# ZihanLiao/pytorch-kaldi-resnet

Hardware: AMD Instinct MI355X
Metric: utterances/sec (300-frame x 80 fbank, bs256/GPU), ResNet-34 + AAM-softmax training step (higher is better)
Workload: dtype f32 (operands as 2 fp16 terms of value x 2^k, 3 cross products, f32 accumulate); 1 GPU; BASELINE configs[1]: ResNet-34 + AAM-softmax (m 0.2, s 30), 1211 speakers, 300-frame x 80 fbank, per-GPU batch 256, fwd+CE+bwd+SGD(0.9, wd 5e-4); global_batch=256, frames=300, feat_dim=80, parallelism=dp1, launch=hipGraph replay (1 graph), mfma=f16x3

## Files before the change

include/spkhip.h:

```cpp
#ifndef SPKHIP_H
#define SPKHIP_H
#include <stddef.h>
#ifdef __cplusplus
extern "C" {
#endif

int spk_version(void);
const char* spk_last_error(void);
int spk_build_flags(void);

#define SPK_IN_AFFINE_RELU 1
#define SPK_EPI_AFFINE 2
#define SPK_EPI_ADD 4
#define SPK_EPI_RELU 8
#define SPK_EPI_STATS 16
#define SPK_IN_BNBWD 64
#define SPK_EPI_BNBWD 32

#define SPK_CONV_WS 128
#define SPK_CONV_PIPE 1024

#define SPK_CONV_M16 (1 << 17)

#define SPK_WGRAD_GROUPS 2048

#define SPK_WGRAD_NOSHIFT (1 << 18)
#define SPK_WGRAD_M16 (1 << 19)
#define SPK_IN_PRESPLIT (1 << 14)
#define SPK_SIDE_PRESPLIT (1 << 15)
#define SPK_DY_PRESPLIT (1 << 16)
#define SPK_EPI_WMASK (1 << 24)


int spk_pack_conv_weight(const float* w, float* wpk, int Cout, int Cin, int KH, int KW, int transpose, void* stream);
int spk_pack_conv_weight_split(const float* w, void* wpk, int Cout, int Cin, int KH, int KW, int transpose, int split,
                               void* stream);
int spk_pack_job_bytes(void);
int spk_pack_conv_weights_batched(const void* jobs, int njobs, int total_blocks, int has_f16 , void* stream);

int spk_conv_mfma(const float* in, const float* wpk, float* out, const float* in_scale, const float* in_shift,
                  const float* epi_scale, const float* epi_shift, const float* epi_add, const float* in_raw,
                  const float* in_act, const float* in_bn4, const float* in_coef, const unsigned* in_mask , const unsigned* bn_mask , const unsigned* add_mask ,
                  float* side_draw, float* side_dz,
                  const float* bn_raw, const float* bn_act, const float* bn4, float* stats, int B, int IH,
                  int IW, int Cin, int OH, int OW, int OHf, int OWf, int Cout, int IS, int OS, int ooy, int oox,
                  int ntaps, const int* tap_dy , const int* tap_dx , const int* tap_w , int TH,
                  int TW, int MT, int NT, int kc, int ips, int flags, int split, const unsigned* in_amax, unsigned* out_amax,
                  unsigned* side_amax, void* stream);
int spk_conv_mfma_len(const float* in, const float* wpk, float* out, const float* in_scale, const float* in_shift,
                      const float* epi_scale, const float* epi_shift, const float* epi_add, const float* in_raw,
                      const float* in_act, const float* in_bn4, const float* in_coef, const unsigned* in_mask,
                      const unsigned* bn_mask, const unsigned* add_mask, float* side_draw, float* side_dz,
                      const float* bn_raw, const float* bn_act, const float* bn4, float* stats, int B, int IH,
                      int IW, int Cin, int OH, int OW, int OHf, int OWf, int Cout, int IS, int OS, int ooy, int oox,
                      int ntaps, const int* tap_dy , const int* tap_dx , const int* tap_w , int TH,
                      int TW, int MT, int NT, int kc, int ips, int flags, int split, const unsigned* in_amax, unsigned* out_amax,
                      unsigned* side_amax, const int* wlen , void* stream);

int spk_conv_wgrad_limits(int WN, int* max_halo_pix , int* max_tile_pix );
size_t spk_conv_wgrad_workspace(int nsplit, int ksize, int Cin, int Cout);
int spk_conv3x3_c32_stream(const float* in, const float* wpk, float* out, const float* in_scale, const float* in_shift, float* stats,
                           int B, int H, int W, int flags, const unsigned* in_amax, unsigned* out_amax, int nblocks, void* stream);
int spk_conv1x1_stream(const float* in, const float* wpk, float* out, const float* in_scale, const float* in_shift,
                       const float* epi_add, const unsigned* add_mask, const float* bn_raw, const unsigned* bn_mask,
                       const float* bn4, float* stats, long long P, int C, int flags, const unsigned* in_amax, unsigned* out_amax,
                       int nblocks, void* stream);
int spk_conv1x1_stream_rows(int nblocks, int C);
int spk_wgrad_reduce(const float* partial, float* dw, int nslab, int ksize, int Cin, int Cout, int accumulate, void* stream);
int spk_conv_wgrad(const float* x, const float* dy, float* dw, float* partial, const float* in_scale,
                   const float* in_shift, int B, int IH, int IW, int Cin, int OH, int OW, int Cout, int ksize, int stride,
                   int TH, int TW, int WN, int nsplit, int flags, int accumulate, int split , const unsigned* dy_amax , const unsigned* x_amax , void* stream);

int spk_stem_fwd_blocks(int B, int F, int T);
int spk_stem_conv_fwd(const float* x, const float* w, float* out, float* stats, const float* epi_scale,
                      const float* epi_shift, int B, int F, int T, int flags,
                      unsigned* amax_out , void* stream);
int spk_stem_conv_fwd_len(const float* x, const float* w, float* out, float* stats, const float* epi_scale,
                          const float* epi_shift, int B, int F, int T, int flags, unsigned* amax_out, const int* len ,
                          void* stream);
int spk_stem_wgrad_blocks(int B, int F, int T);
int spk_stem_conv_wgrad(const float* x, const float* draw, float* dw, float* partial, int B, int F, int T,
                        int accumulate, void* stream);

int spk_bn_stats_blocks(long long N, int C);
int spk_bn_stats_partial(const float* x, float* partial , long long N, int C, void* stream);
size_t spk_bn_finalize_workspace(int nblk, int C);
int spk_bn_finalize(const float* partial, int nblk, int C, double count, const float* gamma, const float* beta,
                    float* running_mean, float* running_var, long long* num_batches_tracked, float* mean, float* invstd,
                    float* scale, float* shift, float momentum, float eps, double* ws,
                    const unsigned* amax_in, unsigned* est_out ,
                    void* stream);
int spk_bn_eval_coeffs(const float* gamma, const float* beta, const float* running_mean, const float* running_var,
                       float* scale, float* shift, int C, float eps, void* stream);
int spk_bn_apply(const float* raw, const float* scale, const float* shift, const float* res, const float* res_scale,
                 const float* res_shift, float* out, unsigned* mask_out, long long N, int C, int relu,
                 unsigned* amax_out , void* stream);
int spk_bn_bwd_reduce(const float* dy, const float* raw, const float* act, const float* mean, const float* invstd,
                      const float* scale, const float* shift, float* partial, long long N, int C, int mask_mode,
                      unsigned* chan_amax , void* stream);
int spk_bn_bwd_finalize(const float* partial, int nblk, int C, double count, const float* gamma, const float* invstd,
                        float* dgamma, float* dbeta, float* coef , int accumulate, double* ws,
                        const unsigned* amax_in, const unsigned* raw_amax, const float* mean, unsigned* est_out ,
                        const unsigned* chan_amax ,
                        void* stream);
int spk_bn_bwd_apply(const float* dy, const float* raw, const float* act, const float* mean, const float* invstd,
                     const float* scale, const float* shift, const float* coef, float* draw, float* dz_out, long long N,
                     int C, int mask_mode, unsigned* amax_out ,
                     const unsigned* pair_scale , void* stream);
int spk_absmax(const float* x, unsigned* slot, long long n, void* stream);
int spk_bnbwd_estimate(const float* coef, const float* mean, const float* invstd, int C, const unsigned* amax_in,
                       const unsigned* raw_amax, unsigned* est, void* stream);
int spk_f16_window_count(const float* x, const float* scale, const float* shift, long long n, int C, const unsigned* slot,
                         int pairs, unsigned long long* counts , void* stream);
int spk_affine_estimate(const float* scale, const float* shift, int C, const unsigned* amax_in, unsigned* est, void* stream);

int spk_stats_pool_fwd(const float* x , float* out , int B, int H, int W, int C,
                       int mode, void* stream);
int spk_stats_pool_fwd_len(const float* x, float* out, const int* wlen, int B, int H, int W, int C, int mode, void* stream);
int spk_stats_pool_bwd(const float* x, const float* gout, float* dx, int B, int H, int W, int C, int mode,
                       unsigned* amax_out , void* stream);

int spk_gemm_splitk(int M, int N, int K);
size_t spk_gemm_workspace(int M, int N, int K);
int spk_gemm_f32(const float* A, const float* B, float* C, const float* bias, int M, int N, int K, long long sam,
                 long long sak, long long sbk, long long sbn, long long ldc, float alpha, int accumulate, float* workspace,
                 void* stream);
int spk_colsum(const float* dy, float* db, int M, int N, int accumulate, void* stream);

int spk_l2norm_fwd(const float* x, float* y, float* inv_norm, int R, int D, float eps, void* stream);
int spk_l2norm_bwd(const float* y, const float* inv_norm, const float* dy, float* dx, int R, int D, float eps,
                   int accumulate, void* stream);
int spk_aam_margin_fwd(const float* cosv, const long long* label, float* logits, int B, int S, float m, float s,
                       void* stream);
int spk_aam_margin_bwd(const float* cosv, const long long* label, const float* dlogits, float* dcos, int B, int S,
                       float m, float s, void* stream);
int spk_softmax_ce(const float* logits, const long long* label, float* loss_row, float* dlogits, int* rank, int B, int S,
                   float grad_scale, void* stream);
int spk_mean(const float* v, float* out, int n, void* stream);
int spk_relu_bwd(const float* y, const float* dy, float* dx, long long n, void* stream);

int spk_sgd_step(float* p, const float* g, float* buf, long long n, float lr, float momentum, float weight_decay,
                 float grad_scale, int first_step, void* stream);

int spk_center_normalize(const float* emb , const float* mean , float* out, int N, int D, float eps,
                         void* stream);
int spk_trial_cosine(const float* en , const float* te , const int* ia, const int* ib, float* out,
                     int T, int D, int n_en, int n_te, void* stream);
int spk_topk_mean_std(const float* scores, float* mean_out, float* std_out, int N, int M, int k, long long ld, void* stream);

int spk_fbank_tile_frames(int L, int S, int P, int F);
int spk_fbank_fwd(const float* wave, const int* nsamp, const long long* utt_ids, int B, long long Nmax, const float* window,
                  const float* twiddle, const float* mel_w, const int* mel_lo, const int* mel_off, int L, int S, int P, int F,
                  int snip_edges, float dither, float preemph, int remove_dc, float energy_floor, unsigned long long seed,
                  float* feats, float* log_energy, int* T_out, int Tcap, void* stream);
int spk_fbank_dither_noise(float* out , long long utt_id, unsigned long long seed, int frame0, int nframes, int L,
                           void* stream);
int spk_vad_count(const float* log_energy, const int* T, int B, int Tcap, double energy_threshold, double mean_scale,
                  int frames_context, double proportion, int* vad , int* idx , int* count ,
                  void* stream);
int spk_cmn_select(const float* x, const int* T, const int* idx, const int* count, double* prefix, float* out, int B, int F,
                   int Tcap, int Tout, int cmn_window, void* stream);

int spk_resample_tile(int iu, int ou, int K);
int spk_resample_fwd(const float* wave_in, const int* nsamp_in, int B, long long Nmax_in, const int* first, const float* wq,
                     int fi, int fo, int K, float* wave_out, int* nsamp_out, long long Nmax_out, void* stream);

int spk_augment_max_rir(void);
int spk_augment_max_early(void);
int spk_augment_workspace(int B, long long Nmax, int Rmax, int Emax, long long Fmax, int nd, long long* sizes );
int spk_augment_fwd(const float* wave, const int* nsamp, int B, long long Nmax, const float* rir_pool, long long rir_pool_len,
                    const long long* rir_off, const int* rir_row, int Rmax, int Emax, const float* noise_pool,
                    long long noise_pool_len, const int* desc_ptr, const long long* desc_off, const int* desc_len,
                    const double* desc_snr, int nd, long long Fmax, const float* twiddle, float* spectra, float* y, double* work,
                    int quantize, float* out, unsigned long long* clipped, void* stream);

int spk_cm_decode(const unsigned char* codes, const float* colhdr, const int* lengths, int B, int F, int T, float* out, void* stream);
int spk_cm_compress(const float* x, const int* T, int B, int F, int Tcap, float* ws, float* minrange, int* hdr, unsigned char* codes,
                    void* stream);

#ifdef __cplusplus
}
#endif
#endif
```

pytorch-kaldi-resnet_amd/csrc/bn.hip:

```cpp
#include "spk_common.h"

enum { MASK_NONE = 0, MASK_ACT = 1, MASK_RAW = 2, MASK_BITS = 3 };

__global__ __launch_bounds__(256) void bn_stats_partial_kernel(const float* __restrict__ x, float* __restrict__ partial,
                                                               long long N, int C, int rows_per_block) {
    __shared__ float red[256][8];
    const int tid = threadIdx.x;
    const int qpr = C >> 2;
    const int quad = tid % qpr, prow = tid / qpr, rstep = 256 / qpr;
    const long long r0 = (long long)blockIdx.x * rows_per_block;
    long long r1 = r0 + rows_per_block;
    if (r1 > N) r1 = N;
    f32x4 s = {0.f, 0.f, 0.f, 0.f}, ss = {0.f, 0.f, 0.f, 0.f};
    for (long long r = r0 + prow; r < r1; r += rstep) {
        const f32x4 v = *(const f32x4*)(x + r * C + quad * 4);
        s += v;
        ss += v * v;
    }
#pragma unroll
    for (int k = 0; k < 4; ++k) {
        red[tid][k] = s[k];
        red[tid][4 + k] = ss[k];
    }
    __syncthreads();
    if (tid < qpr) {
        float a[8];
#pragma unroll
        for (int k = 0; k < 8; ++k) a[k] = 0.f;
        for (int p = 0; p < rstep; ++p)
#pragma unroll
            for (int k = 0; k < 8; ++k) a[k] += red[p * qpr + tid][k];
        float* dst = partial + ((size_t)blockIdx.x * C + tid * 4) * 2;
#pragma unroll
        for (int k = 0; k < 4; ++k) {
            dst[k * 2 + 0] = a[k];
            dst[k * 2 + 1] = a[4 + k];
        }
    }
}

static bool bn_c_ok(int C) { return C >= 4 && C <= 1024 && (C & (C - 1)) == 0; }

#ifndef BN_STATS_BLOCKS
#define BN_STATS_BLOCKS 4096
#endif
extern "C" int spk_bn_stats_blocks(long long N, int C) {
    (void)C;
    long long nb = (N + 255) / 256;
    if (nb > BN_STATS_BLOCKS) nb = BN_STATS_BLOCKS;
    return (int)(nb < 1 ? 1 : nb);
}

extern "C" int spk_bn_stats_partial(const float* x, float* partial, long long N, int C, void* stream) {
    SPK_REQUIRE(x && partial, "spk_bn_stats_partial: null pointer");
    SPK_REQUIRE(N > 0 && bn_c_ok(C), "spk_bn_stats_partial: N=%lld C=%d (C must be a power of two in [4,1024])", N, C);
    const int nb = spk_bn_stats_blocks(N, C);
    const int rpb = (int)((N + nb - 1) / nb);
    hipLaunchKernelGGL(bn_stats_partial_kernel, dim3(nb), dim3(256), 0, (hipStream_t)stream, x, partial, N, C, rpb);
    SPK_LAUNCH_CHECK("spk_bn_stats_partial");
    return 0;
}

#define BN_STAGE_ROWS 256
__global__ __launch_bounds__(256) void bn_fold_partials_kernel(const float* __restrict__ partial, double* __restrict__ ws,
                                                               int nblk, int C) {
    __shared__ double red[8][32][2];
    const int tid = threadIdx.x, c = tid & 31, row = tid >> 5;
    const int ch = blockIdx.x * 32 + c;
    const int per = (nblk + BN_STAGE_ROWS - 1) / BN_STAGE_ROWS;
    const int k0 = blockIdx.y * per;
    int k1 = k0 + per;
    if (k1 > nblk) k1 = nblk;
    double s = 0.0, ss = 0.0;
    if (ch < C) {
        const size_t pitch = (size_t)8 * C * 2;
        const float* q = partial + ((size_t)(k0 + row) * C + ch) * 2;
        int k = k0 + row;
        for (; k + 24 < k1; k += 32, q += 4 * pitch) {
            const float2 a = *(const float2*)q, b = *(const float2*)(q + pitch);
            const float2 c2 = *(const float2*)(q + 2 * pitch), d = *(const float2*)(q + 3 * pitch);
            s += (double)a.x; ss += (double)a.y;
            s += (double)b.x; ss += (double)b.y;
            s += (double)c2.x; ss += (double)c2.y;
            s += (double)d.x; ss += (double)d.y;
        }
        for (; k < k1; k += 8, q += pitch) {
            const float2 p = *(const float2*)q;
            s += (double)p.x;
            ss += (double)p.y;
        }
    }
    red[row][c][0] = s;
    red[row][c][1] = ss;
    __syncthreads();
    if (row == 0 && ch < C) {
        for (int k = 1; k < 8; ++k) {
            s += red[k][c][0];
            ss += red[k][c][1];
        }
        ws[((size_t)blockIdx.y * C + ch) * 2 + 0] = s;
        ws[((size_t)blockIdx.y * C + ch) * 2 + 1] = ss;
    }
}

template <typename T>
__device__ inline void bn_sum_rows(const T* __restrict__ partial, int nrows, int C, int ch, int row, double& s, double& ss) {
    const size_t pitch = (size_t)8 * C * 2;
    const T* p = partial + ((size_t)row * C + ch) * 2;
    int k = row;
    for (; k + 24 < nrows; k += 32, p += 4 * pitch) {
        const T a0 = p[0], a1 = p[1], b0 = p[pitch], b1 = p[pitch + 1];
        const T c0 = p[2 * pitch], c1 = p[2 * pitch + 1], d0 = p[3 * pitch], d1 = p[3 * pitch + 1];
        s += (double)a0; ss += (double)a1;
        s += (double)b0; ss += (double)b1;
        s += (double)c0; ss += (double)c1;
        s += (double)d0; ss += (double)d1;
    }
    for (; k < nrows; k += 8, p += pitch) {
        s += (double)p[0];
        ss += (double)p[1];
    }
}

template <typename T>
__global__ __launch_bounds__(256) void bn_finalize_kernel(const T* __restrict__ partial, int nblk, int C, double count,
                                                          const float* __restrict__ gamma, const float* __restrict__ beta,
                                                          float* __restrict__ running_mean, float* __restrict__ running_var,
                                                          long long* __restrict__ nbt, float* __restrict__ mean_out,
                                                          float* __restrict__ invstd_out, float* __restrict__ scale,
                                                          float* __restrict__ shift, float momentum, float eps,
                                                          const unsigned* __restrict__ amax_in, unsigned* __restrict__ est_out) {
    __shared__ double red[8][32][2];
    const int tid = threadIdx.x, c = tid & 31, row = tid >> 5;
    const int ch = blockIdx.x * 32 + c;
    double s = 0.0, ss = 0.0;
    if (ch < C) bn_sum_rows<T>(partial, nblk, C, ch, row, s, ss);
    red[row][c][0] = s;
    red[row][c][1] = ss;
    __syncthreads();
    if (row == 0 && ch < C) {
        for (int k = 1; k < 8; ++k) {
            s += red[k][c][0];
            ss += red[k][c][1];
        }
        const double mean = s / count;
        double var = ss / count - mean * mean;
        if (var < 0.0) var = 0.0;
        const float invstd = (float)(1.0 / sqrt(var + (double)eps));
        const float g = gamma[ch], b = beta[ch];
        const float sc = g * invstd;
        mean_out[ch] = (float)mean;
        invstd_out[ch] = invstd;
        const float shv = b - (float)mean * sc;
        scale[ch] = sc;
        shift[ch] = shv;
        if (est_out) {
            const float e = fabsf(sc) * __uint_as_float(*amax_in) + fabsf(shv);
            const unsigned bits = __float_as_uint(e);
            if (bits > __hip_atomic_load(est_out, __ATOMIC_RELAXED, __HIP_MEMORY_SCOPE_AGENT)) atomicMax(est_out, bits);
        }
        if (running_mean) {
            const double unbiased = count > 1.0 ? var * (count / (count - 1.0)) : var;
            running_mean[ch] = (1.f - momentum) * running_mean[ch] + momentum * (float)mean;
            running_var[ch] = (1.f - momentum) * running_var[ch] + momentum * (float)unbiased;
        }
    }
    if (nbt && blockIdx.x == 0 && tid == 0) *nbt += 1;
}

extern "C" size_t spk_bn_finalize_workspace(int nblk, int C) {
    return nblk > BN_STAGE_ROWS ? (size_t)BN_STAGE_ROWS * C * 2 * sizeof(double) : 0;
}

extern "C" int spk_bn_finalize(const float* partial, int nblk, int C, double count, const float* gamma, const float* beta,
                               float* running_mean, float* running_var, long long* num_batches_tracked, float* mean,
                               float* invstd, float* scale, float* shift, float momentum, float eps, double* ws,
                               const unsigned* amax_in, unsigned* est_out, void* stream) {
    SPK_REQUIRE(partial && gamma && beta && mean && invstd && scale && shift, "spk_bn_finalize: null pointer");
    SPK_REQUIRE(nblk > 0 && C > 0 && count > 0, "spk_bn_finalize: bad sizes");
    SPK_REQUIRE((running_mean == nullptr) == (running_var == nullptr), "spk_bn_finalize: running stats must come in pairs");
    SPK_REQUIRE(!est_out || amax_in, "spk_bn_finalize: est_out needs amax_in");
    hipStream_t st = (hipStream_t)stream;
    if (spk_bn_finalize_workspace(nblk, C)) {
        SPK_REQUIRE(ws, "spk_bn_finalize: %d partial rows need the fp64 workspace", nblk);
        hipLaunchKernelGGL(bn_fold_partials_kernel, dim3(spk_ceil_div(C, 32), BN_STAGE_ROWS), dim3(256), 0, st, partial, ws, nblk, C);
        SPK_LAUNCH_CHECK("spk_bn_finalize(fold)");
        hipLaunchKernelGGL(bn_finalize_kernel<double>, dim3(spk_ceil_div(C, 32)), dim3(256), 0, st, ws, BN_STAGE_ROWS, C, count,
                           gamma, beta, running_mean, running_var, num_batches_tracked, mean, invstd, scale, shift, momentum, eps,
                           amax_in, est_out);
    } else {
        hipLaunchKernelGGL(bn_finalize_kernel<float>, dim3(spk_ceil_div(C, 32)), dim3(256), 0, st, partial, nblk, C, count, gamma,
                           beta, running_mean, running_var, num_batches_tracked, mean, invstd, scale, shift, momentum, eps, amax_in,
                           est_out);
    }
    SPK_LAUNCH_CHECK("spk_bn_finalize");
    return 0;
}

__global__ void bn_eval_coeffs_kernel(const float* gamma, const float* beta, const float* rm, const float* rv,
                                      float* scale, float* shift, int C, float eps) {
    const int c = blockIdx.x * blockDim.x + threadIdx.x;
    if (c >= C) return;
    const float invstd = 1.f / sqrtf(rv[c] + eps);
    const float sc = gamma[c] * invstd;
    scale[c] = sc;
    shift[c] = beta[c] - rm[c] * sc;
}

extern "C" int spk_bn_eval_coeffs(const float* gamma, const float* beta, const float* running_mean,
                                  const float* running_var, float* scale, float* shift, int C, float eps, void* stream) {
    SPK_REQUIRE(gamma && beta && running_mean && running_var && scale && shift, "spk_bn_eval_coeffs: null pointer");
    hipLaunchKernelGGL(bn_eval_coeffs_kernel, dim3(spk_ceil_div(C, 256)), dim3(256), 0, (hipStream_t)stream, gamma, beta,
                       running_mean, running_var, scale, shift, C, eps);
    SPK_LAUNCH_CHECK("spk_bn_eval_coeffs");
    return 0;
}

#ifndef BN_APPLY_U
#define BN_APPLY_U 4
#endif
#ifndef BN_APPLY_CAP
#define BN_APPLY_CAP 0
#endif
#ifndef BN_BWD_APPLY_U
#define BN_BWD_APPLY_U 1
#endif
#ifndef BN_BWD_APPLY_CAP
#define BN_BWD_APPLY_CAP 2048
#endif
static int stream_grid(long long nquads, int per_thread = 1, int cap = 8192) {
    long long nb = (nquads + 256LL * per_thread - 1) / (256LL * per_thread);
    if (cap > 0 && nb > cap) nb = cap;
    if (nb > 2147483647LL) nb = 2147483647LL;
    return (int)(nb < 1 ? 1 : nb);
}
#ifndef BN_NT
#define BN_NT 1
#endif
static __device__ __forceinline__ f32x4 ld_stream(const float* p) {
#if BN_NT
    return __builtin_nontemporal_load((const f32x4*)p);
#else
    return *(const f32x4*)p;
#endif
}
static __device__ __forceinline__ void st_stream(float* p, f32x4 v) {
#if BN_NT
    __builtin_nontemporal_store(v, (f32x4*)p);
#else
    *(f32x4*)p = v;
#endif
}
__global__ __launch_bounds__(256) void bn_apply_kernel(const float* __restrict__ raw, const float* __restrict__ scale,
                                                       const float* __restrict__ shift, const float* __restrict__ res,
                                                       const float* __restrict__ rscale, const float* __restrict__ rshift,
                                                       float* __restrict__ out, unsigned* __restrict__ mask_out, long long nquads,
                                                       int C, int relu, unsigned* __restrict__ amax_out) {
    const int cmask = C - 1;
    float mx = 0.f;
    constexpr int U = BN_APPLY_U;
    const long long stride = (long long)gridDim.x * 256;
    const bool fixed_c = C <= 1024;
    const int c0 = (threadIdx.x * 4) & cmask;
    f32x4 psc = *(const f32x4*)(scale + c0), psh = *(const f32x4*)(shift + c0), prs = psc, prh = psh;
    if (rscale) {
        prs = *(const f32x4*)(rscale + c0);
        prh = *(const f32x4*)(rshift + c0);
    }
    for (long long i0 = (long long)blockIdx.x * 256 + threadIdx.x; i0 < nquads; i0 += stride * U) {
        f32x4 rv[U], sv[U];
        long long idx[U];
#pragma unroll
        for (int u = 0; u < U; ++u) {
            const long long i = i0 + stride * u;
            idx[u] = i < nquads ? i : i0;
            rv[u] = ld_stream(raw + idx[u] * 4);
            if (res) sv[u] = ld_stream(res + idx[u] * 4);
        }
#pragma unroll
        for (int u = 0; u < U; ++u) {
            const long long i = i0 + stride * u;
            if (i >= nquads) continue;
            if (!fixed_c) {
                const int c = (int)((i * 4) & cmask);
                psc = *(const f32x4*)(scale + c);
                psh = *(const f32x4*)(shift + c);
                if (rscale) {
                    prs = *(const f32x4*)(rscale + c);
                    prh = *(const f32x4*)(rshift + c);
                }
            }
            f32x4 v = rv[u] * psc + psh;
            if (res) {
                f32x4 r = sv[u];
                if (rscale) r = r * prs + prh;
                v += r;
            }
            if (relu) {
                v[0] = fmaxf(v[0], 0.f);
                v[1] = fmaxf(v[1], 0.f);
                v[2] = fmaxf(v[2], 0.f);
                v[3] = fmaxf(v[3], 0.f);
            }
            st_stream(out + i * 4, v);
            mx = fmaxf(fmaxf(mx, fmaxf(fabsf(v[0]), fabsf(v[1]))), fmaxf(fabsf(v[2]), fabsf(v[3])));
            if (mask_out) {
                unsigned bits = (v[0] > 0.f ? 1u : 0u) | (v[1] > 0.f ? 2u : 0u) | (v[2] > 0.f ? 4u : 0u) | (v[3] > 0.f ? 8u : 0u);
                bits <<= 4 * (threadIdx.x & 7);
                bits |= __shfl_xor(bits, 1, 64);
                bits |= __shfl_xor(bits, 2, 64);
                bits |= __shfl_xor(bits, 4, 64);
                if ((threadIdx.x & 7) == 0) mask_out[i >> 3] = bits;
            }
        }
    }
    if (amax_out) spk_wave_amax_commit(mx, amax_out);
}

extern "C" int spk_bn_apply(const float* raw, const float* scale, const float* shift, const float* res,
                            const float* res_scale, const float* res_shift, float* out, unsigned* mask_out, long long N, int C,
                            int relu, unsigned* amax_out, void* stream) {
    SPK_REQUIRE(raw && scale && shift && out, "spk_bn_apply: null pointer");
    SPK_REQUIRE(N > 0 && bn_c_ok(C), "spk_bn_apply: N=%lld C=%d", N, C);
    SPK_REQUIRE((res_scale == nullptr) == (res_shift == nullptr), "spk_bn_apply: residual affine must come in pairs");
    SPK_REQUIRE(!res_scale || res, "spk_bn_apply: residual affine without residual");
    SPK_REQUIRE(!mask_out || C % 32 == 0, "spk_bn_apply: the sign mask needs C %% 32 == 0 (C=%d)", C);
    const long long nquads = N * C / 4;
    hipLaunchKernelGGL(bn_apply_kernel, dim3(stream_grid(nquads, BN_APPLY_U, BN_APPLY_CAP)), dim3(256), 0, (hipStream_t)stream, raw, scale, shift, res,
                       res_scale, res_shift, out, mask_out, nquads, C, relu, amax_out);
    SPK_LAUNCH_CHECK("spk_bn_apply");
    return 0;
}

__device__ inline f32x4 bn_mask(f32x4 dy, int mode, const float* act, const float* raw_p, f32x4 rawv, f32x4 sc, f32x4 sh,
                                long long off, int C = 0) {
    if (mode == MASK_BITS) {
        const int lg = 31 - __builtin_clz((unsigned)C);
        const long long pix = off >> lg;
        const int c = (int)(off & (C - 1));
        const unsigned bits = ((const unsigned*)act)[pix * (C >> 5) + (c >> 5)] >> (c & 31);
#pragma unroll
        for (int k = 0; k < 4; ++k) dy[k] = ((bits >> k) & 1u) ? dy[k] : 0.f;
    } else if (mode == MASK_ACT) {
        const f32x4 a = *(const f32x4*)(act + off);
#pragma unroll
        for (int k = 0; k < 4; ++k) dy[k] = a[k] > 0.f ? dy[k] : 0.f;
    } else if (mode == MASK_RAW) {
        const f32x4 z = rawv * sc + sh;
#pragma unroll
        for (int k = 0; k < 4; ++k) dy[k] = z[k] > 0.f ? dy[k] : 0.f;
    }
    (void)raw_p;
    return dy;
}

__global__ __launch_bounds__(256) void bn_bwd_reduce_kernel(const float* __restrict__ dy, const float* __restrict__ raw,
                                                            const float* __restrict__ act, const float* __restrict__ mean,
                                                            const float* __restrict__ invstd, const float* __restrict__ scale,
                                                            const float* __restrict__ shift, float* __restrict__ partial,
                                                            long long N, int C, int rows_per_block, int mode,
                                                            unsigned* __restrict__ chan_amax) {
    __shared__ float red[256][8];
    const int tid = threadIdx.x;
    const int qpr = C >> 2;
    const int quad = tid % qpr, prow = tid / qpr, rstep = 256 / qpr;
    const long long r0 = (long long)blockIdx.x * rows_per_block;
    long long r1 = r0 + rows_per_block;
    if (r1 > N) r1 = N;
    const f32x4 mu = *(const f32x4*)(mean + quad * 4), is = *(const f32x4*)(invstd + quad * 4);
    const f32x4 sc = *(const f32x4*)(scale + quad * 4), sh = *(const f32x4*)(shift + quad * 4);
    f32x4 s = {0.f, 0.f, 0.f, 0.f}, ss = {0.f, 0.f, 0.f, 0.f}, mx = {0.f, 0.f, 0.f, 0.f};
    for (long long r = r0 + prow; r < r1; r += rstep) {
        const long long off = r * C + quad * 4;
        const f32x4 rv = ld_stream(raw + off);
        f32x4 d = ld_stream(dy + off);
        d = bn_mask(d, mode, act, raw, rv, sc, sh, off, C);
        const f32x4 xh = (rv - mu) * is;
        s += d;
        ss += d * xh;
#pragma unroll
        for (int k = 0; k < 4; ++k) mx[k] = fmaxf(mx[k], spk_finite_abs(d[k]));
    }
#pragma unroll
    for (int k = 0; k < 4; ++k) {
        red[tid][k] = s[k];
        red[tid][4 + k] = ss[k];
    }
    __syncthreads();
    if (tid < qpr) {
        float a[8];
#pragma unroll
        for (int k = 0; k < 8; ++k) a[k] = 0.f;
        for (int p = 0; p < rstep; ++p)
#pragma unroll
            for (int k = 0; k < 8; ++k) a[k] += red[p * qpr + tid][k];
        float* dst = partial + ((size_t)blockIdx.x * C + tid * 4) * 2;
#pragma unroll
        for (int k = 0; k < 4; ++k) {
            dst[k * 2 + 0] = a[k];
            dst[k * 2 + 1] = a[4 + k];
        }
    }
    if (chan_amax) {
        __syncthreads();
#pragma unroll
        for (int k = 0; k < 4; ++k) red[tid][k] = mx[k];
        __syncthreads();
        if (tid < qpr) {
#pragma unroll
            for (int k = 0; k < 4; ++k) {
                float m = 0.f;
                for (int p = 0; p < rstep; ++p) m = fmaxf(m, red[p * qpr + tid][k]);
                const unsigned bits = __float_as_uint(m);
                unsigned* slot = chan_amax + tid * 4 + k;
                if (bits > __hip_atomic_load(slot, __ATOMIC_RELAXED, __HIP_MEMORY_SCOPE_AGENT)) atomicMax(slot, bits);
            }
        }
    }
}

extern "C" int spk_bn_bwd_reduce(const float* dy, const float* raw, const float* act, const float* mean, const float* invstd,
                                 const float* scale, const float* shift, float* partial, long long N, int C, int mask_mode,
                                 unsigned* chan_amax, void* stream) {
    SPK_REQUIRE(dy && raw && mean && invstd && scale && shift && partial, "spk_bn_bwd_reduce: null pointer");
    SPK_REQUIRE(N > 0 && bn_c_ok(C), "spk_bn_bwd_reduce: N=%lld C=%d", N, C);
    SPK_REQUIRE(mask_mode >= 0 && mask_mode <= 3, "spk_bn_bwd_reduce: mask_mode=%d", mask_mode);
    SPK_REQUIRE((mask_mode != MASK_ACT && mask_mode != MASK_BITS) || act, "spk_bn_bwd_reduce: MASK_ACT / MASK_BITS need the activated tensor / its sign bits");
    const int nb = spk_bn_stats_blocks(N, C);
    const int rpb = (int)((N + nb - 1) / nb);
    hipLaunchKernelGGL(bn_bwd_reduce_kernel, dim3(nb), dim3(256), 0, (hipStream_t)stream, dy, raw, act, mean, invstd, scale,
                       shift, partial, N, C, rpb, mask_mode, chan_amax);
    SPK_LAUNCH_CHECK("spk_bn_bwd_reduce");
    return 0;
}

__device__ inline float bnbwd_bound(float k1, float m1, float m2, float mean, float invstd, float A, float R) {
    const float xh = (R + fabsf(mean)) * fabsf(invstd);
    return fabsf(k1) * (A + fabsf(m1) + xh * fabsf(m2)) * (1.f + 1.52587890625e-05f);
}

template <typename T>
__global__ __launch_bounds__(256) void bn_bwd_finalize_kernel(const T* __restrict__ partial, int nblk, int C, double count,
                                                              const float* __restrict__ gamma, const float* __restrict__ invstd,
                                                              float* __restrict__ dgamma, float* __restrict__ dbeta,
                                                              float* __restrict__ coef, int accumulate,
                                                              const unsigned* __restrict__ amax_in, const unsigned* __restrict__ raw_amax,
                                                              const float* __restrict__ mean, unsigned* __restrict__ est_out,
                                                              const unsigned* __restrict__ chan_amax) {
    __shared__ double red[8][32][2];
    const int tid = threadIdx.x, c = tid & 31, row = tid >> 5;
    const int ch = blockIdx.x * 32 + c;
    double s = 0.0, ss = 0.0;
    if (ch < C) bn_sum_rows<T>(partial, nblk, C, ch, row, s, ss);
    red[row][c][0] = s;
    red[row][c][1] = ss;
    __syncthreads();
    if (row == 0 && ch < C) {
        for (int k = 1; k < 8; ++k) {
            s += red[k][c][0];
            ss += red[k][c][1];
        }
        dbeta[ch] = accumulate ? dbeta[ch] + (float)s : (float)s;
        dgamma[ch] = accumulate ? dgamma[ch] + (float)ss : (float)ss;
        const float k1 = gamma[ch] * invstd[ch], m1 = (float)(s / count), m2 = (float)(ss / count);
        coef[ch] = k1;
        coef[C + ch] = m1;
        coef[2 * C + ch] = m2;
        if (est_out) {
            const float A = chan_amax ? __uint_as_float(chan_amax[ch]) : __uint_as_float(*amax_in);
            const float e = bnbwd_bound(k1, m1, m2, mean[ch], invstd[ch], A, __uint_as_float(*raw_amax));
            const unsigned bits = __float_as_uint(e);
            if (bits > __hip_atomic_load(est_out, __ATOMIC_RELAXED, __HIP_MEMORY_SCOPE_AGENT)) atomicMax(est_out, bits);
        }
    }
}

extern "C" int spk_bn_bwd_finalize(const float* partial, int nblk, int C, double count, const float* gamma,
                                   const float* invstd, float* dgamma, float* dbeta, float* coef, int accumulate,
                                   double* ws, const unsigned* amax_in, const unsigned* raw_amax, const float* mean,
                                   unsigned* est_out, const unsigned* chan_amax, void* stream) {
    SPK_REQUIRE(partial && gamma && invstd && dgamma && dbeta && coef, "spk_bn_bwd_finalize: null pointer");
    SPK_REQUIRE(nblk > 0 && C > 0 && count > 0, "spk_bn_bwd_finalize: bad sizes");
    SPK_REQUIRE(!est_out || ((amax_in || chan_amax) && raw_amax && mean),
                "spk_bn_bwd_finalize: est_out needs amax_in (or chan_amax), raw_amax and mean");
    hipStream_t st = (hipStream_t)stream;
    if (spk_bn_finalize_workspace(nblk, C)) {
        SPK_REQUIRE(ws, "spk_bn_bwd_finalize: %d partial rows need the fp64 workspace", nblk);
        hipLaunchKernelGGL(bn_fold_partials_kernel, dim3(spk_ceil_div(C, 32), BN_STAGE_ROWS), dim3(256), 0, st, partial, ws, nblk, C);
        SPK_LAUNCH_CHECK("spk_bn_bwd_finalize(fold)");
        hipLaunchKernelGGL(bn_bwd_finalize_kernel<double>, dim3(spk_ceil_div(C, 32)), dim3(256), 0, st, ws, BN_STAGE_ROWS, C, count,
                           gamma, invstd, dgamma, dbeta, coef, accumulate, amax_in, raw_amax, mean, est_out, chan_amax);
    } else {
        hipLaunchKernelGGL(bn_bwd_finalize_kernel<float>, dim3(spk_ceil_div(C, 32)), dim3(256), 0, st, partial, nblk, C, count, gamma,
                           invstd, dgamma, dbeta, coef, accumulate, amax_in, raw_amax, mean, est_out, chan_amax);
    }
    SPK_LAUNCH_CHECK("spk_bn_bwd_finalize");
    return 0;
}

__global__ __launch_bounds__(256) void bn_bwd_apply_kernel(const float* __restrict__ dy, const float* __restrict__ raw,
                                                           const float* __restrict__ act, const float* __restrict__ mean,
                                                           const float* __restrict__ invstd, const float* __restrict__ scale,
                                                           const float* __restrict__ shift, const float* __restrict__ coef,
                                                           float* __restrict__ draw, float* __restrict__ dz_out,
                                                           unsigned nquads, int C, int mode, unsigned* __restrict__ amax_out,
                                                           const unsigned* __restrict__ pair_scale) {
    const int cmask = C - 1;
    float mx = 0.f;
    const float sig = pair_scale ? spk_sigma_from_amax_bits(*pair_scale) : 1.f;
    constexpr int U = BN_BWD_APPLY_U;
    const unsigned stride = gridDim.x * 256u;
    const int lgq = 29 - __builtin_clz((unsigned)C);
    const unsigned cw = (unsigned)C >> 5;
    const bool fixed_c = C <= 1024;
    const int c0 = (threadIdx.x * 4) & cmask;
    f32x4 pmu = *(const f32x4*)(mean + c0), pis = *(const f32x4*)(invstd + c0), pk1 = *(const f32x4*)(coef + c0);
    f32x4 pm1 = *(const f32x4*)(coef + C + c0), pm2 = *(const f32x4*)(coef + 2 * C + c0), psc = pmu, psh = pmu;
    if (mode == MASK_RAW) {
        psc = *(const f32x4*)(scale + c0);
        psh = *(const f32x4*)(shift + c0);
    }
    for (unsigned i0 = blockIdx.x * 256u + threadIdx.x; i0 < nquads; i0 += stride * U) {
        f32x4 rvv[U], dv[U], av[U];
        unsigned mw[U];
#pragma unroll
        for (int u = 0; u < U; ++u) {
            const unsigned i = i0 + stride * u;
            const unsigned ii = i < nquads && i >= i0 ? i : i0;
            const size_t off = (size_t)ii * 4;
            rvv[u] = ld_stream(raw + off);
            dv[u] = ld_stream(dy + off);
            if (mode == MASK_BITS) mw[u] = ((const unsigned*)act)[(size_t)(ii >> lgq) * cw + (((ii * 4u) & (unsigned)cmask) >> 5)];
            else if (mode == MASK_ACT) av[u] = *(const f32x4*)(act + off);
        }
#pragma unroll
        for (int u = 0; u < U; ++u) {
            const unsigned i = i0 + stride * u;
            if (i >= nquads || i < i0) continue;
            const int c = fixed_c ? c0 : (int)((i * 4u) & (unsigned)cmask);
            if (!fixed_c) {
                pmu = *(const f32x4*)(mean + c);
                pis = *(const f32x4*)(invstd + c);
                pk1 = *(const f32x4*)(coef + c);
                pm1 = *(const f32x4*)(coef + C + c);
                pm2 = *(const f32x4*)(coef + 2 * C + c);
                if (mode == MASK_RAW) {
                    psc = *(const f32x4*)(scale + c);
                    psh = *(const f32x4*)(shift + c);
                }
            }
            const size_t off = (size_t)i * 4;
            const f32x4 rv = rvv[u];
            f32x4 d = dv[u];
            if (mode == MASK_BITS) {
                const unsigned bits = mw[u] >> (c & 31);
#pragma unroll
                for (int k = 0; k < 4; ++k) d[k] = ((bits >> k) & 1u) ? d[k] : 0.f;
            } else if (mode == MASK_ACT) {
#pragma unroll
                for (int k = 0; k < 4; ++k) d[k] = av[u][k] > 0.f ? d[k] : 0.f;
            } else if (mode == MASK_RAW) {
                const f32x4 z = rv * psc + psh;
#pragma unroll
                for (int k = 0; k < 4; ++k) d[k] = z[k] > 0.f ? d[k] : 0.f;
            }
            const f32x4 xh = (rv - pmu) * pis;
            const f32x4 o = pk1 * (d - pm1 - xh * pm2);
            if (dz_out) st_stream(dz_out + off, d);
            if (pair_scale) {
                uint2 t0, t1;
                split2h(o, sig, t0, t1);
                st_stream(draw + off, spk_pair_pack(t0, t1));
            } else
                st_stream(draw + off, o);
            mx = fmaxf(fmaxf(mx, fmaxf(fabsf(o[0]), fabsf(o[1]))), fmaxf(fabsf(o[2]), fabsf(o[3])));
        }
    }
    if (amax_out) spk_wave_amax_commit(mx, amax_out);
}

extern "C" int spk_bn_bwd_apply(const float* dy, const float* raw, const float* act, const float* mean, const float* invstd,
                                const float* scale, const float* shift, const float* coef, float* draw, float* dz_out,
                                long long N, int C, int mask_mode, unsigned* amax_out, const unsigned* pair_scale, void* stream) {
    SPK_REQUIRE(dy && raw && mean && invstd && scale && shift && coef && draw, "spk_bn_bwd_apply: null pointer");
    SPK_REQUIRE(N > 0 && bn_c_ok(C), "spk_bn_bwd_apply: N=%lld C=%d", N, C);
    SPK_REQUIRE(mask_mode >= 0 && mask_mode <= 3, "spk_bn_bwd_apply: mask_mode=%d", mask_mode);
    SPK_REQUIRE((mask_mode != MASK_ACT && mask_mode != MASK_BITS) || act, "spk_bn_bwd_apply: MASK_ACT / MASK_BITS need the activated tensor / its sign bits");
    const long long nquads = N * C / 4;
    SPK_REQUIRE(nquads < 2147483647LL / 8, "spk_bn_bwd_apply: %lld values exceed the 32-bit group index of the kernel", N * C);
    hipLaunchKernelGGL(bn_bwd_apply_kernel, dim3(stream_grid(nquads, BN_BWD_APPLY_U, BN_BWD_APPLY_CAP)), dim3(256), 0, (hipStream_t)stream, dy, raw, act, mean,
                       invstd, scale, shift, coef, draw, dz_out, (unsigned)nquads, C, mask_mode, amax_out, pair_scale);
    SPK_LAUNCH_CHECK("spk_bn_bwd_apply");
    return 0;
}

__global__ __launch_bounds__(256) void absmax_kernel(const float* __restrict__ x, long long n, unsigned* __restrict__ slot) {
    float mx = 0.f;
    const long long nq = n >> 2;
    for (long long i = (long long)blockIdx.x * 256 + threadIdx.x; i < nq; i += (long long)gridDim.x * 256) {
        const f32x4 v = *(const f32x4*)(x + i * 4);
        mx = fmaxf(fmaxf(mx, fmaxf(spk_finite_abs(v[0]), spk_finite_abs(v[1]))), fmaxf(spk_finite_abs(v[2]), spk_finite_abs(v[3])));
    }
    if (blockIdx.x == 0 && threadIdx.x < (n & 3)) mx = fmaxf(mx, spk_finite_abs(x[nq * 4 + threadIdx.x]));
    spk_wave_amax_commit(mx, slot);
}

extern "C" int spk_absmax(const float* x, unsigned* slot, long long n, void* stream) {
    SPK_REQUIRE(x && slot && n > 0, "spk_absmax: bad arguments");
    SPK_REQUIRE((((size_t)x) & 15) == 0, "spk_absmax: x must be 16-byte aligned");
    hipLaunchKernelGGL(absmax_kernel, dim3(stream_grid(n / 4 + 1)), dim3(256), 0, (hipStream_t)stream, x, n, slot);
    SPK_LAUNCH_CHECK("spk_absmax");
    return 0;
}

__global__ __launch_bounds__(256) void bnbwd_estimate_kernel(const float* __restrict__ coef, const float* __restrict__ mean,
                                                             const float* __restrict__ invstd, int C,
                                                             const unsigned* __restrict__ amax_in, const unsigned* __restrict__ raw_amax,
                                                             unsigned* __restrict__ est) {
    __shared__ float red[4];
    const float A = __uint_as_float(*amax_in), R = __uint_as_float(*raw_amax);
    float mx = 0.f;
    for (int c = threadIdx.x; c < C; c += 256)
        mx = fmaxf(mx, bnbwd_bound(coef[c], coef[C + c], coef[2 * C + c], mean[c], invstd[c], A, R));
#pragma unroll
    for (int off = 32; off >= 1; off >>= 1) mx = fmaxf(mx, __shfl_xor(mx, off, 64));
    if ((threadIdx.x & 63) == 0) red[threadIdx.x >> 6] = mx;
    __syncthreads();
    if (threadIdx.x == 0) *est = __float_as_uint(fmaxf(fmaxf(red[0], red[1]), fmaxf(red[2], red[3])));
}

__global__ __launch_bounds__(256) void affine_estimate_kernel(const float* __restrict__ scale, const float* __restrict__ shift, int C,
                                                              const unsigned* __restrict__ amax_in, unsigned* __restrict__ est) {
    __shared__ float red[2][4];
    float ms = 0.f, mh = 0.f;
    for (int c = threadIdx.x; c < C; c += 256) {
        ms = fmaxf(ms, fabsf(scale[c]));
        mh = fmaxf(mh, fabsf(shift[c]));
    }
#pragma unroll
    for (int off = 32; off >= 1; off >>= 1) {
        ms = fmaxf(ms, __shfl_xor(ms, off, 64));
        mh = fmaxf(mh, __shfl_xor(mh, off, 64));
    }
    if ((threadIdx.x & 63) == 0) {
        red[0][threadIdx.x >> 6] = ms;
        red[1][threadIdx.x >> 6] = mh;
    }
    __syncthreads();
    if (threadIdx.x == 0) {
        ms = fmaxf(fmaxf(red[0][0], red[0][1]), fmaxf(red[0][2], red[0][3]));
        mh = fmaxf(fmaxf(red[1][0], red[1][1]), fmaxf(red[1][2], red[1][3]));
        *est = __float_as_uint(ms * __uint_as_float(*amax_in) + mh);
    }
}

extern "C" int spk_affine_estimate(const float* scale, const float* shift, int C, const unsigned* amax_in, unsigned* est,
                                   void* stream) {
    SPK_REQUIRE(scale && shift && amax_in && est && C > 0, "spk_affine_estimate: bad arguments");
    hipLaunchKernelGGL(affine_estimate_kernel, dim3(1), dim3(256), 0, (hipStream_t)stream, scale, shift, C, amax_in, est);
    SPK_LAUNCH_CHECK("spk_affine_estimate");
    return 0;
}

extern "C" int spk_bnbwd_estimate(const float* coef, const float* mean, const float* invstd, int C, const unsigned* amax_in,
                                  const unsigned* raw_amax, unsigned* est, void* stream) {
    SPK_REQUIRE(coef && mean && invstd && amax_in && raw_amax && est && C > 0, "spk_bnbwd_estimate: bad arguments");
    hipLaunchKernelGGL(bnbwd_estimate_kernel, dim3(1), dim3(256), 0, (hipStream_t)stream, coef, mean, invstd, C, amax_in, raw_amax, est);
    SPK_LAUNCH_CHECK("spk_bnbwd_estimate");
    return 0;
}

__global__ __launch_bounds__(256) void f16_window_count_kernel(const float* __restrict__ x, const float* __restrict__ scale,
                                                               const float* __restrict__ shift, long long nquads, int C,
                                                               const unsigned* __restrict__ slot, int pairs,
                                                               unsigned long long* __restrict__ counts) {
    const float sig = spk_sigma_from_amax_bits(*slot);
    const int cmask = C - 1;
    unsigned n = 0, sat = 0, lo_lost = 0, hi_sub = 0;
    for (long long i = (long long)blockIdx.x * 256 + threadIdx.x; i < nquads; i += (long long)gridDim.x * 256) {
        f32x4 v = *(const f32x4*)(x + i * 4);
        float hi[4], lo[4];
        if (pairs) {
            const uint4 u = __builtin_bit_cast(uint4, v);
            const f16x4 a = __builtin_bit_cast(f16x4, (uint2){u.x, u.y}), b = __builtin_bit_cast(f16x4, (uint2){u.z, u.w});
#pragma unroll
            for (int k = 0; k < 4; ++k) {
                hi[k] = (float)a[k];
                lo[k] = (float)b[k];
                sat += fabsf(hi[k]) >= 65504.f;
            }
        } else {
            if (scale) {
                const int c = (int)((i * 4) & cmask);
                v = v * *(const f32x4*)(scale + c) + *(const f32x4*)(shift + c);
#pragma unroll
                for (int k = 0; k < 4; ++k) v[k] = fmaxf(v[k], 0.f);
            }
#pragma unroll
            for (int k = 0; k < 4; ++k) {
                const float u = v[k] * sig;
                sat += fabsf(u) > 65504.f;
                const float uc = __builtin_amdgcn_fmed3f(u, -65504.f, 65504.f);
                const _Float16 a = (_Float16)uc;
                hi[k] = (float)a;
                lo[k] = (float)(_Float16)(uc - (float)a);
            }
        }
#pragma unroll
        for (int k = 0; k < 4; ++k) {
            n += 1;
            lo_lost += lo[k] != 0.f && fabsf(lo[k]) < 6.103515625e-05f;
            hi_sub += hi[k] != 0.f && fabsf(hi[k]) < 6.103515625e-05f;
        }
    }
    unsigned vals[4] = {n, sat, lo_lost, hi_sub};
#pragma unroll
    for (int j = 0; j < 4; ++j) {
        unsigned v = vals[j];
#pragma unroll
        for (int off = 32; off >= 1; off >>= 1) v += __shfl_xor(v, off, 64);
        if ((threadIdx.x & 63) == 0 && v) atomicAdd(counts + j, (unsigned long long)v);
    }
}

extern "C" int spk_f16_window_count(const float* x, const float* scale, const float* shift, long long n, int C,
                                    const unsigned* slot, int pairs, unsigned long long* counts, void* stream) {
    SPK_REQUIRE(x && slot && counts && n > 0 && n % 4 == 0, "spk_f16_window_count: bad arguments (n must be a multiple of 4)");
    SPK_REQUIRE((scale == nullptr) == (shift == nullptr), "spk_f16_window_count: scale / shift come in pairs");
    SPK_REQUIRE(!scale || (bn_c_ok(C) && !pairs), "spk_f16_window_count: the affine form needs a power-of-two C and an fp32 tensor");
    hipLaunchKernelGGL(f16_window_count_kernel, dim3(stream_grid(n / 4)), dim3(256), 0, (hipStream_t)stream, x, scale, shift, n / 4,
                       scale ? C : 4, slot, pairs, counts);
    SPK_LAUNCH_CHECK("spk_f16_window_count");
    return 0;
}
```

pytorch-kaldi-resnet_amd/csrc/conv_split.hip:

```cpp
#include "conv_kernel.h"

template <int MT, int NT, int SPLIT>
static int launch_split(const ConvArgs& a, size_t lds_bytes, hipStream_t st) {
    if (a.flags & SPK_IN_BNBWD) {
#ifndef SPK_NO_FL_VARIANTS
        if constexpr (SPLIT == 3 && MT == 2 && NT == 1) {
            const int var = a.flags | (a.add_mask ? SPK_FL_ADDMASK : 0) | (a.bn_mask ? SPK_FL_BNMASK : 0) | (a.in_mask ? SPK_FL_INMASK : 0);
            constexpr int V2 = SPK_IN_BNBWD | SPK_SIDE_PRESPLIT | SPK_EPI_STATS | SPK_EPI_BNBWD | SPK_FL_INMASK;
            constexpr int V1 = SPK_IN_BNBWD | SPK_SIDE_PRESPLIT | SPK_EPI_ADD | SPK_EPI_STATS | SPK_EPI_BNBWD | SPK_FL_ADDMASK | SPK_FL_BNMASK;
            if (!a.in_act && !a.bn_act && !a.side_dz && (var == V1 || var == V2)) {
                if (var == V2) hipLaunchKernelGGL((conv_mfma_kernel<MT, NT, true, SPLIT, V2>), dim3(a.nblocks), dim3(256), lds_bytes, st, a);
                else hipLaunchKernelGGL((conv_mfma_kernel<MT, NT, true, SPLIT, V1>), dim3(a.nblocks), dim3(256), lds_bytes, st, a);
                SPK_LAUNCH_CHECK("spk_conv_mfma(split)");
                return 0;
            }
        }
#endif
        hipLaunchKernelGGL((conv_mfma_kernel<MT, NT, true, SPLIT>), dim3(a.nblocks), dim3(256), lds_bytes, st, a);
    } else if (a.flags & SPK_EPI_WMASK) {
        hipLaunchKernelGGL((conv_mfma_kernel<MT, NT, false, SPLIT, SPK_EPI_WMASK>), dim3(a.nblocks), dim3(256), lds_bytes, st, a);
    } else {
#ifndef SPK_NO_FL_VARIANTS
        if constexpr (SPLIT == 3 && ((MT == 2 && NT == 1) || (MT == 1 && NT == 2) || (MT == 2 && NT == 2))) {
            if (!a.add_mask && !a.bn_mask && !a.bn_act) {
                if (a.flags == (SPK_IN_AFFINE_RELU | SPK_EPI_STATS)) {
                    hipLaunchKernelGGL((conv_mfma_kernel<MT, NT, false, SPLIT, SPK_IN_AFFINE_RELU | SPK_EPI_STATS>), dim3(a.nblocks), dim3(256), lds_bytes, st, a);
                    SPK_LAUNCH_CHECK("spk_conv_mfma(split)");
                    return 0;
                }
                if (a.flags == SPK_EPI_STATS) {
                    hipLaunchKernelGGL((conv_mfma_kernel<MT, NT, false, SPLIT, SPK_EPI_STATS>), dim3(a.nblocks), dim3(256), lds_bytes, st, a);
                    SPK_LAUNCH_CHECK("spk_conv_mfma(split)");
                    return 0;
                }
            }
        }
#endif
        hipLaunchKernelGGL((conv_mfma_kernel<MT, NT, false, SPLIT>), dim3(a.nblocks), dim3(256), lds_bytes, st, a);
    }
    SPK_LAUNCH_CHECK("spk_conv_mfma(split)");
    return 0;
}

int spk_launch_conv_split(const ConvArgs& a, size_t lds_bytes, int MT, int NT, int split, hipStream_t st) {
#define CASE(M, N)                                                      \
    if (MT == M && NT == N) {                                           \
        if (split == 3) return launch_split<M, N, 3>(a, lds_bytes, st); \
        if (split == 6) return launch_split<M, N, 6>(a, lds_bytes, st); \
        return launch_split<M, N, 9>(a, lds_bytes, st);                 \
    }
    CASE(1, 1) CASE(2, 1) CASE(3, 1) CASE(4, 1) CASE(1, 2) CASE(2, 2) CASE(3, 2) CASE(1, 4)
#undef CASE
    spk_set_error("spk_conv_mfma: unsupported split tile config MT=%d NT=%d", MT, NT);
    return -1;
}

#ifdef CONV_STAMPS
extern "C" int spk_debug_stamps(unsigned long long* out, int nblocks) {
    if (nblocks < 0) {
        void* p = nullptr;
        if (hipGetSymbolAddress(&p, HIP_SYMBOL(g_conv_stamps)) != hipSuccess) return -1;
        return (int)hipMemset(p, 0, sizeof(unsigned long long) * 16 * CONV_STAMP_BLOCKS);
    }
    if (nblocks > CONV_STAMP_BLOCKS) nblocks = CONV_STAMP_BLOCKS;
    return (int)hipMemcpyFromSymbol(out, HIP_SYMBOL(g_conv_stamps), (size_t)nblocks * 16 * sizeof(unsigned long long), 0, hipMemcpyDeviceToHost);
}
#endif
```

pytorch-kaldi-resnet_amd/csrc/spk_common.h:

```cpp
#pragma once
#include <hip/hip_runtime.h>
#include <stdint.h>

typedef float f32x4 __attribute__((ext_vector_type(4)));
typedef float f32x16 __attribute__((ext_vector_type(16)));

void spk_set_error(const char* fmt, ...);
#define SPK_REQUIRE(cond, ...)                 \
    do {                                       \
        if (!(cond)) {                         \
            spk_set_error(__VA_ARGS__);        \
            return -1;                         \
        }                                      \
    } while (0)
#define SPK_LAUNCH_CHECK(name)                                                          \
    do {                                                                                \
        hipError_t e__ = hipGetLastError();                                             \
        if (e__ != hipSuccess) {                                                        \
            spk_set_error("%s: launch failed: %s", name, hipGetErrorString(e__));       \
            return (int)e__;                                                            \
        }                                                                               \
    } while (0)

enum {
    SPK_IN_AFFINE_RELU = 1,
    SPK_EPI_AFFINE = 2,
    SPK_EPI_ADD = 4,
    SPK_EPI_RELU = 8,
    SPK_EPI_STATS = 16,
    SPK_EPI_BNBWD = 32,
    SPK_IN_BNBWD = 64,
    SPK_CONV_WS = 128,
    SPK_CONV_PIPE = 1024,
    SPK_WGRAD_GROUPS = 2048,
    SPK_IN_PRESPLIT = 1 << 14,
    SPK_SIDE_PRESPLIT = 1 << 15,
    SPK_DY_PRESPLIT = 1 << 16,
    SPK_CONV_M16 = 1 << 17,
    SPK_WGRAD_NOSHIFT = 1 << 18,
    SPK_WGRAD_M16 = 1 << 19,
    SPK_EPI_WMASK = 1 << 24
};

static inline int spk_ceil_div(int a, int b) { return (a + b - 1) / b; }

typedef __bf16 bf16x8 __attribute__((ext_vector_type(8)));
#ifdef __HIPCC__
static __device__ __forceinline__ unsigned pack_bf16x2(float lo, float hi, float& rlo, float& rhi) {
    const __bf16 a = (__bf16)lo, b = (__bf16)hi;
    rlo = lo - (float)a;
    rhi = hi - (float)b;
    return (unsigned)__builtin_bit_cast(unsigned short, a) | ((unsigned)__builtin_bit_cast(unsigned short, b) << 16);
}
static __device__ __forceinline__ void split3(f32x4 w, uint2& t0, uint2& t1, uint2& t2) {
    float r0, r1, r2, r3, q0, q1, q2, q3;
    t0.x = pack_bf16x2(w[0], w[1], r0, r1);
    t0.y = pack_bf16x2(w[2], w[3], r2, r3);
    t1.x = pack_bf16x2(r0, r1, q0, q1);
    t1.y = pack_bf16x2(r2, r3, q2, q3);
    t2.x = pack_bf16x2(q0, q1, r0, r1);
    t2.y = pack_bf16x2(q2, q3, r2, r3);
}
typedef _Float16 f16x8 __attribute__((ext_vector_type(8)));
#define SPK_F16_ACT_SIGMA 64.0f
typedef _Float16 f16x4 __attribute__((ext_vector_type(4)));
static __device__ __forceinline__ void split2h(f32x4 w, float sigma, uint2& t0, uint2& t1) {
    f32x4 u = w * sigma;
#pragma unroll
    for (int k = 0; k < 4; ++k) u[k] = __builtin_amdgcn_fmed3f(u[k], -65504.f, 65504.f);
    const f16x4 a = __builtin_convertvector(u, f16x4);
    const f32x4 r = u - __builtin_convertvector(a, f32x4);
    const f16x4 b = __builtin_convertvector(r, f16x4);
    t0 = __builtin_bit_cast(uint2, a);
    t1 = __builtin_bit_cast(uint2, b);
}
static __device__ __forceinline__ f32x4 spk_pair_pack(uint2 t0, uint2 t1) {
    return __builtin_bit_cast(f32x4, (uint4){t0.x, t0.y, t1.x, t1.y});
}
static __device__ __forceinline__ void spk_pair_unpack(f32x4 v, uint2& t0, uint2& t1) {
    const uint4 u = __builtin_bit_cast(uint4, v);
    t0 = (uint2){u.x, u.y};
    t1 = (uint2){u.z, u.w};
}
static __device__ __forceinline__ void spk_terms(f32x4 w, float sigma, bool pairs, uint2& t0, uint2& t1) {
    if (pairs) spk_pair_unpack(w, t0, t1);
    else split2h(w, sigma, t0, t1);
}
static __device__ __forceinline__ float spk_sigma_from_amax_bits(unsigned bits) {
    const int e = (int)((bits >> 23) & 0xffu);
    if (e == 0 || e == 255) return 1.f;
    int se = 127 + 14 - (e - 127);
    se = se < 1 ? 1 : (se > 254 ? 254 : se);
    return __uint_as_float((unsigned)se << 23);
}
static __device__ __forceinline__ float spk_finite_abs(float v) {
    const float a = fabsf(v);
    return a < __builtin_inff() ? a : 0.f;
}
static __device__ __forceinline__ void spk_wave_amax_commit(float v, unsigned* dst) {
#pragma unroll
    for (int off = 32; off >= 1; off >>= 1) v = fmaxf(v, __shfl_xor(v, off, 64));
    if ((threadIdx.x & 63) == 0) {
        const unsigned bits = __float_as_uint(v);
        if (bits > __hip_atomic_load(dst, __ATOMIC_RELAXED, __HIP_MEMORY_SCOPE_AGENT)) atomicMax(dst, bits);
    }
}
#endif

static __device__ __forceinline__ unsigned spk_m20(unsigned magic32) { return (magic32 + 0xFFFu) >> 12; }
static __device__ __forceinline__ int spk_div20(int p, unsigned m20) { return (int)(__umul24((unsigned)p, m20) >> 20); }
```

pytorch-kaldi-resnet_amd/csrc/stem.hip:

```cpp
#include "spk_common.h"

#define STEM_C 32

template <bool LEN>
__global__ __launch_bounds__(256) void stem_fwd_kernel(const float* __restrict__ x, const float* __restrict__ w,
                                                       float* __restrict__ out, float* __restrict__ stats,
                                                       const float* __restrict__ epi_scale,
                                                       const float* __restrict__ epi_shift, int B, int F, int T,
                                                       int flags, unsigned* __restrict__ amax_out, const int* __restrict__ len) {
    __shared__ float red[4][STEM_C][2];
    float mx = 0.f;
    const int tid = threadIdx.x, cg = tid & 3, pl = tid >> 2;
    float wr[9][8];
#pragma unroll
    for (int t = 0; t < 9; ++t)
#pragma unroll
        for (int c = 0; c < 8; ++c) wr[t][c] = w[(cg * 8 + c) * 9 + t];
    float es[8], eh[8], ssum[8], ssq[8];
#pragma unroll
    for (int c = 0; c < 8; ++c) {
        es[c] = (flags & SPK_EPI_AFFINE) ? epi_scale[cg * 8 + c] : 1.f;
        eh[c] = (flags & SPK_EPI_AFFINE) ? epi_shift[cg * 8 + c] : 0.f;
        ssum[c] = 0.f;
        ssq[c] = 0.f;
    }
    const int FT = F * T;
    const long long NP = (long long)B * FT;
    for (long long p = (long long)blockIdx.x * 64 + pl; p < NP; p += (long long)gridDim.x * 64) {
        const int b = (int)(p / FT);
        const int rem = (int)(p - (long long)b * FT);
        const int f = rem / T, t0 = rem - f * T;
        const float* xb = x + (size_t)b * FT;
        const int Tb = LEN ? min(len[b], T) : T;
        float xv[9];
#pragma unroll
        for (int kh = 0; kh < 3; ++kh)
#pragma unroll
            for (int kw = 0; kw < 3; ++kw) {
                const int ff = f + kh - 1, tt = t0 + kw - 1;
                xv[kh * 3 + kw] = (ff >= 0 && ff < F && tt >= 0 && tt < Tb) ? xb[ff * T + tt] : 0.f;
            }
        const bool tail = LEN && t0 >= Tb;
        float o[8];
#pragma unroll
        for (int c = 0; c < 8; ++c) {
            float v = 0.f;
#pragma unroll
            for (int t = 0; t < 9; ++t) v = fmaf(xv[t], wr[t][c], v);
            if (flags & SPK_EPI_AFFINE) v = v * es[c] + eh[c];
            if (flags & SPK_EPI_RELU) v = fmaxf(v, 0.f);
            if (tail) v = 0.f;
            o[c] = v;
            mx = fmaxf(mx, fabsf(v));
            ssum[c] += v;
            ssq[c] += v * v;
        }
        f32x4* dst = (f32x4*)(out + (size_t)p * STEM_C + cg * 8);
        dst[0] = (f32x4){o[0], o[1], o[2], o[3]};
        dst[1] = (f32x4){o[4], o[5], o[6], o[7]};
    }
    if (amax_out) spk_wave_amax_commit(mx, amax_out);
    if (flags & SPK_EPI_STATS) {
#pragma unroll
        for (int c = 0; c < 8; ++c) {
#pragma unroll
            for (int off = 4; off < 64; off <<= 1) {
                ssum[c] += __shfl_xor(ssum[c], off, 64);
                ssq[c] += __shfl_xor(ssq[c], off, 64);
            }
        }
        const int lane = tid & 63, wave = tid >> 6;
        if (lane < 4) {
#pragma unroll
            for (int c = 0; c < 8; ++c) {
                red[wave][lane * 8 + c][0] = ssum[c];
                red[wave][lane * 8 + c][1] = ssq[c];
            }
        }
        __syncthreads();
        if (tid < STEM_C) {
            float s0 = 0.f, s1 = 0.f;
#pragma unroll
            for (int wv = 0; wv < 4; ++wv) {
                s0 += red[wv][tid][0];
                s1 += red[wv][tid][1];
            }
            stats[((size_t)blockIdx.x * STEM_C + tid) * 2 + 0] = s0;
            stats[((size_t)blockIdx.x * STEM_C + tid) * 2 + 1] = s1;
        }
    }
}

extern "C" int spk_stem_fwd_blocks(int B, int F, int T) {
    long long np = (long long)B * F * T;
    long long nb = (np + 63) / 64;
    return (int)(nb < 2048 ? nb : 2048);
}

extern "C" int spk_stem_conv_fwd(const float* x, const float* w, float* out, float* stats, const float* epi_scale,
                                 const float* epi_shift, int B, int F, int T, int flags, unsigned* amax_out, void* stream) {
    SPK_REQUIRE(x && w && out, "spk_stem_conv_fwd: null pointer");
    SPK_REQUIRE(B > 0 && F > 0 && T > 0, "spk_stem_conv_fwd: empty input");
    SPK_REQUIRE(!(flags & SPK_EPI_STATS) || stats, "spk_stem_conv_fwd: EPI_STATS needs a stats buffer");
    SPK_REQUIRE(!(flags & SPK_EPI_AFFINE) || (epi_scale && epi_shift), "spk_stem_conv_fwd: EPI_AFFINE needs scale/shift");
    SPK_REQUIRE(!(flags & SPK_EPI_WMASK), "spk_stem_conv_fwd: SPK_EPI_WMASK needs the lengths (spk_stem_conv_fwd_len)");
    hipLaunchKernelGGL(stem_fwd_kernel<false>, dim3(spk_stem_fwd_blocks(B, F, T)), dim3(256), 0, (hipStream_t)stream, x, w, out,
                       stats, epi_scale, epi_shift, B, F, T, flags, amax_out, nullptr);
    SPK_LAUNCH_CHECK("spk_stem_conv_fwd");
    return 0;
}

extern "C" int spk_stem_conv_fwd_len(const float* x, const float* w, float* out, float* stats, const float* epi_scale,
                                     const float* epi_shift, int B, int F, int T, int flags, unsigned* amax_out, const int* len,
                                     void* stream) {
    SPK_REQUIRE(x && w && out && len, "spk_stem_conv_fwd_len: null pointer");
    SPK_REQUIRE(B > 0 && F > 0 && T > 0, "spk_stem_conv_fwd_len: empty input");
    SPK_REQUIRE(flags & SPK_EPI_WMASK, "spk_stem_conv_fwd_len: flags must carry SPK_EPI_WMASK");
    SPK_REQUIRE(!(flags & SPK_EPI_STATS) || stats, "spk_stem_conv_fwd_len: EPI_STATS needs a stats buffer");
    SPK_REQUIRE(!(flags & SPK_EPI_AFFINE) || (epi_scale && epi_shift), "spk_stem_conv_fwd_len: EPI_AFFINE needs scale/shift");
    hipLaunchKernelGGL(stem_fwd_kernel<true>, dim3(spk_stem_fwd_blocks(B, F, T)), dim3(256), 0, (hipStream_t)stream, x, w, out,
                       stats, epi_scale, epi_shift, B, F, T, flags, amax_out, len);
    SPK_LAUNCH_CHECK("spk_stem_conv_fwd_len");
    return 0;
}

__global__ __launch_bounds__(256) void stem_wgrad_kernel(const float* __restrict__ x, const float* __restrict__ draw,
                                                         float* __restrict__ partial, int B, int F, int T) {
    __shared__ float red[4][STEM_C * 9];
    const int tid = threadIdx.x, cg = tid & 3, pl = tid >> 2;
    float acc[9][8];
#pragma unroll
    for (int t = 0; t < 9; ++t)
#pragma unroll
        for (int c = 0; c < 8; ++c) acc[t][c] = 0.f;
    const int FT = F * T;
    const long long NP = (long long)B * FT;
    for (long long p = (long long)blockIdx.x * 64 + pl; p < NP; p += (long long)gridDim.x * 64) {
        const int b = (int)(p / FT);
        const int rem = (int)(p - (long long)b * FT);
        const int f = rem / T, t0 = rem - f * T;
        const float* xb = x + (size_t)b * FT;
        float xv[9];
#pragma unroll
        for (int kh = 0; kh < 3; ++kh)
#pragma unroll
            for (int kw = 0; kw < 3; ++kw) {
                const int ff = f + kh - 1, tt = t0 + kw - 1;
                xv[kh * 3 + kw] = (ff >= 0 && ff < F && tt >= 0 && tt < T) ? xb[ff * T + tt] : 0.f;
            }
        const f32x4* src = (const f32x4*)(draw + (size_t)p * STEM_C + cg * 8);
        const f32x4 d0 = src[0], d1 = src[1];
        const float d[8] = {d0[0], d0[1], d0[2], d0[3], d1[0], d1[1], d1[2], d1[3]};
#pragma unroll
        for (int t = 0; t < 9; ++t)
#pragma unroll
            for (int c = 0; c < 8; ++c) acc[t][c] = fmaf(xv[t], d[c], acc[t][c]);
    }
    const int lane = tid & 63, wave = tid >> 6;
#pragma unroll
    for (int t = 0; t < 9; ++t)
#pragma unroll
        for (int c = 0; c < 8; ++c) {
            float v = acc[t][c];
#pragma unroll
            for (int off = 4; off < 64; off <<= 1) v += __shfl_xor(v, off, 64);
            if (lane < 4) red[wave][(lane * 8 + c) * 9 + t] = v;
        }
    __syncthreads();
    for (int i = tid; i < STEM_C * 9; i += 256)
        partial[(size_t)blockIdx.x * (STEM_C * 9) + i] = (red[0][i] + red[1][i]) + (red[2][i] + red[3][i]);
}

__global__ __launch_bounds__(256) void stem_wgrad_reduce_kernel(const float* __restrict__ partial, float* __restrict__ dw,
                                                                int nblk, int accumulate) {
    __shared__ double red[256];
    const int i = blockIdx.x;
    double s = 0.0;
    for (int k = threadIdx.x; k < nblk; k += 256) s += (double)partial[(size_t)k * (STEM_C * 9) + i];
    red[threadIdx.x] = s;
    __syncthreads();
    for (int off = 128; off > 0; off >>= 1) {
        if ((int)threadIdx.x < off) red[threadIdx.x] += red[threadIdx.x + off];
        __syncthreads();
    }
    if (threadIdx.x == 0) dw[i] = accumulate ? dw[i] + (float)red[0] : (float)red[0];
}

extern "C" int spk_stem_wgrad_blocks(int B, int F, int T) {
    long long np = (long long)B * F * T;
    long long nb = (np + 63) / 64;
    return (int)(nb < 1024 ? nb : 1024);
}

extern "C" int spk_stem_conv_wgrad(const float* x, const float* draw, float* dw, float* partial, int B, int F, int T,
                                   int accumulate, void* stream) {
    SPK_REQUIRE(x && draw && dw && partial, "spk_stem_conv_wgrad: null pointer");
    SPK_REQUIRE(B > 0 && F > 0 && T > 0, "spk_stem_conv_wgrad: empty input");
    const int nblk = spk_stem_wgrad_blocks(B, F, T);
    hipLaunchKernelGGL(stem_wgrad_kernel, dim3(nblk), dim3(256), 0, (hipStream_t)stream, x, draw, partial, B, F, T);
    SPK_LAUNCH_CHECK("spk_stem_conv_wgrad");
    hipLaunchKernelGGL(stem_wgrad_reduce_kernel, dim3(STEM_C * 9), dim3(256), 0, (hipStream_t)stream, partial, dw, nblk, accumulate);
    SPK_LAUNCH_CHECK("spk_stem_wgrad_reduce");
    return 0;
}
```

pytorch-kaldi-resnet_amd/engine.py:

```python
import torch

from . import ops
from .hip import MASK_ACT, MASK_BITS, MASK_NONE, MASK_RAW


class _Conv:
    def __init__(self, holder):
        self.h = holder
        self.cin, self.cout, self.k, self.stride = holder.cin, holder.cout, holder.k, holder.stride
        self.wpk = None
        self.wpk_t = None

    def repack(self, need_t):
        w = self.h.weight.data
        if self.cin == 1:
            return
        self.wpk = ops.pack_conv_weight(w, False, self.wpk)
        if need_t:
            self.wpk_t = ops.pack_conv_weight(w, True, self.wpk_t)

    def pack_jobs(self, need_t):
        w = self.h.weight.data
        if self.cin == 1:
            return []
        n = ops.packed_numel(w)
        if self.wpk is None or self.wpk.numel() != n:
            self.wpk = torch.empty(n, device=w.device, dtype=torch.float32)
        jobs = [(w, self.wpk, False)]
        if need_t:
            nt = ops.packed_numel(w, bwd=True)
            if self.wpk_t is None or self.wpk_t.numel() != nt:
                self.wpk_t = torch.empty(nt, device=w.device, dtype=torch.float32)
            jobs.append((w, self.wpk_t, True))
        return jobs


class _BN:
    def __init__(self, holder):
        self.h = holder
        self.c = holder.c
        self.t4 = None
        self.s4 = None
        self.e2 = None

    def finalize(self, partial, count, amax_in=None, est_out=None, keep=True):
        name = "t4" if keep else "s4"
        if getattr(self, name) is None:
            setattr(self, name, torch.empty(4, self.c, device=partial.device, dtype=torch.float32))
        t4 = getattr(self, name)
        h = self.h
        ops.bn_finalize(partial, count, h.weight.data, h.bias.data, h.running_mean, h.running_var, h.num_batches_tracked,
                        t4, amax_in=amax_in, est_out=est_out)
        return t4

    def eval_coeffs(self):
        h = self.h
        if self.e2 is None:
            self.e2 = torch.empty(2, self.c, device=h.weight.device, dtype=torch.float32)
        ops.bn_eval_coeffs(h.weight.data, h.bias.data, h.running_mean, h.running_var, self.e2)
        return self.e2


class _Block:
    def __init__(self, bp):
        self.kind = bp.kind
        self.convs = [_Conv(bp.conv1), _Conv(bp.conv2)] + ([_Conv(bp.conv3)] if bp.kind == "bottleneck" else [])
        self.bns = [_BN(bp.bn1), _BN(bp.bn2)] + ([_BN(bp.bn3)] if bp.kind == "bottleneck" else [])
        self.ds = None
        if bp.downsample is not None:
            self.ds = (_Conv(bp.downsample[0]), _BN(bp.downsample[1]))


class _LogitsFn(torch.autograd.Function):

    @staticmethod
    def forward(ctx, eng, x, y, anchor):
        logits, saved = eng.forward_train(x, y)
        ctx.eng = eng
        ctx.saved = saved
        return logits

    @staticmethod
    def backward(ctx, dlogits):
        ctx.eng.backward(ctx.saved, dlogits.contiguous())
        ctx.saved = None
        return None, None, None, None


class Engine:
    def __init__(self, model):
        self.m = model
        r = model.res
        self.stem_conv = _Conv(r.conv1)
        self.stem_bn = _BN(r.bn1)
        self.blocks = []
        for li in range(1, 5):
            for bp in getattr(r, "layer%d" % li):
                self.blocks.append(_Block(bp))
        self.head_bn = _BN(model.bn1) if hasattr(model, "bn1") else None
        self.pool_mode = 1 if model.pooling == "mean+std" else 0
        self.dirty = True
        self._packed_for_bwd = False
        self._pack_tables = {}
        self._amax_pool = None
        self._amax_fwd = None
        self._amax_eval = None
        self._fwd_gen = 0
        self.wgrad_stream = None
        self.use_side_stream = True
        self.fuse_bn_reduce = True
        self.fuse_bn_apply = True
        import os
        self.use_sign_masks = os.environ.get("SPK_SIGN_MASKS", "1") == "1"
        self.fuse_apply_min_c = int(os.environ.get("SPK_FUSE_APPLY_MINC", "0"))
        self._fuse_apply_max_c = int(os.environ["SPK_FUSE_APPLY_MAXC"]) if "SPK_FUSE_APPLY_MAXC" in os.environ else None
        self.fuse_apply_1x1 = os.environ.get("SPK_FUSE_APPLY_1X1", "0") == "1"
        self.pair_draw = os.environ.get("SPK_PAIR_DRAW", "1") == "1"
        self.chan_amax = os.environ.get("SPK_CHAN_AMAX", "1") == "1"
        self.window_counts = None
        self.bound_log = None

    @property
    def fuse_apply_max_c(self):
        if self._fuse_apply_max_c is not None:
            return self._fuse_apply_max_c
        return 32 if (self.pair_draw and ops.split_for(3, True) == 3) else 1000000

    @fuse_apply_max_c.setter
    def fuse_apply_max_c(self, v):
        self._fuse_apply_max_c = v

    def _all_convs(self):
        for b in self.blocks:
            for c in b.convs:
                yield c
            if b.ds is not None:
                yield b.ds[0]

    def _repack(self, need_t):
        if not self.dirty and (self._packed_for_bwd or not need_t):
            return
        jobs = [j for c in self._all_convs() for j in c.pack_jobs(need_t)]
        key = [(w.data_ptr(), p.data_ptr(), t, ops.split_for(w.shape[2], t)) for w, p, t in jobs]
        tab = self._pack_tables.get(need_t)
        if tab is None or tab.key != key:
            assert not torch.cuda.is_current_stream_capturing() or tab is None, "pack table changed during graph capture"
            tab = self._pack_tables[need_t] = ops.PackTable(jobs, jobs[0][0].device)
        tab.run()
        self.dirty = False
        self._packed_for_bwd = need_t

    def _check_input(self, x):
        if not x.is_cuda:
            raise RuntimeError("pytorch_kaldi_resnet_amd runs on MI355X only: input must be a device tensor "
                               "(there is no CPU fallback)")
        if x.dim() != 3 or x.size(1) != self.m.feat_dim:
            raise RuntimeError("expected input [B, %d, T], got %s" % (self.m.feat_dim, tuple(x.shape)))
        if x.dtype != torch.float32:
            raise RuntimeError("expected float32 input")
        return x.contiguous()

    def _fwd_pool(self, device, train=False):
        if ops.split_for(3) != 3 and ops.split_for(3, True) != 3:
            return None
        name = "_amax_fwd" if train else "_amax_eval"
        if getattr(self, name) is None:
            setattr(self, name, ops.AmaxPool(device))
        pool = getattr(self, name)
        pool.reset()
        return pool

    def _count(self, x, slot, affine=None, pairs=False):
        if self.window_counts is not None and slot is not None:
            ops.f16_window_count(x, slot, self.window_counts, affine=affine, pairs=pairs)

    def trunk_eval(self, x, wl=None):
        self._repack(False)
        pool = self._fwd_pool(x.device)
        take = (lambda: pool.take()) if pool is not None else (lambda: None)
        f16 = ops.split_for(3) == 3
        e = self.stem_bn.eval_coeffs()
        a_amax = take()
        a, _ = ops.stem_fwd(x, self.stem_conv.h.weight.data, epi_affine=(e[0], e[1]), relu=True, amax_out=a_amax,
                            wlen=None if wl is None else wl[0])
        stage = 0
        for b in self.blocks:
            evs = [bn.eval_coeffs() for bn in b.bns]
            if b.ds is not None:
                ed = b.ds[1].eval_coeffs()
                res, _ = ops.conv_fwd(a, b.ds[0].wpk, b.ds[0].cout, 1, b.ds[0].stride, epi_affine=(ed[0], ed[1]),
                                      in_amax=a_amax if ops.split_for(1) == 3 else None)
            else:
                res = a
            h, h_amax = a, a_amax
            n = len(b.convs)
            for i, (c, ev) in enumerate(zip(b.convs, evs)):
                last = i == n - 1
                o_amax = take()
                if c.stride == 2:
                    stage += 1
                h, _ = ops.conv_fwd(h, c.wpk, c.cout, c.k, c.stride, epi_affine=(ev[0], ev[1]),
                                    epi_add=res if last else None, relu=True,
                                    in_amax=h_amax if ops.split_for(c.k) == 3 else None, out_amax=o_amax,
                                    wlen=None if wl is None else wl[stage])
                h_amax = o_amax
            a, a_amax = h, h_amax
        return a

    def embed_eval(self, x, wl=None):
        feat = self.trunk_eval(x, wl)
        pooled = ops.stats_pool_fwd(feat, self.pool_mode, wlen=None if wl is None else wl[3])
        return ops.linear_fwd(pooled, self.m.fc1.weight.data, self.m.fc1.bias.data)

    @staticmethod
    def stage_widths(lengths, B, T, device):
        if isinstance(lengths, torch.Tensor):
            if lengths.dtype.is_floating_point or lengths.dtype.is_complex or lengths.dtype == torch.bool:
                raise TypeError("lengths must be integers, got a %s tensor" % lengths.dtype)
            L = lengths.detach().to("cpu", torch.int64).reshape(-1)
            if lengths.dim() != 1:
                raise ValueError("lengths must be one-dimensional [B], got shape %s" % (tuple(lengths.shape),))
        else:
            vals = list(lengths)
            if not all(isinstance(v, int) or (hasattr(v, "__index__") and not isinstance(v, (bool, float))) for v in vals) \
                    or any(isinstance(v, bool) for v in vals):
                raise TypeError("lengths must be integers")
            L = torch.tensor([int(v) for v in vals], dtype=torch.int64)
        if L.numel() != B:
            raise ValueError("lengths has %d entries for a batch of %d utterances" % (L.numel(), B))
        if B and (int(L.min()) < 1 or int(L.max()) > T):
            raise ValueError("lengths must lie in [1, T=%d], got min %d max %d" % (T, int(L.min()), int(L.max())))
        w = [L]
        for _ in range(3):
            w.append((w[-1] + 1) // 2)
        return torch.stack(w).to(torch.int32).to(device)

    def predict(self, x, lengths=None):
        x = self._check_input(x)
        with torch.no_grad():
            if lengths is not None:
                if self.m.training:
                    raise RuntimeError("predict(lengths=...) needs eval mode: with BatchNorm batch statistics a padded batch has "
                                       "no per-utterance meaning (call model.eval() first)")
                return self.embed_eval(x, self.stage_widths(lengths, x.shape[0], x.shape[2], x.device))
            if self.m.training:
                emb, _ = self._embed_train(x, save=False)
                return emb
            return self.embed_eval(x)

    def _head_fwd(self, emb, y, train, save):
        m = self.m
        sv = {}
        h = emb
        if m.loss in ("softmax", "AAM-v1"):
            bn = self.head_bn
            if train:
                part = ops.bn_stats_partial(emb)
                t4 = bn.finalize(part, emb.shape[0], keep=save)
                h = ops.bn_apply(emb, t4[2], t4[3], relu=True)
            else:
                e2 = bn.eval_coeffs()
                h = ops.bn_apply(emb, e2[0], e2[1], relu=True)
            sv["h"] = h
        if m.loss == "softmax":
            logits = ops.linear_fwd(h, m.last.weight.data, m.last.bias.data)
        else:
            if y is None:
                raise RuntimeError("AAM heads need labels (scripts/model.py:483: label=None fails in the reference too)")
            y = y.contiguous()
            hn, hinv = ops.l2norm_fwd(h)
            wn, winv = ops.l2norm_fwd(m.last.weight.data)
            B, S, D = h.shape[0], wn.shape[0], wn.shape[1]
            cosv = ops.gemm(hn, wn, B, S, D, D, 1, 1, D)
            logits = ops.aam_margin_fwd(cosv, y, m.m, m.s)
            if save:
                sv.update(hn=hn, hinv=hinv, wn=wn, winv=winv, cosv=cosv, y=y)
        return logits, sv

    def _head_bwd(self, emb, sv, dlogits, acc):
        m = self.m
        if m.loss == "softmax":
            dh = ops.linear_bwd(sv["h"], m.last.weight.data, dlogits, m.last.weight.grad, m.last.bias.grad, accumulate=acc)
        else:
            dcos = ops.aam_margin_bwd(sv["cosv"], sv["y"], dlogits, m.m, m.s)
            B, S = dcos.shape
            D = sv["wn"].shape[1]
            dhn = ops.gemm(dcos, sv["wn"], B, D, S, S, 1, D, 1)
            dwn = ops.gemm(dcos, sv["hn"], S, D, B, 1, S, D, 1)
            dh = ops.l2norm_bwd(sv["hn"], sv["hinv"], dhn)
            ops.l2norm_bwd(sv["wn"], sv["winv"], dwn, out=m.last.weight.grad, accumulate=acc)
        if m.loss in ("softmax", "AAM-v1"):
            bn = self.head_bn
            dh = ops.bn_backward(dh, emb, sv["h"], bn.t4, bn.h.weight.data, bn.h.weight.grad, bn.h.bias.grad, MASK_ACT,
                                 accumulate=acc)
        return dh

    def _trunk_train(self, x, save):
        saved = {"x": x, "blocks": []}
        pool = self._fwd_pool(x.device, train=save)
        if save:
            self._fwd_gen += 1
        saved["gen"] = self._fwd_gen
        take = (lambda: pool.take()) if pool is not None else (lambda: None)
        f16 = ops.split_for(3) == 3
        raw0, st = ops.stem_fwd(x, self.stem_conv.h.weight.data, stats=True)
        B, F, T, _ = raw0.shape
        t4 = self.stem_bn.finalize(st, B * F * T, keep=save)
        use_masks = save and self.use_sign_masks
        a_amax = take()
        a = ops.bn_apply(raw0, t4[2], t4[3], relu=True, mask=use_masks, amax_out=a_amax)
        a, amask = a if use_masks else (a, None)
        saved["raw0"] = raw0
        for b in self.blocks:
            rec = {"x": a, "xmask": amask, "in_amax": [], "raw_amax": []}
            raws = []
            h, aff, h_amax = a, None, a_amax
            for c, bn in zip(b.convs, b.bns):
                rec["in_amax"].append(h_amax)
                raw_amax = take()
                rec["raw_amax"].append(raw_amax)
                if ops.split_for(c.k) == 3:
                    self._count(h, h_amax, affine=aff)
                raw, st = ops.conv_fwd(h, c.wpk, c.cout, c.k, c.stride, in_affine=aff, stats=True,
                                       in_amax=h_amax if ops.split_for(c.k) == 3 else None, out_amax=raw_amax)
                est = take()
                t4 = bn.finalize(st, raw.shape[0] * raw.shape[1] * raw.shape[2], amax_in=raw_amax, est_out=est, keep=save)
                raws.append(raw)
                h, aff, h_amax = raw, (t4[2], t4[3]), est
            out_amax = take()
            if b.ds is not None:
                rawd, st = ops.conv_fwd(a, b.ds[0].wpk, b.ds[0].cout, 1, b.ds[0].stride, stats=True,
                                        in_amax=a_amax if ops.split_for(1) == 3 else None)
                td = b.ds[1].finalize(st, rawd.shape[0] * rawd.shape[1] * rawd.shape[2], keep=save)
                out = ops.bn_apply(h, aff[0], aff[1], res=rawd, res_affine=(td[2], td[3]), relu=True, mask=use_masks,
                                   amax_out=out_amax)
                rec["rawd"] = rawd
            else:
                out = ops.bn_apply(h, aff[0], aff[1], res=a, relu=True, mask=use_masks, amax_out=out_amax)
            out, amask = out if use_masks else (out, None)
            rec["raws"] = raws
            rec["out"] = out
            rec["mask"] = amask
            if save:
                saved["blocks"].append(rec)
            a, a_amax = out, out_amax
        return a, saved

    def _embed_train(self, x, save):
        self._repack(save)
        feat, saved = self._trunk_train(x, save)
        pooled = ops.stats_pool_fwd(feat, self.pool_mode)
        emb = ops.linear_fwd(pooled, self.m.fc1.weight.data, self.m.fc1.bias.data)
        saved["feat"], saved["pooled"], saved["emb"] = feat, pooled, emb
        return emb, saved

    def forward_train(self, x, y):
        emb, saved = self._embed_train(x, True)
        logits, sv = self._head_fwd(emb, y, True, True)
        saved["head"] = sv
        return logits, saved

    def forward_logits(self, x, y=None):
        x = self._check_input(x)
        m = self.m
        if m.training and torch.is_grad_enabled():
            anchor = m.fc1.bias
            return _LogitsFn.apply(self, x, y, anchor)
        with torch.no_grad():
            if m.training:
                emb, _ = self._embed_train(x, save=False)
                logits, _ = self._head_fwd(emb, y, True, False)
            else:
                emb = self.embed_eval(x)
                logits, _ = self._head_fwd(emb, y, False, False)
            return logits

    def _wgrad(self, x, dy, dw, k, stride, in_affine=None, accumulate=False, dy_amax=None, x_amax=None, dy_presplit=False):
        if not self.use_side_stream:
            return ops.conv_wgrad(x, dy, dw, k, stride, in_affine=in_affine, accumulate=accumulate, dy_amax=dy_amax,
                                  x_amax=x_amax, dy_presplit=dy_presplit)
        if self.wgrad_stream is None:
            self.wgrad_stream = torch.cuda.Stream()
        main = torch.cuda.current_stream()
        side = self.wgrad_stream
        side.wait_stream(main)
        for t in (x, dy):
            t.record_stream(side)
        with torch.cuda.stream(side):
            ops.conv_wgrad(x, dy, dw, k, stride, in_affine=in_affine, accumulate=accumulate, dy_amax=dy_amax, x_amax=x_amax,
                           dy_presplit=dy_presplit)

    def _join_wgrad(self):
        if self.use_side_stream and self.wgrad_stream is not None:
            torch.cuda.current_stream().wait_stream(self.wgrad_stream)

    def backward(self, saved, dlogits, on_stage_done=None):
        m = self.m
        acc = not m.attach_grads()
        if saved.get("gen") != self._fwd_gen:
            raise RuntimeError("backward of a training forward whose BatchNorm statistics rows and operand-scale slots were reused "
                               "by a later training forward (the engine keeps one set per model: run backward before the next "
                               "forward that requires grad)")
        with torch.no_grad():
            demb = self._head_bwd(saved["emb"], saved["head"], dlogits, acc)
            dpooled = ops.linear_bwd(saved["pooled"], m.fc1.weight.data, demb, m.fc1.weight.grad, m.fc1.bias.grad,
                                     accumulate=acc)
            amx = None
            if ops.split_for(3, True) == 3:
                if self._amax_pool is None:
                    self._amax_pool = ops.AmaxPool(dpooled.device)
                amx = self._amax_pool
                amx.reset()
            d_amax = amx.take() if amx else None
            d = ops.stats_pool_bwd(saved["feat"], dpooled, self.pool_mode, amax_out=d_amax)
            if on_stage_done:
                on_stage_done("head")
            nblk = len(self.blocks)
            stage_of = []
            for li in range(1, 5):
                stage_of += [li] * len(getattr(m.res, "layer%d" % li))
            part = None
            last_stage = stage_of[-1]
            for bi in range(nblk - 1, -1, -1):
                if bi > 0:
                    prev = (saved["blocks"][bi - 1]["raws"][-1], self.blocks[bi - 1].bns[-1].t4)
                else:
                    prev = (saved["raw0"], self.stem_bn.t4)
                chan = self.chan_amax and amx is not None and stage_of[bi] == last_stage
                if chan and bi > 0 and stage_of[bi - 1] == last_stage:
                    prev = None
                d, part, d_amax = self._block_bwd(self.blocks[bi], saved["blocks"][bi], d, acc, part, prev, d_amax, amx, chan)
                saved["blocks"][bi] = None
                if on_stage_done and (bi == 0 or stage_of[bi - 1] != stage_of[bi]):
                    self._join_wgrad()
                    on_stage_done("layer%d" % stage_of[bi])
            bn = self.stem_bn
            draw0 = ops.bn_backward(d, saved["raw0"], None, bn.t4, bn.h.weight.data, bn.h.weight.grad, bn.h.bias.grad,
                                    MASK_RAW, draw_out=d, accumulate=acc, partial=part)
            ops.stem_wgrad(saved["x"], draw0, self.stem_conv.h.weight.grad, accumulate=acc)
            self._join_wgrad()
            if on_stage_done:
                on_stage_done("stem")

    def _block_bwd(self, b, rec, dout, acc, dout_partial=None, prev=None, dout_amax=None, amx=None, chan=False):
        x, raws, out = rec["x"], rec["raws"], rec["out"]
        n = len(b.convs)
        g, g_part, g_amax, dz = dout, dout_partial, dout_amax, None
        take = (lambda: amx.take()) if amx is not None else (lambda: None)
        for i in range(n - 1, -1, -1):
            c, bn, raw = b.convs[i], b.bns[i], raws[i]
            last = i == n - 1
            inp = x if i == 0 else raws[i - 1]
            in_aff = None if i == 0 else (b.bns[i - 1].t4[2], b.bns[i - 1].t4[3])
            hw = (inp.shape[1], inp.shape[2])
            act = out if last else None
            f16 = amx is not None and ops.split_for(c.k, True) == 3
            add_dz, bnb = False, None
            if i > 0:
                if c.stride == 1 and self.fuse_bn_reduce:
                    bnb = (raws[i - 1], None, b.bns[i - 1].t4)
            elif b.ds is None:
                add_dz = True
                if c.stride == 1 and self.fuse_bn_reduce and prev is not None:
                    bnb = (prev[0], x, prev[1])
                    if rec.get("xmask") is not None:
                        bnb = bnb + (rec["xmask"],)
            res_amax, draw_amax = take(), take()
            pairs = f16 and self.pair_draw
            raw_amax = rec["raw_amax"][i] if f16 else None
            if self.fuse_bn_apply and c.stride == 1 and (self.fuse_apply_min_c <= c.cout <= self.fuse_apply_max_c
                                                         or (c.k == 1 and self.fuse_apply_1x1)):
                ca = None
                if g_part is None:
                    ca = amx.take_n(c.cout) if (chan and last and f16) else None
                    g_part = ops.bn_bwd_partial(g, raw, act, bn.t4, MASK_ACT if last else MASK_RAW, chan_amax=ca)
                est = take() if f16 else None
                coef = ops.bn_bwd_coef(g_part, raw.numel() // raw.shape[-1], bn.h.weight.data, bn.t4, bn.h.weight.grad,
                                       bn.h.bias.grad, acc, amax_in=g_amax, raw_amax=raw_amax, est_out=est, chan_amax=ca)
                draw = torch.empty_like(raw)
                lazy_dz = b.ds is None and rec.get("mask") is not None and n > 1
                dzb = torch.empty_like(raw) if (last and not lazy_dz) else None
                inb = (raw, act, bn.t4, coef)
                if last and rec.get("mask") is not None:
                    inb = inb + (rec["mask"],)
                if add_dz and lazy_dz:
                    res = ops.conv_dgrad(g, c.wpk_t, c.cin, c.k, 1, hw, add=dout, add_mask=rec["mask"], bn_bwd=bnb,
                                         in_bnbwd=inb, side=(draw, dzb), in_amax=est, out_amax=res_amax, side_amax=draw_amax,
                                         side_presplit=pairs)
                else:
                    res = ops.conv_dgrad(g, c.wpk_t, c.cin, c.k, 1, hw, add=dz if add_dz else None, bn_bwd=bnb,
                                         in_bnbwd=inb, side=(draw, dzb), in_amax=est, out_amax=res_amax, side_amax=draw_amax,
                                         side_presplit=pairs)
                if last:
                    dz = dzb
                draw_slot = est if pairs else draw_amax
                self._count(draw, draw_slot, pairs=pairs)
                if self.bound_log is not None and est is not None:
                    self.bound_log.append((c.cout, c.k, est, draw_amax))
            else:
                lazy_dz = False
                est = take() if pairs else None
                pair = (g_amax, raw_amax, est) if pairs else None
                if last:
                    bits = rec.get("mask")
                    lazy_dz = b.ds is None and bits is not None and n > 1
                    ca = amx.take_n(c.cout) if (chan and pairs and g_part is None) else None
                    draw = ops.bn_backward(g, raw, bits if bits is not None else out, bn.t4, bn.h.weight.data, bn.h.weight.grad,
                                           bn.h.bias.grad, MASK_BITS if bits is not None else MASK_ACT,
                                           dz_out=None if lazy_dz else g, accumulate=acc, partial=g_part, amax_out=draw_amax,
                                           pair=pair, chan_amax=ca)
                    dz = None if lazy_dz else g
                else:
                    draw = ops.bn_backward(g, raw, None, bn.t4, bn.h.weight.data, bn.h.weight.grad, bn.h.bias.grad, MASK_RAW,
                                           draw_out=g, accumulate=acc, partial=g_part, amax_out=draw_amax, pair=pair)
                draw_slot = est if pairs else draw_amax
                self._count(draw, draw_slot, pairs=pairs)
                if self.bound_log is not None and est is not None:
                    self.bound_log.append((c.cout, c.k, est, draw_amax))
                if add_dz and dz is None and rec.get("mask") is not None:
                    res = ops.conv_dgrad(draw, c.wpk_t, c.cin, c.k, c.stride, hw, add=dout, add_mask=rec["mask"], bn_bwd=bnb,
                                         in_amax=draw_slot if f16 else None, out_amax=res_amax, in_presplit=pairs)
                else:
                    res = ops.conv_dgrad(draw, c.wpk_t, c.cin, c.k, c.stride, hw, add=dz if add_dz else None, bn_bwd=bnb,
                                         in_amax=draw_slot if f16 else None, out_amax=res_amax, in_presplit=pairs)
            g, g_part = res if bnb is not None else (res, None)
            g_amax = res_amax
            self._wgrad(inp, draw, c.h.weight.grad, c.k, c.stride, in_affine=in_aff, accumulate=acc,
                        dy_amax=draw_slot if f16 else None, x_amax=rec["in_amax"][i] if f16 else None, dy_presplit=pairs)
        dx, part, dx_amax = g, g_part, g_amax
        if b.ds is not None:
            cd, bnd = b.ds
            f16d = amx is not None and ops.split_for(1, True) == 3
            drawd_amax = take() if f16d else None
            drawd = ops.bn_backward(dz, rec["rawd"], None, bnd.t4, bnd.h.weight.data, bnd.h.weight.grad, bnd.h.bias.grad,
                                    MASK_NONE, draw_out=dz, accumulate=acc, amax_out=drawd_amax)
            self._count(drawd, drawd_amax)
            self._wgrad(x, drawd, cd.h.weight.grad, 1, cd.stride, accumulate=acc, dy_amax=drawd_amax,
                        x_amax=rec["in_amax"][0] if f16d else None)
            ops.conv_dgrad(drawd, cd.wpk_t, cd.cin, 1, cd.stride, (x.shape[1], x.shape[2]), out=dx, accumulate=True,
                           in_amax=drawd_amax, out_amax=dx_amax)
            part = None
        return dx, part, dx_amax

    def loss_and_grad(self, x, y, on_stage_done=None):
        x = self._check_input(x)
        y = y.contiguous()
        with torch.no_grad():
            logits, saved = self.forward_train(x, y)
            loss_row, dl, rank = ops.softmax_ce(logits, y, grad_scale=1.0 / logits.shape[0])
            loss = ops.mean(loss_row)
        self.backward(saved, dl, on_stage_done)
        return loss, logits, rank


STAGE_ORDER = ["head", "layer4", "layer3", "layer2", "layer1", "stem"]


class GraphedTrainStep:

    def __init__(self, engine, batch, frames, warmup=2, side_stream=None, segmented=False, pool=None):
        import os
        if side_stream is None:
            side_stream = os.environ.get("SPK_GRAPH_SIDE", "0") == "1"
        m = engine.m
        dev = m.flat_parameters().device
        self.eng = engine
        side, engine.use_side_stream = engine.use_side_stream, bool(side_stream)
        self.x = torch.zeros(batch, m.feat_dim, frames, device=dev)
        self.y = torch.zeros(batch, dtype=torch.long, device=dev)
        self.shape = (batch, m.feat_dim, frames)
        saved_buffers = [b.clone() for b in m.buffers()]
        s = torch.cuda.Stream()
        s.wait_stream(torch.cuda.current_stream())
        with torch.cuda.stream(s):
            for _ in range(warmup):
                for p in m.parameters():
                    p.grad = None
                engine.loss_and_grad(self.x, self.y)
        torch.cuda.current_stream().wait_stream(s)
        torch.cuda.synchronize()
        for b, sb in zip(m.buffers(), saved_buffers):
            b.copy_(sb)
        for p in m.parameters():
            p.grad = None
        engine.dirty = True
        self.segments = []
        cap = {"g": None, "ctx": None}

        def begin():
            g = torch.cuda.CUDAGraph()
            kw = {"pool": self.segments[0][0].pool()} if self.segments else ({"pool": pool} if pool is not None else {})
            ctx = torch.cuda.graph(g, capture_error_mode="thread_local", **kw)
            ctx.__enter__()
            cap["g"], cap["ctx"] = g, ctx

        def end(name):
            cap["ctx"].__exit__(None, None, None)
            self.segments.append((cap["g"], name))
            cap["g"] = cap["ctx"] = None

        def cut(name):
            end(name)
            if name != STAGE_ORDER[-1]:
                begin()

        begin()
        try:
            self.loss, self.logits, self.rank = engine.loss_and_grad(self.x, self.y, cut if segmented else None)
            if cap["ctx"] is not None:
                end(None)
        except BaseException:
            if cap["ctx"] is not None:
                cap["ctx"].__exit__(None, None, None)
            raise
        self.graph = self.segments[0][0]
        assert [n for _, n in self.segments] == (STAGE_ORDER if segmented else [None])
        self.pack_table = engine._pack_tables.get(True)
        assert self.pack_table is not None and self.pack_table.launches_captured >= 1, \
            "the captured training step does not contain the conv-weight re-pack"
        engine.dirty = True
        engine.use_side_stream = side

    def matches(self, x):
        return tuple(x.shape) == self.shape

    def pool(self):
        return self.segments[0][0].pool()

    def __call__(self, x, y, on_stage_done=None):
        self.x.copy_(x, non_blocking=True)
        self.y.copy_(y, non_blocking=True)
        for g, name in self.segments:
            g.replay()
            if name is not None and on_stage_done is not None:
                on_stage_done(name)
        self.eng.dirty, self.eng._packed_for_bwd = False, True
        self.eng.m.attach_grads()
        return self.loss, self.logits, self.rank


class GraphedStepCache:

    def __init__(self, engine, segmented=False, max_graphs=64, warmup=2):
        self.eng, self.segmented, self.max_graphs, self.warmup = engine, segmented, max_graphs, warmup
        self.steps = {}
        self._pool_owner = None
        self.captures = 0

    def get(self, batch, frames):
        key = (int(batch), int(frames))
        st = self.steps.pop(key, None)
        if st is None:
            pool = self._pool_owner.pool() if self._pool_owner is not None else None
            st = GraphedTrainStep(self.eng, key[0], key[1], warmup=self.warmup, segmented=self.segmented, pool=pool)
            if self._pool_owner is None:
                self._pool_owner = st
            self.captures += 1
            while len(self.steps) >= self.max_graphs:
                old = next(iter(self.steps))
                if self.steps[old] is self._pool_owner:
                    self.steps[old] = self.steps.pop(old)
                    if len(self.steps) == 1:
                        break
                    continue
                del self.steps[old]
        self.steps[key] = st
        return st

    def __call__(self, x, y, on_stage_done=None):
        return self.get(x.shape[0], x.shape[2])(x, y, on_stage_done)

    def __len__(self):
        return len(self.steps)
```

pytorch-kaldi-resnet_amd/hip.py:

```python
import ctypes
import os

import torch

_HERE = os.path.dirname(os.path.abspath(__file__))
LIB_PATH = os.environ.get("SPK_LIB", os.path.join(_HERE, "libspkhip.so"))

IN_AFFINE_RELU, EPI_AFFINE, EPI_ADD, EPI_RELU, EPI_STATS, EPI_BNBWD, IN_BNBWD, CONV_WS = 1, 2, 4, 8, 16, 32, 64, 128
CONV_PIPE = 1024
WGRAD_GROUPS = 2048
IN_PRESPLIT, SIDE_PRESPLIT, DY_PRESPLIT = 1 << 14, 1 << 15, 1 << 16
CONV_M16 = 1 << 17
WGRAD_NOSHIFT = 1 << 18
WGRAD_M16 = 1 << 19
EPI_WMASK = 1 << 24
MASK_NONE, MASK_ACT, MASK_RAW, MASK_BITS = 0, 1, 2, 3

_P = ctypes.c_void_p
_I = ctypes.c_int
_L = ctypes.c_longlong
_F = ctypes.c_float
_D = ctypes.c_double
_IP = ctypes.POINTER(ctypes.c_int)

_SIGS = {
    "spk_pack_conv_weight": [_P, _P, _I, _I, _I, _I, _I, _P],
    "spk_pack_conv_weight_split": [_P, _P, _I, _I, _I, _I, _I, _I, _P],
    "spk_pack_job_bytes": [],
    "spk_build_flags": [],
    "spk_pack_conv_weights_batched": [_P, _I, _I, _I, _P],
    "spk_conv_mfma": [_P] * 21 + [_I] * 14 + [_IP, _IP, _IP] + [_I] * 8 + [_P, _P, _P, _P],
    "spk_conv_mfma_len": [_P] * 21 + [_I] * 14 + [_IP, _IP, _IP] + [_I] * 8 + [_P, _P, _P, _P, _P],
    "spk_conv3x3_c32_stream": [_P] * 6 + [_I] * 4 + [_P, _P, _I, _P],
    "spk_conv1x1_stream": [_P] * 11 + [_L, _I, _I, _P, _P, _I, _P],
    "spk_conv1x1_stream_rows": [_I, _I],
    "spk_conv_wgrad": [_P] * 6 + [_I] * 16 + [_P, _P, _P],
    "spk_conv_wgrad_limits": [_I, _IP, _IP],
    "spk_wgrad_reduce": [_P, _P, _I, _I, _I, _I, _I, _P],
    "spk_stem_fwd_blocks": [_I, _I, _I],
    "spk_stem_conv_fwd": [_P] * 6 + [_I] * 4 + [_P, _P],
    "spk_stem_conv_fwd_len": [_P] * 6 + [_I] * 4 + [_P, _P, _P],
    "spk_stem_wgrad_blocks": [_I, _I, _I],
    "spk_stem_conv_wgrad": [_P] * 4 + [_I] * 4 + [_P],
    "spk_bn_stats_blocks": [_L, _I],
    "spk_bn_stats_partial": [_P, _P, _L, _I, _P],
    "spk_bn_finalize": [_P, _I, _I, _D] + [_P] * 9 + [_F, _F, _P, _P, _P, _P],
    "spk_bn_eval_coeffs": [_P] * 6 + [_I, _F, _P],
    "spk_bn_apply": [_P] * 8 + [_L, _I, _I, _P, _P],
    "spk_bn_bwd_reduce": [_P] * 8 + [_L, _I, _I, _P, _P],
    "spk_bn_bwd_finalize": [_P, _I, _I, _D] + [_P] * 5 + [_I, _P, _P, _P, _P, _P, _P, _P],
    "spk_bn_bwd_apply": [_P] * 10 + [_L, _I, _I, _P, _P, _P],
    "spk_absmax": [_P, _P, _L, _P],
    "spk_bnbwd_estimate": [_P, _P, _P, _I, _P, _P, _P, _P],
    "spk_f16_window_count": [_P, _P, _P, _L, _I, _P, _I, _P, _P],
    "spk_affine_estimate": [_P, _P, _I, _P, _P, _P],
    "spk_stats_pool_fwd": [_P, _P, _I, _I, _I, _I, _I, _P],
    "spk_stats_pool_fwd_len": [_P, _P, _P, _I, _I, _I, _I, _I, _P],
    "spk_stats_pool_bwd": [_P, _P, _P, _I, _I, _I, _I, _I, _P, _P],
    "spk_gemm_f32": [_P] * 4 + [_I] * 3 + [_L] * 5 + [_F, _I, _P, _P],
    "spk_gemm_splitk": [_I, _I, _I],
    "spk_colsum": [_P, _P, _I, _I, _I, _P],
    "spk_l2norm_fwd": [_P, _P, _P, _I, _I, _F, _P],
    "spk_l2norm_bwd": [_P, _P, _P, _P, _I, _I, _F, _I, _P],
    "spk_aam_margin_fwd": [_P, _P, _P, _I, _I, _F, _F, _P],
    "spk_aam_margin_bwd": [_P, _P, _P, _P, _I, _I, _F, _F, _P],
    "spk_softmax_ce": [_P] * 5 + [_I, _I, _F, _P],
    "spk_mean": [_P, _P, _I, _P],
    "spk_relu_bwd": [_P, _P, _P, _L, _P],
    "spk_sgd_step": [_P, _P, _P, _L, _F, _F, _F, _F, _I, _P],
    "spk_center_normalize": [_P, _P, _P, _I, _I, _F, _P],
    "spk_trial_cosine": [_P, _P, _P, _P, _P, _I, _I, _I, _I, _P],
    "spk_topk_mean_std": [_P, _P, _P, _I, _I, _I, _L, _P],
    "spk_fbank_tile_frames": [_I, _I, _I, _I],
    "spk_fbank_fwd": [_P, _P, _P, _I, _L] + [_P] * 5 + [_I] * 5 + [_F, _F, _I, _F, ctypes.c_ulonglong, _P, _P, _P, _I, _P],
    "spk_fbank_dither_noise": [_P, _L, ctypes.c_ulonglong, _I, _I, _I, _P],
    "spk_vad_count": [_P, _P, _I, _I, _D, _D, _I, _D, _P, _P, _P, _P],
    "spk_cmn_select": [_P] * 6 + [_I] * 5 + [_P],
    "spk_resample_tile": [_I, _I, _I],
    "spk_resample_fwd": [_P, _P, _I, _L, _P, _P, _I, _I, _I, _P, _P, _L, _P],
    "spk_augment_max_rir": [],
    "spk_augment_max_early": [],
    "spk_augment_workspace": [_I, _L, _I, _I, _L, _I, ctypes.POINTER(_L)],
    "spk_cm_decode": [_P, _P, _P, _I, _I, _I, _P, _P],
    "spk_cm_compress": [_P, _P, _I, _I, _I, _P, _P, _P, _P, _P],
    "spk_augment_fwd": [_P, _P, _I, _L, _P, _L, _P, _P, _I, _I, _P, _L, _P, _P, _P, _P, _I, _L, _P, _P, _P, _P, _I, _P, _P, _P],
}

_lib = None


def lib():
    global _lib
    if _lib is None:
        if not os.path.exists(LIB_PATH) and "SPK_LIB" not in os.environ:
            try:
                import importlib.util
                spec = importlib.util.spec_from_file_location("spk_build", os.path.join(_HERE, "build.py"))
                mod = importlib.util.module_from_spec(spec)
                spec.loader.exec_module(mod)
                mod.build(force=True, verbose=False)
            except Exception as e:
                raise RuntimeError("libspkhip.so is missing at %s and building it failed (%s). Run `python "
                                   "__graft_entry__.py build` (hipcc --offload-arch=gfx950). There is no fallback path."
                                   % (LIB_PATH, e))
        if not os.path.exists(LIB_PATH):
            raise RuntimeError(
                "libspkhip.so is missing at %s: run `python __graft_entry__.py build` "
                "(hipcc --offload-arch=gfx950). There is no fallback path." % LIB_PATH)
        l = ctypes.CDLL(LIB_PATH)
        l.spk_last_error.restype = ctypes.c_char_p
        l.spk_version.restype = ctypes.c_int
        l.spk_conv_wgrad_workspace.restype = ctypes.c_size_t
        l.spk_conv_wgrad_workspace.argtypes = [_I, _I, _I, _I]
        l.spk_bn_finalize_workspace.restype = ctypes.c_size_t
        l.spk_bn_finalize_workspace.argtypes = [_I, _I]
        l.spk_gemm_workspace.restype = ctypes.c_size_t
        l.spk_gemm_workspace.argtypes = [_I, _I, _I]
        for name, sig in _SIGS.items():
            fn = getattr(l, name)
            fn.argtypes = sig
            fn.restype = ctypes.c_int
        _lib = l
    return _lib


def has_experimental():
    return bool(lib().spk_build_flags() & 1)


def exported_symbols():
    return ["spk_version", "spk_last_error", "spk_conv_wgrad_workspace", "spk_bn_finalize_workspace", "spk_gemm_workspace"] + list(_SIGS)


def ptr(t):
    if t is None:
        return None
    assert t.is_cuda, "libspkhip takes device tensors only"
    assert t.is_contiguous(), "libspkhip takes contiguous tensors only"
    return t.data_ptr()


def stream():
    return torch.cuda.current_stream().cuda_stream


def check(rc, name):
    if rc != 0:
        msg = lib().spk_last_error().decode()
        raise RuntimeError("%s failed (rc=%d): %s" % (name, rc, msg))


def call(name, *args):
    rc = getattr(lib(), name)(*args)
    check(rc, name)
```

pytorch-kaldi-resnet_amd/ops.py:

```python
import ctypes
import os

import torch

from . import hip, tiling
from .hip import (CONV_M16, CONV_PIPE, CONV_WS, DY_PRESPLIT, IN_PRESPLIT, SIDE_PRESPLIT, WGRAD_GROUPS, EPI_ADD, EPI_AFFINE, EPI_BNBWD, EPI_RELU,
                  EPI_STATS, EPI_WMASK, IN_AFFINE_RELU, IN_BNBWD, MASK_ACT, MASK_NONE, MASK_RAW,
                  call, ptr, stream)

BN_EPS = 1e-5
BN_MOMENTUM = 0.1

PROFILE = None
_raw_call = call


def call(name, *args, label=None, flops=0.0, nbytes=0.0):
    if PROFILE is None:
        return _raw_call(name, *args)
    e0 = torch.cuda.Event(enable_timing=True)
    e1 = torch.cuda.Event(enable_timing=True)
    e0.record()
    _raw_call(name, *args)
    e1.record()
    PROFILE.append((label or name, flops, e0, e1, nbytes))


def _iarr(v):
    return (ctypes.c_int * len(v))(*v)


class AmaxPool:

    def __init__(self, device, n=4096):
        self.table = torch.zeros(n, device=device, dtype=torch.int32)
        self.next = 0

    def take_n(self, n):
        i = self.next
        assert i + n <= self.table.numel(), "AmaxPool exhausted"
        self.next = i + n
        return self.table[i:i + n]

    def reset(self):
        self.table.zero_()
        self.next = 0

    def take(self):
        i = self.next
        assert i < self.table.numel(), "AmaxPool exhausted"
        self.next = i + 1
        return self.table[i:i + 1]


def absmax_into(t, slot):
    call("spk_absmax", ptr(t), ptr(slot), t.numel(), stream())
    return slot


def affine_estimate(scale, shift, amax_in, est):
    call("spk_affine_estimate", ptr(scale), ptr(shift), scale.numel(), ptr(amax_in), ptr(est), stream())
    return est


def _amax_fwd_fallback(x, in_affine):
    slot = absmax_into(x, torch.zeros(1, device=x.device, dtype=torch.int32))
    if in_affine is None:
        return slot
    return affine_estimate(in_affine[0], in_affine[1], slot, torch.zeros(1, device=x.device, dtype=torch.int32))


def bnbwd_estimate(coef, bn4, amax_in, raw_amax, est=None):
    if est is None:
        est = torch.zeros(1, device=coef.device, dtype=torch.int32)
    call("spk_bnbwd_estimate", ptr(coef), ptr(bn4[0]), ptr(bn4[1]), coef.shape[1], ptr(amax_in), ptr(raw_amax), ptr(est), stream())
    return est


def _amax_fallback(dy, in_bnbwd):
    slot = torch.zeros(1, device=dy.device, dtype=torch.int32)
    absmax_into(dy, slot)
    if in_bnbwd is None:
        return slot
    raw_slot = absmax_into(in_bnbwd[0], torch.zeros(1, device=dy.device, dtype=torch.int32))
    return bnbwd_estimate(in_bnbwd[3], in_bnbwd[2], slot, raw_slot)


def f16_window_count(x, slot, counts, affine=None, pairs=False):
    C = x.shape[-1]
    call("spk_f16_window_count", ptr(x), ptr(affine[0]) if affine else None, ptr(affine[1]) if affine else None, x.numel(), C,
         ptr(slot), 1 if pairs else 0, ptr(counts), stream())
    return counts


def conv_out_hw(h, w, ksize, stride):
    pad = 1 if ksize == 3 else 0
    return (h + 2 * pad - ksize) // stride + 1, (w + 2 * pad - ksize) // stride + 1


MFMA_MODES = {"f32": 0, "bf16x6": 6, "bf16x9": 9, "f16x3": 3}
SPLIT = MFMA_MODES[os.environ.get("SPK_MFMA", "f16x3")]
SPLIT_BWD = MFMA_MODES[os.environ["SPK_MFMA_BWD"]] if os.environ.get("SPK_MFMA_BWD") else None


WS_CONV = os.environ.get("SPK_CONV_WS", "auto")
assert WS_CONV in ("0", "1", "auto"), "SPK_CONV_WS must be 0, 1 or auto"
WS_AUTO_MIN_COUT = 128
PIPE_CONV = os.environ.get("SPK_CONV_PIPE", "1") == "1"
PIPE_M16 = os.environ.get("SPK_PIPE_M16", "1") == "1"
PIPE_WGRAD = os.environ.get("SPK_WGRAD_PIPE", "0") == "1"
PIPE_BNBWD = os.environ.get("SPK_PIPE_BNBWD", "0") == "1"
GROUPED_1X1 = os.environ.get("SPK_WGRAD_1X1_GROUPS", "1") == "1"
WM16 = os.environ.get("SPK_WM16", "1") == "1"
C32M16 = os.environ.get("SPK_C32M16", "1") == "1"
WM_SHIFT = os.environ.get("SPK_WM_SHIFT", "1") == "1"
GROUPED_3X3 = os.environ.get("SPK_WGRAD_3X3_GROUPS", "1") == "1"
GROUPED_1X1_BLOCKS = int(os.environ.get("SPK_WGRAD_1X1_BLOCKS", "512"))
PIPE_MIN_CIN = int(os.environ.get("SPK_PIPE_MIN_CIN", "64"))
PIPE_MAX_LDS = int(os.environ.get("SPK_PIPE_MAX_LDS", str(80 * 1024)))
WS_WGRAD = os.environ.get("SPK_WGRAD_WS", "0") == "1"
WS_WGRAD_BLOCKS = int(os.environ.get("SPK_WGRAD_WS_BLOCKS", "256"))
WS_MIN_TAPS = int(os.environ.get("SPK_WS_MIN_TAPS", "9"))
LABEL_SHAPES = os.environ.get("SPK_LABEL_SHAPES", "0") == "1"
WS_FORCE = None


def _experimental():
    return hip.has_experimental()


SPLIT_1X1 = os.environ.get("SPK_SPLIT_1X1", "1") == "1"
KC_CANDIDATES = tuple(int(v) for v in os.environ.get("SPK_KC", "4,2").split(","))


def split_for(ksize, bwd=False):
    mode = SPLIT_BWD if (bwd and SPLIT_BWD is not None) else SPLIT
    if ksize == 3:
        return mode
    return 3 if (mode == 3 and SPLIT_1X1 and ksize == 1) else 0


def pack_conv_weight(w, transpose=False, out=None):
    Cout, Cin, KH, KW = w.shape
    split = split_for(KH, bwd=transpose)
    n = packed_numel(w, bwd=transpose)
    if out is None or out.numel() != n:
        out = torch.empty(n, device=w.device, dtype=torch.float32)
    if split:
        call("spk_pack_conv_weight_split", ptr(w), ptr(out), Cout, Cin, KH, KW, 1 if transpose else 0, split, stream(),
             label="spk_pack_conv_weight")
    else:
        call("spk_pack_conv_weight", ptr(w), ptr(out), Cout, Cin, KH, KW, 1 if transpose else 0, stream(),
             label="spk_pack_conv_weight")
    return out


def packed_numel(w, bwd=False):
    sp = split_for(w.shape[2], bwd)
    return w.numel() * 3 // 2 if sp in (6, 9) else (w.numel() + 4 if sp == 3 else w.numel())


class PackTable:

    def __init__(self, jobs, device):
        import struct
        assert hip.lib().spk_pack_job_bytes() == 48
        blob, block0 = b"", 0
        self.key = []
        for w, wpk, transpose in jobs:
            Cout, Cin, KH, KW = w.shape
            split = split_for(KH, bwd=transpose)
            assert wpk.numel() == packed_numel(w, bwd=transpose) and w.is_contiguous()
            blob += struct.pack("<QQ8i", w.data_ptr(), wpk.data_ptr(), Cout, Cin, KH * KW, 1 if transpose else 0, split,
                                w.numel(), block0, 0)
            block0 += (w.numel() + 255) // 256
            self.key.append((w.data_ptr(), wpk.data_ptr(), transpose, split))
        self.njobs, self.blocks = len(jobs), block0
        self.has_f16 = any(k[3] == 3 for k in self.key)
        self.table = torch.frombuffer(bytearray(blob), dtype=torch.uint8).to(device)
        self.launches = 0
        self.launches_captured = 0

    def run(self):
        self.launches += 1
        if torch.cuda.is_current_stream_capturing():
            self.launches_captured += 1
        call("spk_pack_conv_weights_batched", ptr(self.table), self.njobs, self.blocks, 1 if self.has_f16 else 0, stream(),
             label="spk_pack_conv_weight")


STREAM_1X1 = os.environ.get("SPK_STREAM_1X1", "1") == "1"
STREAM_1X1_BLOCKS = int(os.environ.get("SPK_STREAM_1X1_BLOCKS", "512"))


def _conv1x1_stream(x, wpk, out, in_affine, epi_add, add_mask, bn_bwd, want_stats, in_amax, out_amax, in_presplit):
    B, H, W, C = x.shape
    P = B * H * W
    tp = 64 * (1 if C >= 128 else (2 if C == 64 else 4))
    nblocks = max(1, min(STREAM_1X1_BLOCKS, -(-P // tp)))
    flags = 0
    if in_affine is not None:
        flags |= IN_AFFINE_RELU
    if in_presplit:
        assert in_affine is None
        flags |= IN_PRESPLIT
    if epi_add is not None:
        assert epi_add.shape == out.shape
        flags |= EPI_ADD
    bn_mask = bn_bwd[3] if (bn_bwd is not None and len(bn_bwd) > 3) else None
    for mk in (bn_mask, add_mask):
        if mk is not None:
            assert mk.dtype == torch.int32 and mk.numel() == out.numel() // 32, "sign mask shape"
    stats = None
    if bn_bwd is not None:
        want_stats = True
        flags |= EPI_BNBWD
        assert bn_bwd[0].shape == out.shape
    if want_stats:
        flags |= EPI_STATS
        stats = torch.empty(hip.lib().spk_conv1x1_stream_rows(nblocks, C), C, 2, device=x.device, dtype=torch.float32)
    call("spk_conv1x1_stream", ptr(x), ptr(wpk), ptr(out), ptr(in_affine[0]) if in_affine else None,
         ptr(in_affine[1]) if in_affine else None, ptr(epi_add), ptr(add_mask), ptr(bn_bwd[0]) if bn_bwd else None, ptr(bn_mask),
         ptr(bn_bwd[2]) if bn_bwd else None, ptr(stats), P, C, flags, ptr(in_amax), ptr(out_amax), nblocks, stream(),
         label="conv1x1_stream_kernel<%d>" % C + (" C%d %dx%d" % (C, H, W) if LABEL_SHAPES else ""),
         flops=2.0 * P * C * C,
         nbytes=4.0 * (P * C * (2 + (1 if epi_add is not None else 0) + (1 if bn_bwd is not None else 0))
                       + (P * C / 32) * ((bn_mask is not None) + (add_mask is not None)) + wpk.numel()))
    return stats


STREAM_C32 = os.environ.get("SPK_STREAM_C32", "1") == "1"
STREAM_C32_BLOCKS = int(os.environ.get("SPK_STREAM_C32_BLOCKS", "512"))


def _conv3x3_c32_stream(x, wpk, out, in_affine, in_amax, out_amax):
    B, H, W, _ = x.shape
    ntiles = B * (-(-H // 8)) * (-(-W // 16))
    nblocks = max(1, min(STREAM_C32_BLOCKS, ntiles))
    stats = torch.empty(4 * nblocks, 32, 2, device=x.device, dtype=torch.float32)
    flags = EPI_STATS | (IN_AFFINE_RELU if in_affine is not None else 0)
    call("spk_conv3x3_c32_stream", ptr(x), ptr(wpk), ptr(out), ptr(in_affine[0]) if in_affine else None,
         ptr(in_affine[1]) if in_affine else None, ptr(stats), B, H, W, flags, ptr(in_amax), ptr(out_amax), nblocks, stream(),
         label="conv3x3_c32_stream_kernel" + (" C32 %dx%d" % (H, W) if LABEL_SHAPES else ""),
         flops=2.0 * B * H * W * 32 * 32 * 9, nbytes=4.0 * (2 * B * H * W * 32 + wpk.numel()))
    return stats


def _conv_launch(x, wpk, out, Cout, taps, IS, OS, ooy, oox, OH, OW, in_affine, epi_affine, epi_add, relu, want_stats,
                 bn_bwd=None, in_bnbwd=None, side=None, split=0, add_mask=None, in_amax=None, out_amax=None, side_amax=None,
                 in_presplit=False, side_presplit=False, wlen=None):
    B, IH, IW, Cin = x.shape
    OHf, OWf = out.shape[1], out.shape[2]
    if wlen is not None:
        _check_wlen(wlen, B)
    if (STREAM_C32 and wlen is None and split == 3 and Cin == 32 and Cout == 32 and IS == 1 and OS == 1 and ooy == 0 and oox == 0
            and (IH, IW) == (OH, OW) == (OHf, OWf) and want_stats and in_bnbwd is None and side is None and epi_affine is None
            and epi_add is None and not relu and bn_bwd is None and not in_presplit and not side_presplit and add_mask is None
            and list(taps) == [(kh - 1, kw - 1, kh * 3 + kw) for kh in range(3) for kw in range(3)] and B * OH * OW * 32 < 2 ** 31 - 65536):
        return _conv3x3_c32_stream(x, wpk, out, in_affine, in_amax, out_amax)
    if (STREAM_1X1 and wlen is None and split == 3 and len(taps) == 1 and taps[0][0] == 0 and taps[0][1] == 0 and IS == 1 and OS == 1 and ooy == 0
            and oox == 0 and Cin == Cout and Cin in (32, 64, 128) and (IH, IW) == (OH, OW) == (OHf, OWf) and in_bnbwd is None
            and side is None and epi_affine is None and not relu and not side_presplit and out is not x
            and (bn_bwd is None or bn_bwd[1] is None or len(bn_bwd) > 3) and B * OH * OW * Cin < 2 ** 31):
        return _conv1x1_stream(x, wpk, out, in_affine, epi_add, add_mask, bn_bwd, want_stats, in_amax, out_amax, in_presplit)
    dys = [t[0] for t in taps]
    dxs = [t[1] for t in taps]
    tws = [t[2] for t in taps]
    ips = 1
    if len(taps) == 1 and IS > 1 and dys[0] == 0 and dxs[0] == 0:
        ips, IS = IS, 1
    key = (OH, OW, IS, max(dys) - min(dys) + 1, max(dxs) - min(dxs) + 1, len(taps), Cout)
    if tiling.AUTOTUNE and key not in (tiling.FORCE_CONV_SPLIT if split else tiling.FORCE_CONV) and PROFILE is None and not torch.cuda.is_current_stream_capturing():
        _autotune_conv(key, x, wpk, out, Cout, taps, IS, OS, ooy, oox, OH, OW, in_affine, epi_affine, epi_add, relu, split,
                       in_amax=in_amax, in_presplit=in_presplit)
    TH, TW, MT, NT = tiling.conv_tile(*key, mode=1 if in_bnbwd is not None else 0, split=split)
    ws, WC = None, 1
    pipe_fused = (PIPE_CONV and PIPE_BNBWD and split == 3 and in_bnbwd is not None and len(in_bnbwd) > 4 and MT * NT <= 4
                  and Cout <= 128 and WS_FORCE is None and WS_CONV != "1" and not side_presplit)
    ws_on = (WS_CONV == "1" or WS_FORCE is not None or (
        WS_CONV == "auto" and _experimental() and split == 3 and in_bnbwd is not None and Cout >= WS_AUTO_MIN_COUT
        and not pipe_fused))
    if side_presplit or in_presplit:
        ws_on = False
    if split and ws_on and len(taps) >= WS_MIN_TAPS and ips == 1:
        ws = WS_FORCE or tiling.ws_tile(*key)
    if ws is not None:
        TH, TW, MT, NT, WC = ws
    kc = 1
    if len(taps) == 1:
        halo = ((TH - 1) * IS + 1) * ((TW - 1) * IS + 1)
        for cand in KC_CANDIDATES:
            if Cin % (32 * cand) == 0 and cand * halo * tiling.LDS_PIX_BYTES <= tiling.LDS_HARD:
                kc = cand
                break
    flags = 0
    halo9 = ((TH - 1) * IS + key[3]) * ((TW - 1) * IS + key[4])
    bnbwd_ok = in_bnbwd is None or pipe_fused
    pipe = (PIPE_CONV and ws is None and split == 3 and len(taps) == 9 and kc == 1 and bnbwd_ok and halo9 <= 576
            and (2 * halo9 + 1) * 80 <= PIPE_MAX_LDS and Cin >= PIPE_MIN_CIN)
    if pipe:
        flags |= CONV_PIPE
    m16 = pipe and PIPE_M16 and in_bnbwd is None and (MT, NT) == (3, 2) and halo9 <= 512 and IS == 1
    if m16:
        flags |= CONV_M16
    if ws is not None:
        flags |= CONV_WS | ({1: 0, 2: 1, 4: 2}[WC] << 8)
    if in_affine is not None:
        flags |= IN_AFFINE_RELU
    if in_presplit:
        assert split == 3 and in_affine is None and in_bnbwd is None, "f16 pair input: f16x3 mode, plain input"
        flags |= IN_PRESPLIT
    if side_presplit:
        assert split == 3 and in_bnbwd is not None, "f16 pair side output: fused BatchNorm-backward data gradient in the f16x3 mode"
        flags |= SIDE_PRESPLIT
    if epi_affine is not None:
        flags |= EPI_AFFINE
    if epi_add is not None:
        flags |= EPI_ADD
        assert epi_add.shape == out.shape
    if relu:
        flags |= EPI_RELU
    in_mask = in_bnbwd[4] if (in_bnbwd is not None and len(in_bnbwd) > 4) else None
    bn_mask = bn_bwd[3] if (bn_bwd is not None and len(bn_bwd) > 3) else None
    for mk, ref in ((in_mask, x), (bn_mask, out), (add_mask, out)):
        if mk is not None:
            assert mk.dtype == torch.int32 and mk.numel() == ref.numel() // 32, "sign mask shape"
    if in_bnbwd is not None:
        flags |= IN_BNBWD
        assert in_affine is None and side is not None and side[0].shape == x.shape
        assert in_bnbwd[0].shape == x.shape and (in_bnbwd[1] is None or in_bnbwd[1].shape == x.shape)
    stats = None
    if bn_bwd is not None:
        want_stats = True
        flags |= EPI_BNBWD
        assert bn_bwd[0].shape == out.shape and (bn_bwd[1] is None or bn_bwd[1].shape == out.shape)
    if wlen is not None:
        flags |= EPI_WMASK
    if want_stats:
        flags |= EPI_STATS
        ntile = (4 // WC) * B * (-(-OH // TH)) * (-(-OW // TW))
        stats = torch.empty(ntile, Cout, 2, device=x.device, dtype=torch.float32)
    call("spk_conv_mfma" if wlen is None else "spk_conv_mfma_len", ptr(x), ptr(wpk), ptr(out),
         ptr(in_affine[0]) if in_affine else None, ptr(in_affine[1]) if in_affine else None,
         ptr(epi_affine[0]) if epi_affine else None, ptr(epi_affine[1]) if epi_affine else None,
         ptr(epi_add),
         ptr(in_bnbwd[0]) if in_bnbwd else None, ptr(in_bnbwd[1]) if (in_bnbwd and in_mask is None) else None,
         ptr(in_bnbwd[2]) if in_bnbwd else None, ptr(in_bnbwd[3]) if in_bnbwd else None,
         ptr(in_mask), ptr(bn_mask), ptr(add_mask),
         ptr(side[0]) if side else None, ptr(side[1]) if side else None,
         ptr(bn_bwd[0]) if bn_bwd else None, ptr(bn_bwd[1]) if (bn_bwd and bn_mask is None) else None,
         ptr(bn_bwd[2]) if bn_bwd else None, ptr(stats), B, IH, IW, Cin, OH, OW, OHf, OWf, Cout, IS, OS, ooy, oox, len(taps),
         _iarr(dys), _iarr(dxs), _iarr(tws), TH, TW, MT, NT, kc, ips, flags, split, ptr(in_amax), ptr(out_amax), ptr(side_amax),
         *(() if wlen is None else (ptr(wlen),)), stream(),
         label=(("conv_ws_kernel<%d,%d,%d,%s,%d>" % (MT, NT, WC, "true" if in_bnbwd is not None else "false", split)) if ws is not None
                else ("conv_pipe_kernel<%d,%d,false,false%s>" % (MT, NT, (",true,true" if in_presplit else ",false,true") if m16 else (",true" if in_presplit else "")) if in_bnbwd is None
                      else "conv_pipe_kernel<%d,%d,true,true>" % (MT, NT)) if pipe
                else "conv_mfma_kernel<%d,%d,%s,%d>" % (MT, NT, "true" if in_bnbwd is not None else "false", split)) + (
             " C%d %dx%d" % (Cout, OH, OW) if LABEL_SHAPES else ""),
         flops=2.0 * B * OH * OW * Cout * Cin * len(taps),
         nbytes=4.0 * (B * (IH // ips) * (IW // ips) * Cin * (min(1.0, len(taps) * OH * OW / max(1, (IH // ips) * (IW // ips))) if IS == 1 and OS > 1 else 1.0)
                       + B * OH * OW * Cout * (1 + (1 if epi_add is not None else 0) + (1 if bn_bwd is not None else 0))
                       + (2 * x.numel() if in_bnbwd is not None else 0)
                       + (x.numel() / 32 if in_mask is not None else 0) + (B * OH * OW * Cout / 32) * ((bn_mask is not None) + (add_mask is not None))
                       + wpk.numel()))
    return stats


def _check_wlen(wlen, B):
    if not (wlen.is_cuda and wlen.dtype == torch.int32 and wlen.dim() == 1 and wlen.numel() == B and wlen.is_contiguous()):
        raise RuntimeError("wlen must be a contiguous int32 device tensor [%d], got %s %s %s" % (B, wlen.dtype, tuple(wlen.shape), wlen.device))


def _time_launch(fn, reps=2):
    fn()
    e0, e1 = torch.cuda.Event(enable_timing=True), torch.cuda.Event(enable_timing=True)
    e0.record()
    for _ in range(reps):
        fn()
    e1.record()
    e1.synchronize()
    return e0.elapsed_time(e1) / reps


def _autotune_conv(key, x, wpk, out, Cout, taps, IS, OS, ooy, oox, OH, OW, in_affine, epi_affine, epi_add, relu, split=0,
                   in_amax=None, in_presplit=False):
    scratch = torch.empty_like(out)
    if split == 3 and in_amax is None:
        in_amax = _amax_fwd_fallback(x, in_affine)
    add = epi_add if (epi_add is None or epi_add.data_ptr() != out.data_ptr()) else scratch
    best = None
    table = tiling.FORCE_CONV_SPLIT if split else tiling.FORCE_CONV
    for cand in tiling.conv_candidates(*key, split=split):
        table[key] = cand
        try:
            ms = _time_launch(lambda: _conv_launch(x, wpk, scratch, Cout, taps, IS, OS, ooy, oox, OH, OW, in_affine,
                                                   epi_affine, add, relu, True, split=split, in_amax=in_amax,
                                                   in_presplit=in_presplit))
        except RuntimeError:
            continue
        if best is None or ms < best[0]:
            best = (ms, cand)
    if best is None:
        del table[key]
    else:
        table[key] = best[1]


def _autotune_wgrad(key, x, dy, ksize, stride, in_affine, dy_amax=None, x_amax=None, dy_presplit=False):
    scratch = torch.empty(dy.shape[3], x.shape[3], ksize, ksize, device=x.device, dtype=torch.float32)
    best = None
    for cand in tiling.wgrad_candidates(*key):
        tiling.FORCE_WGRAD[key] = cand
        try:
            ms = _time_launch(lambda: conv_wgrad(x, dy, scratch, ksize, stride, in_affine=in_affine, dy_amax=dy_amax,
                                                 x_amax=x_amax, dy_presplit=dy_presplit))
        except RuntimeError:
            continue
        if best is None or ms < best[0]:
            best = (ms, cand)
    if best is None:
        del tiling.FORCE_WGRAD[key]
    else:
        tiling.FORCE_WGRAD[key] = best[1]


def conv_fwd(x, wpk, Cout, ksize, stride, in_affine=None, epi_affine=None, epi_add=None, relu=False, stats=False,
             out=None, in_amax=None, out_amax=None, wlen=None):
    B, IH, IW, Cin = x.shape
    if split_for(ksize) == 3 and in_amax is None:
        in_amax = _amax_fwd_fallback(x, in_affine)
    OH, OW = conv_out_hw(IH, IW, ksize, stride)
    if out is None:
        out = torch.empty(B, OH, OW, Cout, device=x.device, dtype=torch.float32)
    if ksize == 3:
        taps = [(kh - 1, kw - 1, kh * 3 + kw) for kh in range(3) for kw in range(3)]
    else:
        taps = [(0, 0, 0)]
    st = _conv_launch(x, wpk, out, Cout, taps, stride, 1, 0, 0, OH, OW, in_affine, epi_affine, epi_add, relu, stats,
                      split=split_for(ksize), in_amax=in_amax, out_amax=out_amax, wlen=wlen)
    return out, st


def conv_dgrad(dy, wpk_t, Cin, ksize, stride, in_hw, add=None, out=None, accumulate=False, bn_bwd=None, in_bnbwd=None,
               side=None, add_mask=None, in_amax=None, out_amax=None, side_amax=None, in_presplit=False, side_presplit=False):
    B, OH, OW, Cout = dy.shape
    assert not in_presplit or in_amax is not None, "an f16 pair tensor comes with its scale slot"
    if split_for(ksize, True) == 3 and in_amax is None:
        in_amax = _amax_fallback(dy, in_bnbwd)
    IH, IW = in_hw
    if out is None:
        assert not accumulate
        out = torch.empty(B, IH, IW, Cin, device=dy.device, dtype=torch.float32)
    if accumulate:
        assert add is None
        add = out
    if stride == 1:
        if ksize == 3:
            taps = [(1 - kh, 1 - kw, kh * 3 + kw) for kh in range(3) for kw in range(3)]
        else:
            taps = [(0, 0, 0)]
        st = _conv_launch(dy, wpk_t, out, Cin, taps, 1, 1, 0, 0, IH, IW, None, None, add, False, False, bn_bwd, in_bnbwd,
                          side, split=split_for(ksize, True), add_mask=add_mask, in_amax=in_amax, out_amax=out_amax,
                          side_amax=side_amax, in_presplit=in_presplit, side_presplit=side_presplit)
        return (out, st) if bn_bwd is not None else out
    assert stride == 2 and bn_bwd is None and in_bnbwd is None and add_mask is None
    if ksize == 1:
        if not accumulate:
            if add is not None:
                out.copy_(add)
            else:
                out.zero_()
        _conv_launch(dy, wpk_t, out, Cin, [(0, 0, 0)], 1, 2, 0, 0, (IH + 1) // 2, (IW + 1) // 2, None, None, out, False,
                     False, split=split_for(1, True), in_amax=in_amax, out_amax=out_amax, in_presplit=in_presplit)
        return out
    for cy in range(2):
        for cx in range(2):
            LH, LW = (IH - cy + 1) // 2, (IW - cx + 1) // 2
            if LH <= 0 or LW <= 0:
                continue
            taps = []
            for kh in range(3):
                if (cy + 1 - kh) % 2:
                    continue
                for kw in range(3):
                    if (cx + 1 - kw) % 2:
                        continue
                    taps.append(((cy + 1 - kh) // 2, (cx + 1 - kw) // 2, kh * 3 + kw))
            _conv_launch(dy, wpk_t, out, Cin, taps, 1, 2, cy, cx, LH, LW, None, None, add, False, False, split=split_for(3, True),
                         in_amax=in_amax, out_amax=out_amax, in_presplit=in_presplit)
    return out


_ws_cache = {}
_ws_retired = []


def _workspace(nbytes, device):
    key = (str(device), torch.cuda.current_stream().cuda_stream)
    w = _ws_cache.get(key)
    if w is None or w.numel() * 4 < nbytes:
        if w is not None:
            _ws_retired.append(w)
        w = torch.empty((nbytes + 3) // 4, device=device, dtype=torch.float32)
        _ws_cache[key] = w
    return w


def _workspace_named(name, nbytes, device):
    key = (name, str(device), torch.cuda.current_stream().cuda_stream)
    w = _ws_cache.get(key)
    if w is None or w.numel() * 4 < nbytes:
        if w is not None:
            _ws_retired.append(w)
        w = torch.empty((nbytes + 3) // 4, device=device, dtype=torch.float32)
        _ws_cache[key] = w
    return w


def conv_wgrad(x, dy, dw, ksize, stride, in_affine=None, accumulate=False, dy_amax=None, x_amax=None, dy_presplit=False):
    B, IH, IW, Cin = x.shape
    _, OH, OW, Cout = dy.shape
    split = split_for(ksize, True)
    assert not dy_presplit or (split == 3 and dy_amax is not None), "an f16 pair tensor comes with its scale slot (f16x3 mode)"
    if split == 3 and dy_amax is None:
        dy_amax = absmax_into(dy, torch.zeros(1, device=dy.device, dtype=torch.int32))
    if split == 3 and x_amax is None:
        x_amax = _amax_fwd_fallback(x, in_affine)
    wkey = (OH, OW, Cin, Cout, ksize, stride)
    if tiling.AUTOTUNE and wkey not in tiling.FORCE_WGRAD and PROFILE is None and not torch.cuda.is_current_stream_capturing():
        tiling.FORCE_WGRAD[wkey] = tiling._wgrad_tile(*wkey)
        _autotune_wgrad(wkey, x, dy, ksize, stride, in_affine, dy_amax, x_amax, dy_presplit)
    TH, TW, WN = tiling.wgrad_tile(OH, OW, Cin, Cout, ksize, stride, split=split)
    if C32M16 and split == 3 and ksize == 3 and WN == 1 and dy_presplit:
        TH, TW, WN = tiling.c32m16_tile(OH, OW, Cin, Cout, ksize, stride) or (TH, TW, WN)
    nreg = B * (-(-OH // TH)) * (-(-OW // TW))
    halo = ((TH - 1) * stride + ksize) * ((TW - 1) * stride + ksize)
    wgws = (WS_WGRAD and split == 3 and ksize == 3 and not dy_presplit
            and 2 * (halo * 192 + -(-(TH * TW) // 16) * 16 * (WN * 192 + (64 if WN > 1 else 0))) <= 160 * 1024)
    nst = -(-(TH * TW) // 16)
    wgp = (PIPE_WGRAD and not wgws and not dy_presplit and split == 3 and ksize == 3 and nst % (4 // WN) == 0 and nst // (4 // WN) in (1, 2)
           and 2 * (2 * halo * 64 + 2 * WN * -(-(TH * TW) // 16) * 16 * 64) + 128 <= PIPE_MAX_LDS)
    cg = 0
    if GROUPED_1X1 and split == 3 and ksize == 1 and WN in (2, 4) and TH * TW <= 64:
        cg = 4 if Cin % 128 == 0 else (2 if Cin % 64 == 0 else 0)
        if cg and -(-(TH * TW) // 16) * 16 * (cg * 192 + WN * 192 + 64) > 80 * 1024:
            cg = 2 if cg == 4 else 0
    wm = (GROUPED_3X3 and not wgws and not wgp and split == 3 and ksize == 3 and WN == 2 and Cin % 64 == 0 and Cout % 64 == 0
          and halo <= 112 and TH * TW <= 64 and halo * 384 + -(-(TH * TW) // 16) * 16 * 448 <= 80 * 1024)
    wm16 = wm and WM16 and dy_presplit and halo * 416 + 2 * -(-(TH * TW) // 32) * 32 * 256 <= 80 * 1024
    c32m16 = (C32M16 and not wm and not wgws and not wgp and split == 3 and ksize == 3 and WN == 1 and dy_presplit and halo <= 192
              and halo * 192 + 2 * -(-(TH * TW) // 32) * 32 * 128 <= 80 * 1024)
    if wm:
        cg = 2
    nsplit = min(nreg, tiling.wgrad_nsplit(nreg, Cin, Cout, WN, WS_WGRAD_BLOCKS if wgws else (GROUPED_1X1_BLOCKS if cg else None),
                                           cin_groups=cg or 1))
    nslab = nsplit
    nbytes = hip.lib().spk_conv_wgrad_workspace(nslab, ksize, Cin, Cout)
    ws = _workspace(nbytes, x.device)
    flags = (IN_AFFINE_RELU if in_affine is not None else 0) | (CONV_WS if wgws else 0) | (CONV_PIPE if wgp else 0)
    if cg:
        flags |= WGRAD_GROUPS | ({2: 1, 4: 2}[cg] << 12)
    if dy_presplit:
        flags |= DY_PRESPLIT
    if wm and not WM_SHIFT:
        flags |= hip.WGRAD_NOSHIFT
    if wm16 or c32m16:
        flags |= hip.WGRAD_M16
    call("spk_conv_wgrad", ptr(x), ptr(dy), ptr(dw), ptr(ws),
         ptr(in_affine[0]) if in_affine else None, ptr(in_affine[1]) if in_affine else None,
         B, IH, IW, Cin, OH, OW, Cout, ksize, stride, TH, TW, WN, nsplit, flags, 1 if accumulate else 0, split,
         ptr(dy_amax) if split == 3 else None, ptr(x_amax) if split == 3 else None, stream(),
         label=("conv_wgrad_wm16_kernel" if wm16 else "conv_wgrad_c32m16_kernel" if c32m16 else "conv_wgrad_wm_kernel" if wm
         else ("conv_wgrad_1x1_kernel<%d,%d,%d>" % (4 // WN, WN, cg)) if cg
         else ("conv_wgrad_ws_kernel<%d,%d,%d,%d>" % (ksize * ksize, 4 // WN, WN, 4 if halo <= 128 else 5)) if wgws
         else ("conv_wgrad_pipe_kernel<%d,%d,%d,%d>" % (4 // WN, WN, 4 if halo <= 128 else 5, nst // (4 // WN))) if wgp
         else ("conv_wgrad_split_kernel<%d,%d,%d,%d,%d>" % (
             ksize * ksize, 4 // WN, WN, split, 4 if ((TH - 1) * stride + ksize) * ((TW - 1) * stride + ksize) <= 128 else 5)) if split
         else "conv_wgrad_kernel<%d,%d,%d>" % (ksize * ksize, 4 // WN, WN)) + (
             " C%d %dx%d" % (Cout, OH, OW) if LABEL_SHAPES else ""),
         flops=2.0 * B * OH * OW * Cout * Cin * ksize * ksize, nbytes=4.0 * (x.numel() + dy.numel() + nbytes / 4))
    call("spk_wgrad_reduce", ptr(ws), ptr(dw), nslab, ksize, Cin, Cout, 1 if accumulate else 0, stream())
    return dw


def stem_fwd(x, w, epi_affine=None, relu=False, stats=False, amax_out=None, wlen=None):
    B, F, T = x.shape
    out = torch.empty(B, F, T, 32, device=x.device, dtype=torch.float32)
    flags = (EPI_AFFINE if epi_affine is not None else 0) | (EPI_RELU if relu else 0) | (EPI_STATS if stats else 0)
    st = None
    if stats:
        st = torch.empty(hip.lib().spk_stem_fwd_blocks(B, F, T), 32, 2, device=x.device, dtype=torch.float32)
    args = (ptr(x), ptr(w), ptr(out), ptr(st), ptr(epi_affine[0]) if epi_affine else None,
            ptr(epi_affine[1]) if epi_affine else None, B, F, T)
    if wlen is None:
        call("spk_stem_conv_fwd", *args, flags, ptr(amax_out), stream())
    else:
        _check_wlen(wlen, B)
        call("spk_stem_conv_fwd_len", *args, flags | EPI_WMASK, ptr(amax_out), ptr(wlen), stream())
    return out, st


def stem_wgrad(x, draw, dw, accumulate=False):
    B, F, T = x.shape
    nblk = hip.lib().spk_stem_wgrad_blocks(B, F, T)
    ws = _workspace(nblk * 288 * 4, x.device)
    call("spk_stem_conv_wgrad", ptr(x), ptr(draw), ptr(dw), ptr(ws), B, F, T, 1 if accumulate else 0, stream())
    return dw


def bn_stats_partial(x2d):
    N, C = x2d.shape
    nblk = hip.lib().spk_bn_stats_blocks(N, C)
    part = torch.empty(nblk, C, 2, device=x2d.device, dtype=torch.float32)
    call("spk_bn_stats_partial", ptr(x2d), ptr(part), N, C, stream())
    return part


_ws64_cache = {}


def _ws64(device):
    w = _ws64_cache.get(str(device))
    if w is None:
        w = torch.zeros(256 * 2048 * 2 + 64, device=device, dtype=torch.float64)
        _ws64_cache[str(device)] = w
    return w


def bn_finalize(partial, count, gamma, beta, running_mean, running_var, nbt, out4, amax_in=None, est_out=None):
    C = gamma.numel()
    call("spk_bn_finalize", ptr(partial), partial.shape[0], C, float(count), ptr(gamma), ptr(beta), ptr(running_mean),
         ptr(running_var), ptr(nbt), ptr(out4[0]), ptr(out4[1]), ptr(out4[2]), ptr(out4[3]), BN_MOMENTUM, BN_EPS,
         ptr(_ws64(partial.device)), ptr(amax_in), ptr(est_out), stream())


def bn_eval_coeffs(gamma, beta, rm, rv, out2):
    C = gamma.numel()
    call("spk_bn_eval_coeffs", ptr(gamma), ptr(beta), ptr(rm), ptr(rv), ptr(out2[0]), ptr(out2[1]), C, BN_EPS, stream())


def bn_apply(raw, scale, shift, res=None, res_affine=None, relu=True, out=None, mask=False, amax_out=None):
    C = raw.shape[-1]
    N = raw.numel() // C
    if out is None:
        out = torch.empty_like(raw)
    mk = torch.empty(N * (C // 32), device=raw.device, dtype=torch.int32) if mask else None
    call("spk_bn_apply", ptr(raw), ptr(scale), ptr(shift), ptr(res),
         ptr(res_affine[0]) if res_affine else None, ptr(res_affine[1]) if res_affine else None, ptr(out), ptr(mk), N, C,
         1 if relu else 0, ptr(amax_out), stream(),
         nbytes=4.0 * raw.numel() * (2 + (1 if res is not None else 0)) + (raw.numel() / 8 if mask else 0))
    return (out, mk) if mask else out


def _bn_bwd_bytes(raw, mask_mode, passes):
    n = raw.numel()
    return 4.0 * n * passes + {MASK_NONE: 0.0, MASK_RAW: 0.0, MASK_ACT: 4.0 * n}.get(mask_mode, n / 8.0)


def bn_backward(dy, raw, act, bn4, gamma, dgamma, dbeta, mask_mode, draw_out=None, dz_out=None, accumulate=False,
                partial=None, amax_out=None, pair=None, chan_amax=None):
    C = raw.shape[-1]
    N = raw.numel() // C
    coef = torch.empty(3, C, device=raw.device, dtype=torch.float32)
    if partial is None:
        nblk = hip.lib().spk_bn_stats_blocks(N, C)
        part = torch.empty(nblk, C, 2, device=raw.device, dtype=torch.float32)
        call("spk_bn_bwd_reduce", ptr(dy), ptr(raw), ptr(act), ptr(bn4[0]), ptr(bn4[1]), ptr(bn4[2]), ptr(bn4[3]), ptr(part),
             N, C, mask_mode, ptr(chan_amax), stream(), nbytes=_bn_bwd_bytes(raw, mask_mode, 2))
    else:
        assert chan_amax is None, "chan_amax comes out of the reduction pass: partial must be None"
        part, nblk = partial, partial.shape[0]
    call("spk_bn_bwd_finalize", ptr(part), nblk, C, float(N), ptr(gamma), ptr(bn4[1]), ptr(dgamma), ptr(dbeta), ptr(coef),
         1 if accumulate else 0, ptr(_ws64(raw.device)), ptr(pair[0]) if pair else None, ptr(pair[1]) if pair else None,
         ptr(bn4[0]) if pair else None, ptr(pair[2]) if pair else None, ptr(chan_amax) if pair else None, stream())
    if draw_out is None:
        draw_out = torch.empty_like(raw)
    call("spk_bn_bwd_apply", ptr(dy), ptr(raw), ptr(act), ptr(bn4[0]), ptr(bn4[1]), ptr(bn4[2]), ptr(bn4[3]), ptr(coef),
         ptr(draw_out), ptr(dz_out), N, C, mask_mode, ptr(amax_out), ptr(pair[2]) if pair else None, stream(),
         nbytes=_bn_bwd_bytes(raw, mask_mode, 3 + (1 if dz_out is not None else 0)))
    return draw_out


def bn_bwd_coef(partial, count, gamma, bn4, dgamma, dbeta, accumulate=False, amax_in=None, raw_amax=None, est_out=None,
                chan_amax=None):
    C = gamma.numel()
    coef = torch.empty(3, C, device=gamma.device, dtype=torch.float32)
    assert est_out is None or (amax_in is not None and raw_amax is not None)
    call("spk_bn_bwd_finalize", ptr(partial), partial.shape[0], C, float(count), ptr(gamma), ptr(bn4[1]), ptr(dgamma),
         ptr(dbeta), ptr(coef), 1 if accumulate else 0, ptr(_ws64(gamma.device)), ptr(amax_in) if est_out is not None else None,
         ptr(raw_amax) if est_out is not None else None, ptr(bn4[0]) if est_out is not None else None, ptr(est_out),
         ptr(chan_amax) if est_out is not None else None, stream())
    return coef


def bn_bwd_partial(dy, raw, act, bn4, mask_mode, chan_amax=None):
    C = raw.shape[-1]
    N = raw.numel() // C
    nblk = hip.lib().spk_bn_stats_blocks(N, C)
    part = torch.empty(nblk, C, 2, device=raw.device, dtype=torch.float32)
    call("spk_bn_bwd_reduce", ptr(dy), ptr(raw), ptr(act), ptr(bn4[0]), ptr(bn4[1]), ptr(bn4[2]), ptr(bn4[3]), ptr(part),
         N, C, mask_mode, ptr(chan_amax), stream(), nbytes=_bn_bwd_bytes(raw, mask_mode, 2))
    return part


def stats_pool_fwd(x, mode, wlen=None):
    B, H, W, C = x.shape
    out = torch.empty(B, C * H * (2 if mode else 1), device=x.device, dtype=torch.float32)
    if wlen is None:
        call("spk_stats_pool_fwd", ptr(x), ptr(out), B, H, W, C, mode, stream())
    else:
        _check_wlen(wlen, B)
        call("spk_stats_pool_fwd_len", ptr(x), ptr(out), ptr(wlen), B, H, W, C, mode, stream())
    return out


def stats_pool_bwd(x, gout, mode, amax_out=None):
    B, H, W, C = x.shape
    dx = torch.empty_like(x)
    call("spk_stats_pool_bwd", ptr(x), ptr(gout), ptr(dx), B, H, W, C, mode, ptr(amax_out), stream())
    return dx


def _ptr_rows(t):
    assert t.is_cuda and t.dim() == 2 and (t.stride(1) == 1 or t.shape[1] == 1) and t.stride(0) >= t.shape[1], \
        "libspkhip takes rows of unit stride only"
    return t.data_ptr()


def gemm(A, Bm, M, N, K, sam, sak, sbk, sbn, bias=None, out=None, alpha=1.0, accumulate=False):
    if out is None:
        out = torch.empty(M, N, device=A.device, dtype=torch.float32)
    ws = _workspace_named("gemm", hip.lib().spk_gemm_workspace(M, N, K), A.device)
    call("spk_gemm_f32", ptr(A), ptr(Bm), _ptr_rows(out), ptr(bias), M, N, K, sam, sak, sbk, sbn, out.stride(0), float(alpha),
         1 if accumulate else 0, ptr(ws), stream(), label="gemm_f32_kernel", flops=2.0 * M * N * K)
    return out


def linear_fwd(x, w, bias=None):
    M, K = x.shape
    N = w.shape[0]
    return gemm(x, w, M, N, K, K, 1, 1, K, bias=bias)


def linear_bwd(x, w, dy, dw, db=None, need_dx=True, accumulate=False):
    M, K = x.shape
    N = w.shape[0]
    dx = None
    if need_dx:
        dx = gemm(dy, w, M, K, N, N, 1, K, 1)
    gemm(dy, x, N, K, M, 1, N, K, 1, out=dw, accumulate=accumulate)
    if db is not None:
        call("spk_colsum", ptr(dy), ptr(db), M, N, 1 if accumulate else 0, stream())
    return dx


def l2norm_fwd(x):
    R, D = x.shape
    y = torch.empty_like(x)
    inv = torch.empty(R, device=x.device, dtype=torch.float32)
    call("spk_l2norm_fwd", ptr(x), ptr(y), ptr(inv), R, D, 1e-12, stream())
    return y, inv


def l2norm_bwd(y, inv, dy, out=None, accumulate=False):
    R, D = y.shape
    if out is None:
        out = torch.empty_like(y)
    call("spk_l2norm_bwd", ptr(y), ptr(inv), ptr(dy), ptr(out), R, D, 1e-12, 1 if accumulate else 0, stream())
    return out


def aam_margin_fwd(cosv, label, m, s):
    B, S = cosv.shape
    logits = torch.empty_like(cosv)
    call("spk_aam_margin_fwd", ptr(cosv), ptr(label), ptr(logits), B, S, float(m), float(s), stream())
    return logits


def aam_margin_bwd(cosv, label, dlogits, m, s):
    B, S = cosv.shape
    dcos = torch.empty_like(cosv)
    call("spk_aam_margin_bwd", ptr(cosv), ptr(label), ptr(dlogits), ptr(dcos), B, S, float(m), float(s), stream())
    return dcos


def softmax_ce(logits, label, grad_scale=None, want_rank=True):
    B, S = logits.shape
    loss_row = torch.empty(B, device=logits.device, dtype=torch.float32)
    dl = torch.empty_like(logits) if grad_scale is not None else None
    rank = torch.empty(B, device=logits.device, dtype=torch.int32) if want_rank else None
    call("spk_softmax_ce", ptr(logits), ptr(label), ptr(loss_row), ptr(dl), ptr(rank), B, S,
         float(grad_scale if grad_scale is not None else 0.0), stream())
    return loss_row, dl, rank


def mean(v):
    out = torch.empty(1, device=v.device, dtype=torch.float32)
    call("spk_mean", ptr(v), ptr(out), v.numel(), stream())
    return out


def relu_bwd(y, dy):
    dx = torch.empty_like(dy)
    call("spk_relu_bwd", ptr(y), ptr(dy), ptr(dx), y.numel(), stream())
    return dx


def sgd_step(p, g, buf, lr, momentum, weight_decay, grad_scale, first):
    call("spk_sgd_step", ptr(p), ptr(g), ptr(buf), p.numel(), float(lr), float(momentum), float(weight_decay),
         float(grad_scale), 1 if first else 0, stream())


def center_normalize(emb, mean=None, eps=1e-8):
    N, D = emb.shape
    out = torch.empty_like(emb)
    call("spk_center_normalize", ptr(emb), ptr(mean), ptr(out), N, D, float(eps), stream())
    return out


def trial_cosine(en, te, ia, ib):
    T = ia.numel()
    out = torch.empty(T, device=en.device, dtype=torch.float32)
    assert ia.dtype == torch.int32 and ib.dtype == torch.int32 and ib.numel() == T and en.shape[1] == te.shape[1]
    call("spk_trial_cosine", ptr(en), ptr(te), ptr(ia), ptr(ib), ptr(out), T, en.shape[1], en.shape[0], te.shape[0], stream())
    return out


def topk_mean_std(scores, k):
    N, M = scores.shape
    mean = torch.empty(N, device=scores.device, dtype=torch.float32)
    std = torch.empty_like(mean)
    call("spk_topk_mean_std", _ptr_rows(scores), ptr(mean), ptr(std), N, M, int(k), scores.stride(0), stream())
    return mean, std
```

Baseline: 5447 utt/s.

## Defer stem BN-ReLU into consumers and fuse stem BN backward into wgrad

```diff
diff --git a/include/spkhip.h b/include/spkhip.h
--- a/include/spkhip.h
+++ b/include/spkhip.h
@@ -78,9 +78,14 @@
 int spk_stem_conv_fwd_len(const float* x, const float* w, float* out, float* stats, const float* epi_scale,
                           const float* epi_shift, int B, int F, int T, int flags, unsigned* amax_out, const int* len ,
                           void* stream);
+int spk_stem_fwd_minmax(const float* x, const float* w, float* out, float* stats, float* minmax, int B, int F, int T, int flags,
+                        unsigned* amax_out, void* stream);
 int spk_stem_wgrad_blocks(int B, int F, int T);
 int spk_stem_conv_wgrad(const float* x, const float* draw, float* dw, float* partial, int B, int F, int T,
                         int accumulate, void* stream);
+int spk_stem_bn_wgrad(const float* x, const float* d, const float* raw0, const float* mean, const float* invstd,
+                      const float* scale, const float* shift, const float* coef, float* dw, float* partial, int B, int F, int T,
+                      int accumulate, void* stream);
 
 int spk_bn_stats_blocks(long long N, int C);
 int spk_bn_stats_partial(const float* x, float* partial , long long N, int C, void* stream);
@@ -113,6 +118,8 @@
 int spk_f16_window_count(const float* x, const float* scale, const float* shift, long long n, int C, const unsigned* slot,
                          int pairs, unsigned long long* counts , void* stream);
 int spk_affine_estimate(const float* scale, const float* shift, int C, const unsigned* amax_in, unsigned* est, void* stream);
+int spk_affine_relu_amax(const float* minmax, int nblk, int C, const float* scale, const float* shift, unsigned* amax_out,
+                         void* stream);
 
 int spk_stats_pool_fwd(const float* x , float* out , int B, int H, int W, int C,
                        int mode, void* stream);
diff --git a/pytorch-kaldi-resnet_amd/csrc/bn.hip b/pytorch-kaldi-resnet_amd/csrc/bn.hip
--- a/pytorch-kaldi-resnet_amd/csrc/bn.hip
+++ b/pytorch-kaldi-resnet_amd/csrc/bn.hip
@@ -234,23 +234,6 @@
     if (nb > 2147483647LL) nb = 2147483647LL;
     return (int)(nb < 1 ? 1 : nb);
 }
-#ifndef BN_NT
-#define BN_NT 1
-#endif
-static __device__ __forceinline__ f32x4 ld_stream(const float* p) {
-#if BN_NT
-    return __builtin_nontemporal_load((const f32x4*)p);
-#else
-    return *(const f32x4*)p;
-#endif
-}
-static __device__ __forceinline__ void st_stream(float* p, f32x4 v) {
-#if BN_NT
-    __builtin_nontemporal_store(v, (f32x4*)p);
-#else
-    *(f32x4*)p = v;
-#endif
-}
 __global__ __launch_bounds__(256) void bn_apply_kernel(const float* __restrict__ raw, const float* __restrict__ scale,
                                                        const float* __restrict__ shift, const float* __restrict__ res,
                                                        const float* __restrict__ rscale, const float* __restrict__ rshift,
@@ -294,9 +277,15 @@
             if (res) {
                 f32x4 r = sv[u];
                 if (rscale) r = r * prs + prh;
+                if (relu & 2) {
+                    r[0] = fmaxf(r[0], 0.f);
+                    r[1] = fmaxf(r[1], 0.f);
+                    r[2] = fmaxf(r[2], 0.f);
+                    r[3] = fmaxf(r[3], 0.f);
+                }
                 v += r;
             }
-            if (relu) {
+            if (relu & 1) {
                 v[0] = fmaxf(v[0], 0.f);
                 v[1] = fmaxf(v[1], 0.f);
                 v[2] = fmaxf(v[2], 0.f);
@@ -324,6 +313,7 @@
     SPK_REQUIRE(N > 0 && bn_c_ok(C), "spk_bn_apply: N=%lld C=%d", N, C);
     SPK_REQUIRE((res_scale == nullptr) == (res_shift == nullptr), "spk_bn_apply: residual affine must come in pairs");
     SPK_REQUIRE(!res_scale || res, "spk_bn_apply: residual affine without residual");
+    SPK_REQUIRE(relu >= 0 && relu <= 3 && (!(relu & 2) || res_scale), "spk_bn_apply: relu=%d (bit 1, ReLU on the residual term, needs the residual affine)", relu);
     SPK_REQUIRE(!mask_out || C % 32 == 0, "spk_bn_apply: the sign mask needs C %% 32 == 0 (C=%d)", C);
     const long long nquads = N * C / 4;
     hipLaunchKernelGGL(bn_apply_kernel, dim3(stream_grid(nquads, BN_APPLY_U, BN_APPLY_CAP)), dim3(256), 0, (hipStream_t)stream, raw, scale, shift, res,
@@ -662,6 +652,52 @@
     return 0;
 }
 
+__global__ __launch_bounds__(256) void affine_relu_amax_kernel(const float* __restrict__ minmax, int nblk, int C,
+                                                               const float* __restrict__ scale, const float* __restrict__ shift,
+                                                               unsigned* __restrict__ amax_out) {
+    __shared__ f32x4 smx[256], smn[256];
+    const int tid = threadIdx.x, nq = C / 4, q = tid % nq, rs = 256 / nq;
+    const float inf = __builtin_inff();
+    f32x4 mx = {-inf, -inf, -inf, -inf}, mn = {inf, inf, inf, inf};
+    for (int r = tid / nq; r < nblk; r += rs) {
+        const float* p = minmax + (size_t)r * 2 * C + q * 4;
+        const f32x4 a = *(const f32x4*)p, b = *(const f32x4*)(p + C);
+#pragma unroll
+        for (int k = 0; k < 4; ++k) {
+            mx[k] = fmaxf(mx[k], a[k]);
+            mn[k] = fminf(mn[k], b[k]);
+        }
+    }
+    smx[tid] = mx;
+    smn[tid] = mn;
+    __syncthreads();
+    float best = 0.f;
+    if (tid < nq) {
+        for (int j = 1; j < rs; ++j) {
+            const f32x4 a = smx[tid + j * nq], b = smn[tid + j * nq];
+#pragma unroll
+            for (int k = 0; k < 4; ++k) {
+                mx[k] = fmaxf(mx[k], a[k]);
+                mn[k] = fminf(mn[k], b[k]);
+            }
+        }
+        const f32x4 sc = *(const f32x4*)(scale + tid * 4), sh = *(const f32x4*)(shift + tid * 4);
+        const f32x4 hi = mx * sc + sh, lo = mn * sc + sh;
+#pragma unroll
+        for (int k = 0; k < 4; ++k) best = fmaxf(best, fmaxf(fmaxf(hi[k], 0.f), fmaxf(lo[k], 0.f)));
+    }
+    spk_wave_amax_commit(best, amax_out);
+}
+
+extern "C" int spk_affine_relu_amax(const float* minmax, int nblk, int C, const float* scale, const float* shift,
+                                    unsigned* amax_out, void* stream) {
+    SPK_REQUIRE(minmax && scale && shift && amax_out, "spk_affine_relu_amax: null pointer");
+    SPK_REQUIRE(nblk > 0 && C >= 4 && C <= 1024 && (C & (C - 1)) == 0, "spk_affine_relu_amax: nblk=%d C=%d", nblk, C);
+    hipLaunchKernelGGL(affine_relu_amax_kernel, dim3(1), dim3(256), 0, (hipStream_t)stream, minmax, nblk, C, scale, shift, amax_out);
+    SPK_LAUNCH_CHECK("spk_affine_relu_amax");
+    return 0;
+}
+
 extern "C" int spk_bnbwd_estimate(const float* coef, const float* mean, const float* invstd, int C, const unsigned* amax_in,
                                   const unsigned* raw_amax, unsigned* est, void* stream) {
     SPK_REQUIRE(coef && mean && invstd && amax_in && raw_amax && est && C > 0, "spk_bnbwd_estimate: bad arguments");
diff --git a/pytorch-kaldi-resnet_amd/csrc/conv_split.hip b/pytorch-kaldi-resnet_amd/csrc/conv_split.hip
--- a/pytorch-kaldi-resnet_amd/csrc/conv_split.hip
+++ b/pytorch-kaldi-resnet_amd/csrc/conv_split.hip
@@ -8,8 +8,10 @@
             const int var = a.flags | (a.add_mask ? SPK_FL_ADDMASK : 0) | (a.bn_mask ? SPK_FL_BNMASK : 0) | (a.in_mask ? SPK_FL_INMASK : 0);
             constexpr int V2 = SPK_IN_BNBWD | SPK_SIDE_PRESPLIT | SPK_EPI_STATS | SPK_EPI_BNBWD | SPK_FL_INMASK;
             constexpr int V1 = SPK_IN_BNBWD | SPK_SIDE_PRESPLIT | SPK_EPI_ADD | SPK_EPI_STATS | SPK_EPI_BNBWD | SPK_FL_ADDMASK | SPK_FL_BNMASK;
-            if (!a.in_act && !a.bn_act && !a.side_dz && (var == V1 || var == V2)) {
-                if (var == V2) hipLaunchKernelGGL((conv_mfma_kernel<MT, NT, true, SPLIT, V2>), dim3(a.nblocks), dim3(256), lds_bytes, st, a);
+            constexpr int V0 = V1 & ~SPK_FL_BNMASK;
+            if (!a.in_act && !a.bn_act && !a.side_dz && (var == V0 || var == V1 || var == V2)) {
+                if (var == V0) hipLaunchKernelGGL((conv_mfma_kernel<MT, NT, true, SPLIT, V0>), dim3(a.nblocks), dim3(256), lds_bytes, st, a);
+                else if (var == V2) hipLaunchKernelGGL((conv_mfma_kernel<MT, NT, true, SPLIT, V2>), dim3(a.nblocks), dim3(256), lds_bytes, st, a);
                 else hipLaunchKernelGGL((conv_mfma_kernel<MT, NT, true, SPLIT, V1>), dim3(a.nblocks), dim3(256), lds_bytes, st, a);
                 SPK_LAUNCH_CHECK("spk_conv_mfma(split)");
                 return 0;
diff --git a/pytorch-kaldi-resnet_amd/csrc/spk_common.h b/pytorch-kaldi-resnet_amd/csrc/spk_common.h
--- a/pytorch-kaldi-resnet_amd/csrc/spk_common.h
+++ b/pytorch-kaldi-resnet_amd/csrc/spk_common.h
@@ -4,6 +4,24 @@
 
 typedef float f32x4 __attribute__((ext_vector_type(4)));
 typedef float f32x16 __attribute__((ext_vector_type(16)));
+
+#ifndef BN_NT
+#define BN_NT 1
+#endif
+static __device__ __forceinline__ f32x4 ld_stream(const float* p) {
+#if BN_NT
+    return __builtin_nontemporal_load((const f32x4*)p);
+#else
+    return *(const f32x4*)p;
+#endif
+}
+static __device__ __forceinline__ void st_stream(float* p, f32x4 v) {
+#if BN_NT
+    __builtin_nontemporal_store(v, (f32x4*)p);
+#else
+    *(f32x4*)p = v;
+#endif
+}
 
 void spk_set_error(const char* fmt, ...);
 #define SPK_REQUIRE(cond, ...)                 \
diff --git a/pytorch-kaldi-resnet_amd/csrc/stem.hip b/pytorch-kaldi-resnet_amd/csrc/stem.hip
--- a/pytorch-kaldi-resnet_amd/csrc/stem.hip
+++ b/pytorch-kaldi-resnet_amd/csrc/stem.hip
@@ -2,14 +2,21 @@
 
 #define STEM_C 32
 
-template <bool LEN>
+template <bool LEN, bool MM = false>
 __global__ __launch_bounds__(256) void stem_fwd_kernel(const float* __restrict__ x, const float* __restrict__ w,
                                                        float* __restrict__ out, float* __restrict__ stats,
                                                        const float* __restrict__ epi_scale,
                                                        const float* __restrict__ epi_shift, int B, int F, int T,
-                                                       int flags, unsigned* __restrict__ amax_out, const int* __restrict__ len) {
+                                                       int flags, unsigned* __restrict__ amax_out, const int* __restrict__ len,
+                                                       float* __restrict__ minmax = nullptr) {
     __shared__ float red[4][STEM_C][2];
     float mx = 0.f;
+    float cmx[8], cmn[8];
+#pragma unroll
+    for (int c = 0; c < 8; ++c) {
+        cmx[c] = -__builtin_inff();
+        cmn[c] = __builtin_inff();
+    }
     const int tid = threadIdx.x, cg = tid & 3, pl = tid >> 2;
     float wr[9][8];
 #pragma unroll
@@ -54,6 +61,10 @@
             mx = fmaxf(mx, fabsf(v));
             ssum[c] += v;
             ssq[c] += v * v;
+            if constexpr (MM) {
+                cmx[c] = fmaxf(cmx[c], v);
+                cmn[c] = fminf(cmn[c], v);
+            }
         }
         f32x4* dst = (f32x4*)(out + (size_t)p * STEM_C + cg * 8);
         dst[0] = (f32x4){o[0], o[1], o[2], o[3]};
@@ -87,6 +98,32 @@
             }
             stats[((size_t)blockIdx.x * STEM_C + tid) * 2 + 0] = s0;
             stats[((size_t)blockIdx.x * STEM_C + tid) * 2 + 1] = s1;
+        }
+    }
+    if constexpr (MM) {
+        __shared__ float redm[4][2][STEM_C];
+#pragma unroll
+        for (int c = 0; c < 8; ++c) {
+#pragma unroll
+            for (int off = 4; off < 64; off <<= 1) {
+                cmx[c] = fmaxf(cmx[c], __shfl_xor(cmx[c], off, 64));
+                cmn[c] = fminf(cmn[c], __shfl_xor(cmn[c], off, 64));
+            }
+        }
+        const int lane = tid & 63, wave = tid >> 6;
+        if (lane < 4) {
+#pragma unroll
+            for (int c = 0; c < 8; ++c) {
+                redm[wave][0][lane * 8 + c] = cmx[c];
+                redm[wave][1][lane * 8 + c] = cmn[c];
+            }
+        }
+        __syncthreads();
+        if (tid < STEM_C) {
+            minmax[((size_t)blockIdx.x * 2 + 0) * STEM_C + tid] =
+                fmaxf(fmaxf(redm[0][0][tid], redm[1][0][tid]), fmaxf(redm[2][0][tid], redm[3][0][tid]));
+            minmax[((size_t)blockIdx.x * 2 + 1) * STEM_C + tid] =
+                fminf(fminf(redm[0][1][tid], redm[1][1][tid]), fminf(redm[2][1][tid], redm[3][1][tid]));
         }
     }
 }
@@ -107,6 +144,18 @@
     hipLaunchKernelGGL(stem_fwd_kernel<false>, dim3(spk_stem_fwd_blocks(B, F, T)), dim3(256), 0, (hipStream_t)stream, x, w, out,
                        stats, epi_scale, epi_shift, B, F, T, flags, amax_out, nullptr);
     SPK_LAUNCH_CHECK("spk_stem_conv_fwd");
+    return 0;
+}
+
+extern "C" int spk_stem_fwd_minmax(const float* x, const float* w, float* out, float* stats, float* minmax, int B, int F, int T,
+                                   int flags, unsigned* amax_out, void* stream) {
+    SPK_REQUIRE(x && w && out && minmax, "spk_stem_fwd_minmax: null pointer");
+    SPK_REQUIRE(B > 0 && F > 0 && T > 0, "spk_stem_fwd_minmax: empty input");
+    SPK_REQUIRE(!(flags & SPK_EPI_STATS) || stats, "spk_stem_fwd_minmax: EPI_STATS needs a stats buffer");
+    SPK_REQUIRE(!(flags & ~SPK_EPI_STATS), "spk_stem_fwd_minmax: flags=%#x (only SPK_EPI_STATS)", flags);
+    hipLaunchKernelGGL((stem_fwd_kernel<false, true>), dim3(spk_stem_fwd_blocks(B, F, T)), dim3(256), 0, (hipStream_t)stream, x, w,
+                       out, stats, nullptr, nullptr, B, F, T, flags, amax_out, nullptr, minmax);
+    SPK_LAUNCH_CHECK("spk_stem_fwd_minmax");
     return 0;
 }
 
@@ -171,6 +220,98 @@
         partial[(size_t)blockIdx.x * (STEM_C * 9) + i] = (red[0][i] + red[1][i]) + (red[2][i] + red[3][i]);
 }
 
+#ifndef STEM_BW_U
+#define STEM_BW_U 2
+#endif
+
+__global__ __launch_bounds__(256) void stem_bn_wgrad_kernel(const float* __restrict__ x, const float* __restrict__ dy,
+                                                            const float* __restrict__ raw, const float* __restrict__ mean,
+                                                            const float* __restrict__ invstd, const float* __restrict__ scale,
+                                                            const float* __restrict__ shift, const float* __restrict__ coef,
+                                                            float* __restrict__ partial, int B, int F, int T) {
+    __shared__ float red[4][STEM_C * 9];
+    constexpr int U = STEM_BW_U;
+    const int tid = threadIdx.x, cg = tid & 3, pl = tid >> 2;
+    float acc[9][8];
+#pragma unroll
+    for (int t = 0; t < 9; ++t)
+#pragma unroll
+        for (int c = 0; c < 8; ++c) acc[t][c] = 0.f;
+    f32x4 pmu[2], pis[2], psc[2], psh[2], pk1[2], pm1[2], pm2[2];
+#pragma unroll
+    for (int h = 0; h < 2; ++h) {
+        const int c0 = cg * 8 + h * 4;
+        pmu[h] = *(const f32x4*)(mean + c0);
+        pis[h] = *(const f32x4*)(invstd + c0);
+        psc[h] = *(const f32x4*)(scale + c0);
+        psh[h] = *(const f32x4*)(shift + c0);
+        pk1[h] = *(const f32x4*)(coef + c0);
+        pm1[h] = *(const f32x4*)(coef + STEM_C + c0);
+        pm2[h] = *(const f32x4*)(coef + 2 * STEM_C + c0);
+    }
+    const int FT = F * T;
+    const long long NP = (long long)B * FT;
+    const long long stride = (long long)gridDim.x * 64;
+    for (long long p0 = (long long)blockIdx.x * 64 + pl; p0 < NP; p0 += stride * U) {
+        f32x4 dv[U][2], rv[U][2];
+        float xv[U][9];
+#pragma unroll
+        for (int u = 0; u < U; ++u) {
+            const long long pu = p0 + stride * u;
+            const long long p = pu < NP ? pu : p0;
+            const size_t off = (size_t)p * STEM_C + cg * 8;
+            rv[u][0] = ld_stream(raw + off);
+            rv[u][1] = ld_stream(raw + off + 4);
+            dv[u][0] = ld_stream(dy + off);
+            dv[u][1] = ld_stream(dy + off + 4);
+            const int b = (int)(p / FT);
+            const int rem = (int)(p - (long long)b * FT);
+            const int f = rem / T, t0 = rem - f * T;
+            const float* xb = x + (size_t)b * FT;
+#pragma unroll
+            for (int kh = 0; kh < 3; ++kh)
+#pragma unroll
+                for (int kw = 0; kw < 3; ++kw) {
+                    const int ff = f + kh - 1, tt = t0 + kw - 1;
+                    xv[u][kh * 3 + kw] = (ff >= 0 && ff < F && tt >= 0 && tt < T) ? xb[ff * T + tt] : 0.f;
+                }
+        }
+#pragma unroll
+        for (int u = 0; u < U; ++u) {
+            if (p0 + stride * u >= NP) continue;
+            float o8[8];
+#pragma unroll
+            for (int h = 0; h < 2; ++h) {
+                f32x4 d = dv[u][h];
+                const f32x4 z = rv[u][h] * psc[h] + psh[h];
+#pragma unroll
+                for (int k = 0; k < 4; ++k) d[k] = z[k] > 0.f ? d[k] : 0.f;
+                const f32x4 xh = (rv[u][h] - pmu[h]) * pis[h];
+                const f32x4 o = pk1[h] * (d - pm1[h] - xh * pm2[h]);
+#pragma unroll
+                for (int k = 0; k < 4; ++k) o8[h * 4 + k] = o[k];
+            }
+#pragma unroll
+            for (int t = 0; t < 9; ++t)
+#pragma unroll
+                for (int c = 0; c < 8; ++c) acc[t][c] = fmaf(xv[u][t], o8[c], acc[t][c]);
+        }
+    }
+    const int lane = tid & 63, wave = tid >> 6;
+#pragma unroll
+    for (int t = 0; t < 9; ++t)
+#pragma unroll
+        for (int c = 0; c < 8; ++c) {
+            float v = acc[t][c];
+#pragma unroll
+            for (int off = 4; off < 64; off <<= 1) v += __shfl_xor(v, off, 64);
+            if (lane < 4) red[wave][(lane * 8 + c) * 9 + t] = v;
+        }
+    __syncthreads();
+    for (int i = tid; i < STEM_C * 9; i += 256)
+        partial[(size_t)blockIdx.x * (STEM_C * 9) + i] = (red[0][i] + red[1][i]) + (red[2][i] + red[3][i]);
+}
+
 __global__ __launch_bounds__(256) void stem_wgrad_reduce_kernel(const float* __restrict__ partial, float* __restrict__ dw,
                                                                 int nblk, int accumulate) {
     __shared__ double red[256];
@@ -203,3 +344,17 @@
     SPK_LAUNCH_CHECK("spk_stem_wgrad_reduce");
     return 0;
 }
+
+extern "C" int spk_stem_bn_wgrad(const float* x, const float* d, const float* raw0, const float* mean, const float* invstd,
+                                 const float* scale, const float* shift, const float* coef, float* dw, float* partial, int B,
+                                 int F, int T, int accumulate, void* stream) {
+    SPK_REQUIRE(x && d && raw0 && mean && invstd && scale && shift && coef && dw && partial, "spk_stem_bn_wgrad: null pointer");
+    SPK_REQUIRE(B > 0 && F > 0 && T > 0, "spk_stem_bn_wgrad: empty input");
+    const int nblk = spk_stem_wgrad_blocks(B, F, T);
+    hipLaunchKernelGGL(stem_bn_wgrad_kernel, dim3(nblk), dim3(256), 0, (hipStream_t)stream, x, d, raw0, mean, invstd, scale, shift,
+                       coef, partial, B, F, T);
+    SPK_LAUNCH_CHECK("spk_stem_bn_wgrad");
+    hipLaunchKernelGGL(stem_wgrad_reduce_kernel, dim3(STEM_C * 9), dim3(256), 0, (hipStream_t)stream, partial, dw, nblk, accumulate);
+    SPK_LAUNCH_CHECK("spk_stem_wgrad_reduce");
+    return 0;
+}
diff --git a/pytorch-kaldi-resnet_amd/engine.py b/pytorch-kaldi-resnet_amd/engine.py
--- a/pytorch-kaldi-resnet_amd/engine.py
+++ b/pytorch-kaldi-resnet_amd/engine.py
@@ -69,6 +69,18 @@
         self.ds = None
         if bp.downsample is not None:
             self.ds = (_Conv(bp.downsample[0]), _BN(bp.downsample[1]))
+
+
+class _RawInput:
+
+    def __init__(self, raw, affine):
+        self.raw, self.affine = raw, affine
+
+    def materialize(self):
+        return ops.bn_apply(self.raw, self.affine[0], self.affine[1], relu=True)
+
+    def __gt__(self, other):
+        return self.materialize() > other
 
 
 class _LogitsFn(torch.autograd.Function):
@@ -117,6 +129,8 @@
         self.fuse_apply_1x1 = os.environ.get("SPK_FUSE_APPLY_1X1", "0") == "1"
         self.pair_draw = os.environ.get("SPK_PAIR_DRAW", "1") == "1"
         self.chan_amax = os.environ.get("SPK_CHAN_AMAX", "1") == "1"
+        self.stem_materialize = False
+        self.stem_exact_scale = True
         self.window_counts = None
         self.bound_log = None
 
@@ -303,18 +317,38 @@
         saved["gen"] = self._fwd_gen
         take = (lambda: pool.take()) if pool is not None else (lambda: None)
         f16 = ops.split_for(3) == 3
-        raw0, st = ops.stem_fwd(x, self.stem_conv.h.weight.data, stats=True)
-        B, F, T, _ = raw0.shape
-        t4 = self.stem_bn.finalize(st, B * F * T, keep=save)
         use_masks = save and self.use_sign_masks
-        a_amax = take()
-        a = ops.bn_apply(raw0, t4[2], t4[3], relu=True, mask=use_masks, amax_out=a_amax)
-        a, amask = a if use_masks else (a, None)
+        if self.stem_materialize:
+            raw0, st = ops.stem_fwd(x, self.stem_conv.h.weight.data, stats=True)
+            B, F, T, _ = raw0.shape
+            t4 = self.stem_bn.finalize(st, B * F * T, keep=save)
+            a_amax = take()
+            a = ops.bn_apply(raw0, t4[2], t4[3], relu=True, mask=use_masks, amax_out=a_amax)
+            a, amask = a if use_masks else (a, None)
+            a_aff = None
+        else:
+            a_amax = take()
+            if a_amax is None:
+                raw0, st = ops.stem_fwd(x, self.stem_conv.h.weight.data, stats=True)
+                B, F, T, _ = raw0.shape
+                t4 = self.stem_bn.finalize(st, B * F * T, keep=save)
+            elif self.stem_exact_scale:
+                raw0, st, mm = ops.stem_fwd(x, self.stem_conv.h.weight.data, stats=True, minmax=True)
+                B, F, T, _ = raw0.shape
+                t4 = self.stem_bn.finalize(st, B * F * T, keep=save)
+                ops.affine_relu_amax(mm, t4[2], t4[3], a_amax)
+            else:
+                raw0_amax = take()
+                raw0, st = ops.stem_fwd(x, self.stem_conv.h.weight.data, stats=True, amax_out=raw0_amax)
+                B, F, T, _ = raw0.shape
+                t4 = self.stem_bn.finalize(st, B * F * T, amax_in=raw0_amax, est_out=a_amax, keep=save)
+            a, amask, a_aff = raw0, None, (t4[2], t4[3])
         saved["raw0"] = raw0
+        saved["stem_fused"] = not self.stem_materialize
         for b in self.blocks:
-            rec = {"x": a, "xmask": amask, "in_amax": [], "raw_amax": []}
+            rec = {"x": a if a_aff is None else _RawInput(a, a_aff), "xmask": amask, "in_amax": [], "raw_amax": []}
             raws = []
-            h, aff, h_amax = a, None, a_amax
+            h, aff, h_amax = a, a_aff, a_amax
             for c, bn in zip(b.convs, b.bns):
                 rec["in_amax"].append(h_amax)
                 raw_amax = take()
@@ -329,21 +363,22 @@
                 h, aff, h_amax = raw, (t4[2], t4[3]), est
             out_amax = take()
             if b.ds is not None:
-                rawd, st = ops.conv_fwd(a, b.ds[0].wpk, b.ds[0].cout, 1, b.ds[0].stride, stats=True,
+                rawd, st = ops.conv_fwd(a, b.ds[0].wpk, b.ds[0].cout, 1, b.ds[0].stride, in_affine=a_aff, stats=True,
                                         in_amax=a_amax if ops.split_for(1) == 3 else None)
                 td = b.ds[1].finalize(st, rawd.shape[0] * rawd.shape[1] * rawd.shape[2], keep=save)
                 out = ops.bn_apply(h, aff[0], aff[1], res=rawd, res_affine=(td[2], td[3]), relu=True, mask=use_masks,
                                    amax_out=out_amax)
                 rec["rawd"] = rawd
             else:
-                out = ops.bn_apply(h, aff[0], aff[1], res=a, relu=True, mask=use_masks, amax_out=out_amax)
+                out = ops.bn_apply(h, aff[0], aff[1], res=a, res_affine=a_aff, res_relu=a_aff is not None, relu=True,
+                                   mask=use_masks, amax_out=out_amax)
             out, amask = out if use_masks else (out, None)
             rec["raws"] = raws
             rec["out"] = out
             rec["mask"] = amask
             if save:
                 saved["blocks"].append(rec)
-            a, a_amax = out, out_amax
+            a, a_amax, a_aff = out, out_amax, None
         return a, saved
 
     def _embed_train(self, x, save):
@@ -434,16 +469,26 @@
                 if on_stage_done and (bi == 0 or stage_of[bi - 1] != stage_of[bi]):
                     self._join_wgrad()
                     on_stage_done("layer%d" % stage_of[bi])
-            bn = self.stem_bn
-            draw0 = ops.bn_backward(d, saved["raw0"], None, bn.t4, bn.h.weight.data, bn.h.weight.grad, bn.h.bias.grad,
-                                    MASK_RAW, draw_out=d, accumulate=acc, partial=part)
-            ops.stem_wgrad(saved["x"], draw0, self.stem_conv.h.weight.grad, accumulate=acc)
+            bn, raw0 = self.stem_bn, saved["raw0"]
+            if saved["stem_fused"]:
+                if part is None:
+                    part = ops.bn_bwd_partial(d, raw0, None, bn.t4, MASK_RAW)
+                coef = ops.bn_bwd_coef(part, raw0.numel() // raw0.shape[-1], bn.h.weight.data, bn.t4, bn.h.weight.grad,
+                                       bn.h.bias.grad, acc)
+                ops.stem_bn_wgrad(saved["x"], d, raw0, bn.t4, coef, self.stem_conv.h.weight.grad, accumulate=acc)
+            else:
+                draw0 = ops.bn_backward(d, raw0, None, bn.t4, bn.h.weight.data, bn.h.weight.grad, bn.h.bias.grad,
+                                        MASK_RAW, draw_out=d, accumulate=acc, partial=part)
+                ops.stem_wgrad(saved["x"], draw0, self.stem_conv.h.weight.grad, accumulate=acc)
             self._join_wgrad()
             if on_stage_done:
                 on_stage_done("stem")
 
     def _block_bwd(self, b, rec, dout, acc, dout_partial=None, prev=None, dout_amax=None, amx=None, chan=False):
         x, raws, out = rec["x"], rec["raws"], rec["out"]
+        x_aff = None
+        if isinstance(x, _RawInput):
+            x, x_aff = x.raw, x.affine
         n = len(b.convs)
         g, g_part, g_amax, dz = dout, dout_partial, dout_amax, None
         take = (lambda: amx.take()) if amx is not None else (lambda: None)
@@ -451,7 +496,7 @@
             c, bn, raw = b.convs[i], b.bns[i], raws[i]
             last = i == n - 1
             inp = x if i == 0 else raws[i - 1]
-            in_aff = None if i == 0 else (b.bns[i - 1].t4[2], b.bns[i - 1].t4[3])
+            in_aff = x_aff if i == 0 else (b.bns[i - 1].t4[2], b.bns[i - 1].t4[3])
             hw = (inp.shape[1], inp.shape[2])
             act = out if last else None
             f16 = amx is not None and ops.split_for(c.k, True) == 3
@@ -463,7 +508,9 @@
                 add_dz = True
                 if c.stride == 1 and self.fuse_bn_reduce and prev is not None:
                     bnb = (prev[0], x, prev[1])
-                    if rec.get("xmask") is not None:
+                    if x_aff is not None:
+                        bnb = (prev[0], None, prev[1])
+                    elif rec.get("xmask") is not None:
                         bnb = bnb + (rec["xmask"],)
             res_amax, draw_amax = take(), take()
             pairs = f16 and self.pair_draw
@@ -535,7 +582,7 @@
             drawd = ops.bn_backward(dz, rec["rawd"], None, bnd.t4, bnd.h.weight.data, bnd.h.weight.grad, bnd.h.bias.grad,
                                     MASK_NONE, draw_out=dz, accumulate=acc, amax_out=drawd_amax)
             self._count(drawd, drawd_amax)
-            self._wgrad(x, drawd, cd.h.weight.grad, 1, cd.stride, accumulate=acc, dy_amax=drawd_amax,
+            self._wgrad(x, drawd, cd.h.weight.grad, 1, cd.stride, in_affine=x_aff, accumulate=acc, dy_amax=drawd_amax,
                         x_amax=rec["in_amax"][0] if f16d else None)
             ops.conv_dgrad(drawd, cd.wpk_t, cd.cin, 1, cd.stride, (x.shape[1], x.shape[2]), out=dx, accumulate=True,
                            in_amax=drawd_amax, out_amax=dx_amax)
diff --git a/pytorch-kaldi-resnet_amd/hip.py b/pytorch-kaldi-resnet_amd/hip.py
--- a/pytorch-kaldi-resnet_amd/hip.py
+++ b/pytorch-kaldi-resnet_amd/hip.py
@@ -40,8 +40,10 @@
     "spk_stem_fwd_blocks": [_I, _I, _I],
     "spk_stem_conv_fwd": [_P] * 6 + [_I] * 4 + [_P, _P],
     "spk_stem_conv_fwd_len": [_P] * 6 + [_I] * 4 + [_P, _P, _P],
+    "spk_stem_fwd_minmax": [_P] * 5 + [_I] * 4 + [_P, _P],
     "spk_stem_wgrad_blocks": [_I, _I, _I],
     "spk_stem_conv_wgrad": [_P] * 4 + [_I] * 4 + [_P],
+    "spk_stem_bn_wgrad": [_P] * 10 + [_I] * 4 + [_P],
     "spk_bn_stats_blocks": [_L, _I],
     "spk_bn_stats_partial": [_P, _P, _L, _I, _P],
     "spk_bn_finalize": [_P, _I, _I, _D] + [_P] * 9 + [_F, _F, _P, _P, _P, _P],
@@ -54,6 +56,7 @@
     "spk_bnbwd_estimate": [_P, _P, _P, _I, _P, _P, _P, _P],
     "spk_f16_window_count": [_P, _P, _P, _L, _I, _P, _I, _P, _P],
     "spk_affine_estimate": [_P, _P, _I, _P, _P, _P],
+    "spk_affine_relu_amax": [_P, _I, _I, _P, _P, _P, _P],
     "spk_stats_pool_fwd": [_P, _P, _I, _I, _I, _I, _I, _P],
     "spk_stats_pool_fwd_len": [_P, _P, _P, _I, _I, _I, _I, _I, _P],
     "spk_stats_pool_bwd": [_P, _P, _P, _I, _I, _I, _I, _I, _P, _P],
diff --git a/pytorch-kaldi-resnet_amd/ops.py b/pytorch-kaldi-resnet_amd/ops.py
--- a/pytorch-kaldi-resnet_amd/ops.py
+++ b/pytorch-kaldi-resnet_amd/ops.py
@@ -61,6 +61,11 @@
 def affine_estimate(scale, shift, amax_in, est):
     call("spk_affine_estimate", ptr(scale), ptr(shift), scale.numel(), ptr(amax_in), ptr(est), stream())
     return est
+
+
+def affine_relu_amax(minmax, scale, shift, slot):
+    call("spk_affine_relu_amax", ptr(minmax), minmax.shape[0], minmax.shape[2], ptr(scale), ptr(shift), ptr(slot), stream())
+    return slot
 
 
 def _amax_fwd_fallback(x, in_affine):
@@ -583,13 +588,18 @@
     return dw
 
 
-def stem_fwd(x, w, epi_affine=None, relu=False, stats=False, amax_out=None, wlen=None):
+def stem_fwd(x, w, epi_affine=None, relu=False, stats=False, amax_out=None, wlen=None, minmax=False):
     B, F, T = x.shape
     out = torch.empty(B, F, T, 32, device=x.device, dtype=torch.float32)
     flags = (EPI_AFFINE if epi_affine is not None else 0) | (EPI_RELU if relu else 0) | (EPI_STATS if stats else 0)
     st = None
     if stats:
         st = torch.empty(hip.lib().spk_stem_fwd_blocks(B, F, T), 32, 2, device=x.device, dtype=torch.float32)
+    if minmax:
+        assert epi_affine is None and not relu and wlen is None, "minmax: the raw, unmasked output only"
+        mm = torch.empty(hip.lib().spk_stem_fwd_blocks(B, F, T), 2, 32, device=x.device, dtype=torch.float32)
+        call("spk_stem_fwd_minmax", ptr(x), ptr(w), ptr(out), ptr(st), ptr(mm), B, F, T, flags, ptr(amax_out), stream())
+        return out, st, mm
     args = (ptr(x), ptr(w), ptr(out), ptr(st), ptr(epi_affine[0]) if epi_affine else None,
             ptr(epi_affine[1]) if epi_affine else None, B, F, T)
     if wlen is None:
@@ -608,6 +618,17 @@
     return dw
 
 
+def stem_bn_wgrad(x, d, raw0, bn4, coef, dw, accumulate=False):
+    B, F, T = x.shape
+    assert raw0.shape == (B, F, T, 32) and d.shape == raw0.shape
+    nblk = hip.lib().spk_stem_wgrad_blocks(B, F, T)
+    ws = _workspace(nblk * 288 * 4, x.device)
+    call("spk_stem_bn_wgrad", ptr(x), ptr(d), ptr(raw0), ptr(bn4[0]), ptr(bn4[1]), ptr(bn4[2]), ptr(bn4[3]), ptr(coef), ptr(dw),
+         ptr(ws), B, F, T, 1 if accumulate else 0, stream(),
+         label="stem_bn_wgrad_kernel", flops=2.0 * raw0.numel() * 9, nbytes=4.0 * (2 * raw0.numel() + x.numel()))
+    return dw
+
+
 def bn_stats_partial(x2d):
     N, C = x2d.shape
     nblk = hip.lib().spk_bn_stats_blocks(N, C)
@@ -639,7 +660,8 @@
     call("spk_bn_eval_coeffs", ptr(gamma), ptr(beta), ptr(rm), ptr(rv), ptr(out2[0]), ptr(out2[1]), C, BN_EPS, stream())
 
 
-def bn_apply(raw, scale, shift, res=None, res_affine=None, relu=True, out=None, mask=False, amax_out=None):
+def bn_apply(raw, scale, shift, res=None, res_affine=None, relu=True, out=None, mask=False, amax_out=None, res_relu=False):
+    assert not res_relu or res_affine is not None, "res_relu needs the residual affine"
     C = raw.shape[-1]
     N = raw.numel() // C
     if out is None:
@@ -647,7 +669,7 @@
     mk = torch.empty(N * (C // 32), device=raw.device, dtype=torch.int32) if mask else None
     call("spk_bn_apply", ptr(raw), ptr(scale), ptr(shift), ptr(res),
          ptr(res_affine[0]) if res_affine else None, ptr(res_affine[1]) if res_affine else None, ptr(out), ptr(mk), N, C,
-         1 if relu else 0, ptr(amax_out), stream(),
+         (1 if relu else 0) | (2 if res_relu else 0), ptr(amax_out), stream(),
          nbytes=4.0 * raw.numel() * (2 + (1 if res is not None else 0)) + (raw.numel() / 8 if mask else 0))
     return (out, mk) if mask else out
 
```

Measured after the change: 5564 utt/s (median of 6 runs). 2.1% higher.
